# preshanth/rfi_toolbox

Measured on AMD Instinct MI355X. Metric: training patches/sec (128x128x3), higher is better.
Workload: dtype f32; 1 GPU; UNet(3,1,32) train step (fwd+BCE/dice+bwd+clip+Adam), batch 64/GPU x 128x128x3 NHWC, BASELINE configs[1] shape on the reference's U-Net (the '3-layer CNN' of configs[1] is not in the reference; its builder-defined form runs with --workload cnn3); global_batch=64, parallelism=dp1, params=7765985

## Files before the change

include/rfi_hip.h:

```cpp
#ifndef RFI_HIP_H
#define RFI_HIP_H

#include <stddef.h>
#include <stdint.h>

#ifdef __cplusplus
extern "C" {
#endif

#define RFI_HIP_ABI_VERSION 1

enum { RFI_HOST = 0, RFI_DEVICE = 1 };

typedef struct rfi_ctx rfi_ctx;
typedef struct rfi_model rfi_model;

int         rfi_abi_version(void);
const char* rfi_last_error(void);
int rfi_device_count(int* count);
int rfi_ctx_create(int device_id, rfi_ctx** out);
int rfi_ctx_destroy(rfi_ctx* ctx);
int rfi_ctx_set_overlap(rfi_ctx* ctx, int enabled);
int rfi_ctx_synchronize(rfi_ctx* ctx);
int rfi_ctx_stream(rfi_ctx* ctx, void** hip_stream);
// ... 147 lines not shown
                            const rfi_tiling* tiling, int batch, int combine, float threshold, uint8_t* flags,
                            int flags_mem, float* prob, int prob_mem);

typedef struct rfi_flag_stats {
    int64_t count;
    int64_t flagged;
    double mean, std, median, mad, max;
} rfi_flag_stats;
enum { RFI_FS_ALL = 1, RFI_FS_CLEAN = 2, RFI_FS_MEDIANS = 4 };
int rfi_flag_statistics(rfi_ctx* ctx, const void* data, int data_mem, int dtype, int64_t count,
                        const void* flags, int flags_mem, int flags_dtype, int want,
                        rfi_flag_stats* all_out, rfi_flag_stats* clean_out);

typedef struct rfi_sim_event {
    int32_t i0, i1, i2, i3;
    double s0, sdot, r0, phi0;
    double v0, v1;
} rfi_sim_event;
typedef struct rfi_sim_params {
    int32_t time_bins, freq_bins;
    int32_t n_power;
    int32_t gibbs_ringing;
    int32_t clean;
    int32_t fixed_baseline;
    double baseline_frac, detect_floor, drift_prob, max_time_fringes, max_freq_fringes;
    double gibbs_kernel[17];
} rfi_sim_params;
enum { RFI_SIM_C128 = 0, RFI_SIM_C64 = 1, RFI_SIM_NCHW = 2, RFI_SIM_NHWC = 3 };
#define RFI_SIM_SLOTS(T, F) (14 + (int)((double)(F) * 0.05) + (int)((double)(T) * 0.1))
int rfi_simulate_rfi(rfi_ctx* ctx, uint64_t seed, uint64_t first_sample, int n_samples, const rfi_sim_params* params,
                     const double* power_range_dev, int out_layout, void* out_dev, uint8_t* mask_dev,
                     rfi_sim_event* events_dev, double* baseline_frac_dev);

typedef struct rfi_norm_stats {
    int64_t count, nonfinite;
    double min, max, mean, var;
    double q[3][2];
} rfi_norm_stats;
enum { RFI_NORM_NCHW = 0, RFI_NORM_NHWC = 1 };
int rfi_norm_bracket(int64_t count, double q, int64_t* ranks, double* frac);
int rfi_norm_statistics(rfi_ctx* ctx, const void* const* chunks, const int64_t* counts, int n_chunks, int dtype,
                        int64_t segment, int quantiles, rfi_norm_stats* out, int n_out);
int rfi_norm_apply(rfi_ctx* ctx, const void* src_dev, int dtype, int src_layout, int n, int64_t pixels, double centre,
                   double scale, const double* params_dev, float* dst_dev, int dst_layout);

typedef struct rfi_augment_config {
    uint64_t seed;
    float p_hflip, p_vflip, p_rotate, rotate_limit_deg, p_ssr, shift_limit, scale_limit, ssr_rotate_limit_deg;
} rfi_augment_config;
int rfi_augment_params(const rfi_augment_config* cfg, uint64_t call, int n, int h, int w, int32_t* gates, double* inv);
int rfi_augment_batch(rfi_ctx* ctx, const float* x, int x_mem, const uint8_t* y, int y_mem, int n, int h, int w, int c,
                      const rfi_augment_config* cfg, uint64_t call, float* x_out, uint8_t* y_out);

int rfi_op_conv3x3(rfi_ctx* ctx, int impl, const float* x, int n, int h, int w, int cin,
                   const float* w_oihw, const float* bias, int cout,
                   const float* in_scale, const float* in_shift, int in_relu, float* y);
int rfi_op_conv1x1(rfi_ctx* ctx, int impl, const float* x, int n, int h, int w, int cin, const float* w_oihw, const float* bias,
                   int cout, const float* in_scale, const float* in_shift, int in_relu, float* y);
int rfi_op_conv3x3_dgrad(rfi_ctx* ctx, int impl, const float* dy, int n, int h, int w, int cout,
                         const float* w_oihw, int cin, float* dx);
int rfi_op_conv3x3_wgrad(rfi_ctx* ctx, int impl, const float* x, const float* dy, int n, int h,
                         int w, int cin, int cout, const float* in_scale, const float* in_shift,
                         int in_relu, float* dw_oihw);
int rfi_op_conv_s2(rfi_ctx* ctx, int impl, int ksize, const float* x, int n, int h, int w, int cin,
                   const float* w_oihw, int cout, float* y);
int rfi_op_conv_s2_dgrad(rfi_ctx* ctx, int impl, int ksize, const float* dy, int n, int h, int w, int cout,
                         const float* w_oihw, int cin, float* dx);
int rfi_op_conv_s2_wgrad(rfi_ctx* ctx, int impl, int ksize, const float* x, const float* dy, int n, int h, int w,
                         int cin, int cout, float* dw_oihw);
int rfi_op_convt2x2(rfi_ctx* ctx, int impl, const float* x, int n, int h, int w, int cin,
                    const float* w_iohw, const float* bias, int cout, float* y);
int rfi_op_convt2x2_dgrad(rfi_ctx* ctx, int impl, const float* dy, int n, int h, int w, int cout,
                          const float* w_iohw, int cin, float* dx);
int rfi_op_convt2x2_wgrad(rfi_ctx* ctx, int impl, const float* x, const float* dy, int n, int h,
                          int w, int cin, int cout, float* dw_iohw);
int rfi_op_roi_align(rfi_ctx* ctx, const float* x, int n, int h, int w, int c, const float* rois, int r,
                     float spatial_scale, int ph, int pw, int sampling_ratio, int aligned, float* out);
int rfi_op_roi_align_backward(rfi_ctx* ctx, const float* dout, int n, int h, int w, int c, const float* rois_sorted, int r,
                              float spatial_scale, int ph, int pw, int sampling_ratio, int aligned, float* dx);
int rfi_op_mask_targets(rfi_ctx* ctx, const uint8_t* masks, int g, int h, int w, const float* rois, int r, int ph, int pw,
                        int sampling_ratio, uint8_t* out);
int rfi_op_box_decode(rfi_ctx* ctx, const float* anchors, int64_t n_anchors, const float* deltas, int64_t n, float clip_h,
                      float clip_w, float* boxes);
int rfi_op_nms(rfi_ctx* ctx, const float* boxes_sorted, int n, float iou_threshold, int32_t* keep_host, int* n_keep);
int rfi_op_anchor_match_batched(rfi_ctx* ctx, const float* anchors, int64_t n, int64_t anchor_stride, const int32_t* anchor_count,
                                const float* gt_boxes, int images, int gt_max, const int32_t* gt_count, float fg_iou, float bg_iou,
                                int allow_low_quality, float* best_ws, int8_t* labels, int32_t* matched, float* targets);
int rfi_op_nms_batched(rfi_ctx* ctx, const float* boxes_sorted, const int32_t* count, int sets, int k, float iou_threshold, uint8_t* keep);
int rfi_op_rpn_loss(rfi_ctx* ctx, const float* head, int64_t pixels, int anchors_per_pixel, const int8_t* labels,
                    const float* targets, const int32_t* num_sampled_dev, float beta, float* dhead, void* workspace,
                    float* loss2_dev);
size_t rfi_op_rpn_loss_ws_bytes(void);
int rfi_op_segsort_u64(rfi_ctx* ctx, uint64_t* keys, int n_segs, int stride);
int rfi_op_sample_keys(rfi_ctx* ctx, const int8_t* labels, int images, int n, const int32_t* count, uint64_t seed, uint32_t step,
                       uint32_t stream0, uint64_t* keys, int stride);
int rfi_op_rpn_sample_apply(rfi_ctx* ctx, const uint64_t* keys_sorted, int images, int n, int stride, int batch, int max_pos,
                            const int8_t* labels, const float* targets, int levels, const int32_t* level_off_host,
                            int8_t* const* level_labels_host, float* const* level_targets_host, int32_t* n_sampled);
int rfi_op_topk_keys(rfi_ctx* ctx, const float* head, int images, int pixels, int anchors_per_pixel, uint64_t* keys, int stride);
int rfi_op_topk_decode(rfi_ctx* ctx, const uint64_t* keys_sorted, int images, int stride, int pixels, int anchors_per_pixel, int k,
                       const float* head, const float* anchors, float clip_h, float clip_w, float min_size, float* boxes, float* scores,
                       int32_t* counts, int levels, int level);
int rfi_op_proposals_select(rfi_ctx* ctx, const float* boxes, const float* scores, const uint8_t* keep, int images, int levels, int k,
                            int post_nms, const float* gt_boxes, int gt_max, const int32_t* gt_count, int pmax, float* props,
                            int32_t* pcount);
int rfi_op_roi_sample(rfi_ctx* ctx, const int8_t* labels, const int32_t* pcount, int images, int pmax, int batch, int max_pos,
                      uint64_t seed, uint32_t step, uint32_t stream0, int32_t* sel, int32_t* nsel, int32_t* npos);
int rfi_op_roi_compact(rfi_ctx* ctx, const int32_t* sel, const int32_t* nsel, const int32_t* npos, int images, int batch, int pmax,
                       const float* props, const int32_t* matched, const float* targets, const int32_t* gt_labels, int gt_max,
                       const int32_t* gt_base, float t1, float t2, float t3, float* rois, int32_t* cls, float* tgt, int32_t* gt,
                       int32_t* level, int32_t* img_start, float* rois_fg, float* rois_gt, int32_t* level_fg, int32_t* fg_start,
                       int32_t* counts);
int rfi_op_roi_align_ml(rfi_ctx* ctx, const float* const* maps_host, int n, int h0, int w0, int c, float scale0, const float* rois,
                        const int32_t* level, const int32_t* count_dev, int max_rois, int ph, int pw, int sampling_ratio, float* out);
int rfi_op_roi_align_ml_backward(rfi_ctx* ctx, float* const* dmaps_host, int n, int h0, int w0, int c, float scale0, const float* dout,
                                 const float* rois, const int32_t* level, const int32_t* img_start, int max_rois, int ph, int pw,
                                 int sampling_ratio);
int rfi_op_detect_candidates(rfi_ctx* ctx, const float* head, const float* props, const int32_t* pcount, int images, int pmax, int k1,
                             float clip_h, float clip_w, float score_thresh, float min_size, float* boxes, float* scores,
                             int32_t* counts);
int rfi_op_detect_select(rfi_ctx* ctx, const float* boxes, const float* scores, const uint8_t* keep, int images, int classes, int k,
                         int max_det, float t1, float t2, float t3, float* det_boxes, float* det_scores, int32_t* det_labels,
                         int32_t* det_count, float* rois, int32_t* level);
int rfi_op_rois_from_boxes(rfi_ctx* ctx, const float* props, const int32_t* pcount, int images, int pmax, float t1, float t2, float t3,
                           float* rois, int32_t* level);
int rfi_op_mask_paste(rfi_ctx* ctx, const float* logits, const float* det_boxes, const int32_t* det_count, int images, int max_det, int h,
                      int w, uint8_t* rfi_mask, uint8_t* masks);
int rfi_op_bn_add_relu16(rfi_ctx* ctx, const uint16_t* y, const float* scale, const float* shift, const uint16_t* s, const float* s_scale,
                         const float* s_shift, int64_t m, int c, uint16_t* out);
int rfi_op_relu_mask_sum16(rfi_ctx* ctx, const uint16_t* g0, const uint16_t* g1, const float* g2_f32, const uint16_t* g2_bf16,
                           int64_t g2_stride, const uint16_t* a, int64_t m, int c, uint16_t* dz);
int rfi_op_bn_backward16(rfi_ctx* ctx, const uint16_t* da, const uint16_t* y, int64_t m, int c, const float* gamma, const float* scale,
                         const float* shift, const float* mean, const float* invstd, float slope, uint16_t* dy, float* dgamma,
                         float* dbeta, float* dbias);
int rfi_readback_begin(rfi_ctx* ctx, const void* src_dev, size_t bytes);
int rfi_readback_end(rfi_ctx* ctx, void* dst_host, size_t bytes);
int rfi_op_fpn_merge(rfi_ctx* ctx, const float* lateral, const float* top, int n, int h, int w, int c, float* out);
int rfi_op_fpn_merge_backward(rfi_ctx* ctx, const float* dout, int n, int h, int w, int c, float* dtop);
int rfi_op_bn_stats(rfi_ctx* ctx, const float* y, int64_t m, int c, float* mean, float* var_biased);
int rfi_op_bn_relu_pool(rfi_ctx* ctx, const float* y, int n, int h, int w, int c, const float* scale,
                        const float* shift, float* skip, float* pooled);
int rfi_op_pool_bwd_merge(rfi_ctx* ctx, const float* y, int n, int h, int w, int c, const float* scale,
                          const float* shift, const float* dskip, const float* dpool, float* da);
int rfi_op_bn_relu_backward(rfi_ctx* ctx, const float* y, int64_t m, int c, const float* gamma,
                            const float* beta, float* da_inout, float* dgamma, float* dbeta, float* dbias);

#ifdef __cplusplus
}
#endif
#endif
```

rfi_toolbox_amd/_lib.py:

```python
from __future__ import annotations

import ctypes as C
import os

_HERE = os.path.dirname(os.path.abspath(__file__))
LIB_PATH = os.environ.get("RFI_HIP_LIB") or os.path.join(_HERE, "librfi_hip.so")

HOST, DEVICE = 0, 1
C128, C64, F64, F32 = 0, 1, 2, 3
U8, FLOAT32 = 0, 1
IMPL_AUTO, IMPL_DIRECT, IMPL_MFMA, IMPL_MFMA_BF16, IMPL_MFMA_BF16X3, IMPL_PLANES_X3, IMPL_PLANES_BF16, IMPL_WS_X3, IMPL_WS_BF16 = 0, 1, 2, 3, 4, 5, 6, 7, 8


FS_ALL, FS_CLEAN, FS_MEDIANS = 1, 2, 4


class FlagStats(C.Structure):
    _fields_ = [("count", C.c_int64), ("flagged", C.c_int64), ("mean", C.c_double), ("std", C.c_double),
                ("median", C.c_double), ("mad", C.c_double), ("max", C.c_double)]


SIM_C128, SIM_C64, SIM_NCHW, SIM_NHWC = 0, 1, 2, 3
NORM_NCHW, NORM_NHWC = 0, 1


class NormStats(C.Structure):
    _fields_ = [("count", C.c_int64), ("nonfinite", C.c_int64), ("min", C.c_double), ("max", C.c_double),
                ("mean", C.c_double), ("var", C.c_double), ("q", C.c_double * 2 * 3)]


class AugmentConfig(C.Structure):
    _fields_ = [("seed", C.c_uint64), ("p_hflip", C.c_float), ("p_vflip", C.c_float), ("p_rotate", C.c_float),
                ("rotate_limit_deg", C.c_float), ("p_ssr", C.c_float), ("shift_limit", C.c_float),
                ("scale_limit", C.c_float), ("ssr_rotate_limit_deg", C.c_float)]


class SimParams(C.Structure):
    _fields_ = [("time_bins", C.c_int32), ("freq_bins", C.c_int32), ("n_power", C.c_int32), ("gibbs_ringing", C.c_int32),
                ("clean", C.c_int32), ("fixed_baseline", C.c_int32), ("baseline_frac", C.c_double),
                ("detect_floor", C.c_double), ("drift_prob", C.c_double), ("max_time_fringes", C.c_double),
                ("max_freq_fringes", C.c_double), ("gibbs_kernel", C.c_double * 17)]


EDGE_PAD, EDGE_SHIFT = 0, 1
COMBINE_MEAN, COMBINE_MAX = 0, 1
VALUES_LOGITS, VALUES_PROBS = 0, 1


class Tiling(C.Structure):
    _fields_ = [("ps", C.c_int32), ("stride", C.c_int32), ("edge", C.c_int32), ("views", C.c_int32)]


class Hyper(C.Structure):
    _fields_ = [("lr", C.c_double), ("beta1", C.c_double), ("beta2", C.c_double), ("eps", C.c_double),
                ("weight_decay", C.c_double), ("max_grad_norm", C.c_double)]


def _load():
    if not os.path.exists(LIB_PATH):
        raise ImportError(
            f"{LIB_PATH} is missing: build it with `python -m rfi_toolbox_amd.build` "
            "(needs hipcc; gfx950 cross-compiles without a GPU). rfi_toolbox_amd has no CPU fallback.")
    return C.CDLL(LIB_PATH, mode=C.RTLD_GLOBAL)


lib = _load()

_vp, _i, _i64, _f, _sz = C.c_void_p, C.c_int, C.c_int64, C.c_float, C.c_size_t
_pi, _pi64, _pf, _pd = C.POINTER(C.c_int), C.POINTER(C.c_int64), C.POINTER(C.c_float), C.POINTER(C.c_double)
_pvp = C.POINTER(C.c_void_p)
_cp = C.c_char_p

_PROTOS = {
    "rfi_abi_version": (_i, []),
    "rfi_last_error": (_cp, []),
    "rfi_device_count": (_i, [_pi]),
    "rfi_ctx_create": (_i, [_i, _pvp]),
    "rfi_ctx_destroy": (_i, [_vp]),
    "rfi_ctx_synchronize": (_i, [_vp]),
    "rfi_ctx_set_overlap": (_i, [_vp, _i]),
    "rfi_ctx_stream": (_i, [_vp, _pvp]),
    "rfi_ctx_device_name": (_i, [_vp, _cp, _sz]),
    "rfi_ctx_allocations": (_i, [_vp, _pi64, C.POINTER(C.c_uint64)]),
    "rfi_malloc": (_i, [_vp, _sz, _pvp]),
    "rfi_free": (_i, [_vp, _vp]),
    "rfi_memcpy": (_i, [_vp, _vp, _i, _vp, _i, _sz]),
    "rfi_memset": (_i, [_vp, _vp, _i, _sz]),
    "rfi_timer_start": (_i, [_vp]),
    "rfi_timer_stop": (_i, [_vp, _pf]),
    "rfi_profile_enable": (_i, [_vp, _i]),
    "rfi_profile_reset": (_i, [_vp]),
    "rfi_profile_family_count": (_i, []),
    "rfi_profile_family_name": (_cp, [_i]),
    "rfi_profile_get": (_i, [_vp, _i, _pi64, _pd, _pd, _pd]),
    "rfi_profile_dump": (_i, [_vp, _cp]),
    "rfi_unet_create": (_i, [_vp, _i, _i, _i, _i, _pvp]),
    "rfi_cnn3_create": (_i, [_vp, _i, _i, _i, _pvp]),
    "rfi_unet_resnet_create": (_i, [_vp, _i, _i, _i, _pvp]),
    "rfi_mask_head_create": (_i, [_vp, _i, _i, _i, _pvp]),
    "rfi_model_input_grad": (_i, [_vp, _vp, _i]),
    "rfi_rpn_head_create": (_i, [_vp, _i, _i, _i, _pvp]),
    "rfi_box_head_create": (_i, [_vp, _i, _i, _i, _i, _pvp]),
    "rfi_op_add_inplace": (_i, [_vp, _vp, _vp, _i64]),
# ... 38 lines not shown
    "rfi_op_roi_align": (_i, [_vp, _vp, _i, _i, _i, _i, _vp, _i, _f, _i, _i, _i, _i, _vp]),
    "rfi_op_mask_targets": (_i, [_vp, _vp, _i, _i, _i, _vp, _i, _i, _i, _i, _vp]),
    "rfi_op_nms_batched": (_i, [_vp, _vp, _vp, _i, _i, _f, _vp]),
    "rfi_op_roi_align_backward": (_i, [_vp, _vp, _i, _i, _i, _i, _vp, _i, _f, _i, _i, _i, _i, _vp]),
    "rfi_op_fpn_merge": (_i, [_vp, _vp, _vp, _i, _i, _i, _i, _vp]),
    "rfi_op_box_decode": (_i, [_vp, _vp, _i64, _vp, _i64, _f, _f, _vp]),
    "rfi_op_nms": (_i, [_vp, _vp, _i, _f, _vp, _pi]),
    "rfi_op_rpn_loss_ws_bytes": (_sz, []),
    "rfi_op_rpn_loss": (_i, [_vp, _vp, _i64, _i, _vp, _vp, _vp, _f, _vp, _vp, _vp]),
    "rfi_op_fastrcnn_loss": (_i, [_vp, _vp, _i64, _i, _vp, _vp, _f, _vp, _vp, _vp]),
    "rfi_op_anchor_match_batched": (_i, [_vp, _vp, _i64, _i64, _vp, _vp, _i, _i, _vp, _f, _f, _i, _vp, _vp, _vp, _vp]),
    "rfi_op_segsort_u64": (_i, [_vp, _vp, _i, _i]),
    "rfi_op_sample_keys": (_i, [_vp, _vp, _i, _i, _vp, C.c_uint64, C.c_uint32, C.c_uint32, _vp, _i]),
    "rfi_op_rpn_sample_apply": (_i, [_vp, _vp, _i, _i, _i, _i, _i, _vp, _vp, _i, _vp, _vp, _vp, _vp]),
    "rfi_op_topk_keys": (_i, [_vp, _vp, _i, _i, _i, _vp, _i]),
    "rfi_op_topk_decode": (_i, [_vp, _vp, _i, _i, _i, _i, _i, _vp, _vp, _f, _f, _f, _vp, _vp, _vp, _i, _i]),
    "rfi_op_proposals_select": (_i, [_vp, _vp, _vp, _vp, _i, _i, _i, _i, _vp, _i, _vp, _i, _vp, _vp]),
    "rfi_op_roi_sample": (_i, [_vp, _vp, _vp, _i, _i, _i, _i, C.c_uint64, C.c_uint32, C.c_uint32, _vp, _vp, _vp]),
    "rfi_op_roi_compact": (_i, [_vp, _vp, _vp, _vp, _i, _i, _i, _vp, _vp, _vp, _vp, _i, _vp, _f, _f, _f, _vp, _vp, _vp, _vp, _vp, _vp,
                                _vp, _vp, _vp, _vp, _vp]),
    "rfi_op_roi_align_ml": (_i, [_vp, _vp, _i, _i, _i, _i, _f, _vp, _vp, _vp, _i, _i, _i, _i, _vp]),
    "rfi_op_roi_align_ml_backward": (_i, [_vp, _vp, _i, _i, _i, _i, _f, _vp, _vp, _vp, _vp, _i, _i, _i, _i]),
    "rfi_op_detect_candidates": (_i, [_vp, _vp, _vp, _vp, _i, _i, _i, _f, _f, _f, _f, _vp, _vp, _vp]),
    "rfi_op_detect_select": (_i, [_vp, _vp, _vp, _vp, _i, _i, _i, _i, _f, _f, _f, _vp, _vp, _vp, _vp, _vp, _vp]),
    "rfi_op_rois_from_boxes": (_i, [_vp, _vp, _vp, _i, _i, _f, _f, _f, _vp, _vp]),
    "rfi_op_mask_paste": (_i, [_vp, _vp, _vp, _vp, _i, _i, _i, _i, _vp, _vp]),
    "rfi_op_bn_add_relu16": (_i, [_vp, _vp, _vp, _vp, _vp, _vp, _vp, _i64, _i, _vp]),
    "rfi_op_relu_mask_sum16": (_i, [_vp, _vp, _vp, _vp, _vp, _i64, _vp, _i64, _i, _vp]),
    "rfi_op_bn_backward16": (_i, [_vp, _vp, _vp, _i64, _i, _vp, _vp, _vp, _vp, _vp, _f, _vp, _vp, _vp, _vp]),
    "rfi_readback_begin": (_i, [_vp, _vp, _sz]),
    "rfi_readback_end": (_i, [_vp, _vp, _sz]),
    "rfi_op_fpn_merge_backward": (_i, [_vp, _vp, _i, _i, _i, _i, _vp]),
    "rfi_comm_allreduce_sum_f32": (_i, [_vp, _vp, _i64]),
    "rfi_model_allreduce_grads": (_i, [_vp]),
    "rfi_preprocess_patches": (_i, [_vp, _vp, _i, _i, _i, _i, _i, _vp, _i]),
    "rfi_generate_waterfalls": (_i, [_vp, C.c_uint64, _i, _i, _i, _i, C.c_double, _i, _i, C.c_double, _vp, _vp, _i,
                                     _vp, _i, _vp, _i]),
    "rfi_preprocess_real": (_i, [_vp, _vp, _i, _i, _i, _i, _i, _i, _i, _i, C.c_double, _vp, _i, _vp, _i]),
    "rfi_mad_flags": (_i, [_vp, _vp, _i, _i, _i, _i, _i, C.c_double, _vp, _i]),
    "rfi_patch_any_flag": (_i, [_vp, _vp, _i, _i, _i, _i, _vp, _i, _i, _vp]),
    "rfi_preprocess_gather": (_i, [_vp, _vp, _i, _i, _i, _i, _i, _vp, _i, _vp, _i, _i, _vp, _i, _vp, _i]),
    "rfi_confusion_counts": (_i, [_vp, _vp, _i, _i, _vp, _i, _i, _i64, _pi64, _pi64, _pi64]),
    "rfi_threshold_logits": (_i, [_vp, _vp, _i64, _f, _vp]),
    "rfi_tiling_count": (_i, [_i, _i, C.POINTER(Tiling), _pi64]),
    "rfi_stitch_patches": (_i, [_vp, _vp, _i, _i, _i, _i, _i, C.POINTER(Tiling), _i, _f, _vp, _i, _vp, _i]),
    "rfi_model_predict_flags": (_i, [_vp, _vp, _i, _i, _i, _i, _i, C.POINTER(Tiling), _i, _i, _f, _vp, _i, _vp, _i]),
    "rfi_simulate_rfi": (_i, [_vp, C.c_uint64, C.c_uint64, _i, C.POINTER(SimParams), _vp, _i, _vp, _vp, _vp, _vp]),
    "rfi_flag_statistics": (_i, [_vp, _vp, _i, _i, _i64, _vp, _i, _i, _i, C.POINTER(FlagStats), C.POINTER(FlagStats)]),
    "rfi_norm_bracket": (_i, [_i64, C.c_double, _pi64, _pd]),
    "rfi_norm_statistics": (_i, [_vp, _pvp, _pi64, _i, _i, _i64, _i, C.POINTER(NormStats), _i]),
    "rfi_norm_apply": (_i, [_vp, _vp, _i, _i, _i, _i64, C.c_double, C.c_double, _vp, _vp, _i]),
    "rfi_augment_params": (_i, [C.POINTER(AugmentConfig), C.c_uint64, _i, _i, _i, C.POINTER(C.c_int32), _pd]),
    "rfi_augment_batch": (_i, [_vp, _vp, _i, _vp, _i, _i, _i, _i, _i, C.POINTER(AugmentConfig), C.c_uint64, _vp, _vp]),
    "rfi_op_conv3x3": (_i, [_vp, _i, _vp, _i, _i, _i, _i, _vp, _vp, _i, _vp, _vp, _i, _vp]),
    "rfi_op_conv1x1": (_i, [_vp, _i, _vp, _i, _i, _i, _i, _vp, _vp, _i, _vp, _vp, _i, _vp]),
    "rfi_op_conv_s2": (_i, [_vp, _i, _i, _vp, _i, _i, _i, _i, _vp, _i, _vp]),
    "rfi_op_conv_s2_dgrad": (_i, [_vp, _i, _i, _vp, _i, _i, _i, _i, _vp, _i, _vp]),
    "rfi_op_conv_s2_wgrad": (_i, [_vp, _i, _i, _vp, _vp, _i, _i, _i, _i, _i, _vp]),
    "rfi_op_conv3x3_dgrad": (_i, [_vp, _i, _vp, _i, _i, _i, _i, _vp, _i, _vp]),
    "rfi_op_conv3x3_wgrad": (_i, [_vp, _i, _vp, _vp, _i, _i, _i, _i, _i, _vp, _vp, _i, _vp]),
    "rfi_op_convt2x2": (_i, [_vp, _i, _vp, _i, _i, _i, _i, _vp, _vp, _i, _vp]),
    "rfi_op_convt2x2_dgrad": (_i, [_vp, _i, _vp, _i, _i, _i, _i, _vp, _i, _vp]),
    "rfi_op_convt2x2_wgrad": (_i, [_vp, _i, _vp, _vp, _i, _i, _i, _i, _i, _vp]),
    "rfi_op_bn_stats": (_i, [_vp, _vp, _i64, _i, _vp, _vp]),
    "rfi_op_bn_relu_pool": (_i, [_vp, _vp, _i, _i, _i, _i, _vp, _vp, _vp, _vp]),
    "rfi_op_pool_bwd_merge": (_i, [_vp, _vp, _i, _i, _i, _i, _vp, _vp, _vp, _vp, _vp]),
    "rfi_op_bn_relu_backward": (_i, [_vp, _vp, _i64, _i, _vp, _vp, _vp, _vp, _vp, _vp]),
}

for _name, (_res, _args) in _PROTOS.items():
    _fn = getattr(lib, _name)
    _fn.restype = _res
    _fn.argtypes = _args

EXPORTED = tuple(_PROTOS)


class RfiHipError(RuntimeError):
    pass


def check(rc):
    if rc != 0:
        raise RfiHipError(lib.rfi_last_error().decode("utf-8", "replace"))


def device_count() -> int:
    n = C.c_int(0)
    check(lib.rfi_device_count(C.byref(n)))
    return n.value
```

rfi_toolbox_amd/csrc/api_ops.cpp:

```cpp
#include <algorithm>

#include "model.hpp"

using namespace rfi;

namespace {
float* upload_lib_weight(rfi_ctx* ctx, CallScope& s, const float* dev_ref, size_t numel, bool convt,
                         int d0, int d1, int R) {
    std::vector<float> h(numel), lib;
    RFI_CHECK_HIP(hipMemcpyAsync(h.data(), dev_ref, numel * 4, hipMemcpyDeviceToHost, ctx->stream));
    RFI_CHECK_HIP(hipStreamSynchronize(ctx->stream));
    if (convt) to_lib_convt(h.data(), d0, d1, lib);
    else to_lib_conv(h.data(), d0, d1, R, lib);
    float* d = s.temp<float>(numel);
    RFI_CHECK_HIP(hipMemcpyAsync(d, lib.data(), numel * 4, hipMemcpyHostToDevice, ctx->stream));
    RFI_CHECK_HIP(hipStreamSynchronize(ctx->stream));
    return d;
}
void store_ref_wgrad(rfi_ctx* ctx, const float* lib_dev, size_t numel, bool convt, int d0, int d1, float* dst_ref) {
    std::vector<float> lib(numel), ref(numel);
    RFI_CHECK_HIP(hipMemcpyAsync(lib.data(), lib_dev, numel * 4, hipMemcpyDeviceToHost, ctx->stream));
    RFI_CHECK_HIP(hipStreamSynchronize(ctx->stream));
    if (convt) from_lib_convt(lib.data(), d0, d1, ref.data());
    else from_lib_conv(lib.data(), d0, d1, 3, ref.data());
    RFI_CHECK_HIP(hipMemcpyAsync(dst_ref, ref.data(), numel * 4, hipMemcpyHostToDevice, ctx->stream));
    RFI_CHECK_HIP(hipStreamSynchronize(ctx->stream));
}

struct PlaneTmp {
    bf16_t* p = nullptr;
    int64_t ps = 0;
    int nchunks = 0;
    PlaneSeg seg() const { return PlaneSeg{p, ps, nchunks}; }
};
PlaneTmp plane_tmp(rfi_ctx* ctx, CallScope& s, int64_t pixels, int C) {
    PlaneTmp t;
    t.nchunks = plane_chunks(C);
    t.ps = (int64_t)t.nchunks * 16;
    const size_t bytes = (size_t)pixels * t.ps * 2 + 64;
    t.p = reinterpret_cast<bf16_t*>(s.temp<float>((bytes + 3) / 4));
    RFI_CHECK_HIP(hipMemsetAsync(t.p, 0, bytes, ctx->stream));
    return t;
}
PlaneTmp planes_of(rfi_ctx* ctx, CallScope& s, const float* x, int64_t pixels, int C) {
    PlaneTmp t = plane_tmp(ctx, s, pixels, C);
    launch_act_split(ctx, View{x, C}, pixels, C, InXform{}, 1, t.p, t.ps);
    return t;
}
bf16_t* wb_of(rfi_ctx* ctx, CallScope& s, const float* src, int taps, int Cout, int Cin, int seg0, int seg1) {
    const size_t e = wb_elems(taps, Cout, seg0, seg1, 1);
    bf16_t* wb = reinterpret_cast<bf16_t*>(s.temp<float>((e * 2 + 64 + 3) / 4));
    RFI_CHECK_HIP(hipMemsetAsync(wb, 0, e * 2 + 64, ctx->stream));
    launch_weights_to_wb_one(ctx, WBDesc{src, wb, taps, Cout, Cin, {seg0, seg1}, 1});
    return wb;
}
}

extern "C" {

int rfi_op_conv3x3(rfi_ctx* ctx, int impl, const float* x, int n, int h, int w, int cin,
                   const float* w_oihw, const float* bias, int cout, const float* in_scale,
                   const float* in_shift, int in_relu, float* y) {
    return guarded([&] {
        ctx->activate();
        CallScope s(ctx);
        ConvArgs a;
        a.x = View{x, cin};
        a.N = n; a.H = h; a.W = w; a.Hin = h; a.Win = w; a.Cin = cin; a.Cout = cout;
        a.w = upload_lib_weight(ctx, s, w_oihw, (size_t)9 * cin * cout, false, cout, cin, 3);
        a.bias = bias;
        a.y = MutView{y, cout};
        a.Hout = h; a.Wout = w;
        a.xf = InXform{in_scale, in_shift, in_relu};
        launch_conv(ctx, a, impl);
    });
}
int rfi_op_conv1x1(rfi_ctx* ctx, int impl, const float* x, int n, int h, int w, int cin, const float* w_oihw, const float* bias,
                   int cout, const float* in_scale, const float* in_shift, int in_relu, float* y) {
    return guarded([&] {
        ctx->activate();
        CallScope s(ctx);
        ConvArgs a;
        a.x = View{x, cin};
        a.N = n; a.H = h; a.W = w; a.Hin = h; a.Win = w; a.Cin = cin; a.Cout = cout;
        a.w = upload_lib_weight(ctx, s, w_oihw, (size_t)cin * cout, false, cout, cin, 1);
        a.bias = bias;
        a.y = MutView{y, cout};
        a.Hout = h; a.Wout = w;
        a.R = 1; a.S = 1; a.pad = 0;
        a.xf = InXform{in_scale, in_shift, in_relu};
        launch_conv(ctx, a, impl);
    });
}
int rfi_op_conv3x3_dgrad(rfi_ctx* ctx, int impl, const float* dy, int n, int h, int w, int cout,
                         const float* w_oihw, int cin, float* dx) {
    return guarded([&] {
        ctx->activate();
        CallScope s(ctx);
        float* wf = upload_lib_weight(ctx, s, w_oihw, (size_t)9 * cin * cout, false, cout, cin, 3);
        float* wd = s.temp<float>((size_t)9 * cin * cout);
        launch_weight_to_dgrad(ctx, wf, 9, cout, cin, 1, wd);
        ConvArgs a;
        a.x = View{dy, cout};
        a.N = n; a.H = h; a.W = w; a.Hin = h; a.Win = w; a.Cin = cout; a.Cout = cin;
        a.w = wd;
        a.y = MutView{dx, cin};
        a.Hout = h; a.Wout = w;
        launch_conv(ctx, a, impl);
    });
}
int rfi_op_conv3x3_wgrad(rfi_ctx* ctx, int impl, const float* x, const float* dy, int n, int h, int w,
                         int cin, int cout, const float* in_scale, const float* in_shift, int in_relu,
                         float* dw_oihw) {
    return guarded([&] {
        ctx->activate();
        CallScope s(ctx);
        WgradArgs a;
        a.xop = View{x, cin};
        a.yop = View{dy, cout};
        a.xf_x = InXform{in_scale, in_shift, in_relu};
        a.N = n; a.H = h; a.W = w; a.Hx = h; a.Wx = w; a.Cx = cin; a.Cy = cout;
        a.tap_stride = (int64_t)cin * cout;
        a.sy = cin; a.sx = 1;
        const size_t numel = (size_t)9 * cin * cout;
        a.dw = s.temp<float>(numel);
        a.slab_floats = wgrad_slab_floats(a, impl);
        a.slab = s.temp<float>(a.slab_floats);
        launch_wgrad(ctx, a, impl);
        store_ref_wgrad(ctx, a.dw, numel, false, cout, cin, dw_oihw);
    });
}
int rfi_op_conv_s2(rfi_ctx* ctx, int impl, int ksize, const float* x, int n, int h, int w, int cin, const float* w_oihw,
                   int cout, float* y) {
    return guarded([&] {
        RFI_REQUIRE(ksize == 3 || ksize == 1, "conv_s2: kernel size 3 or 1");
        ctx->activate();
        CallScope s(ctx);
        if (impl == IMPL_PLANES_BF16) {
            RFI_REQUIRE(cout % 4 == 0, "conv_s2 on planes: cout % 4 == 0");
            const int64_t Mo = (int64_t)n * (h / 2) * (w / 2);
            const PlaneTmp xp = planes_of(ctx, s, x, (int64_t)n * h * w, cin);
            const float* wl = ksize == 3 ? upload_lib_weight(ctx, s, w_oihw, (size_t)9 * cin * cout, false, cout, cin, 3) : w_oihw;
            PlaneTmp yp = plane_tmp(ctx, s, Mo, cout);
            PConvArgs a;
            a.x[0] = xp.seg(); a.nseg = 1; a.P = 1;
            a.N = n; a.H = h / 2; a.W = w / 2; a.Hin = h; a.Win = w; a.Hout = h / 2; a.Wout = w / 2;
            a.R = ksize; a.S = 2; a.pad = ksize == 3 ? 1 : 0;
            a.Cout = cout;
            a.wB = wb_of(ctx, s, wl, ksize * ksize, cout, cin, cin, 0);
            a.y16 = yp.p; a.y_pstride = (int)yp.ps;
            launch_pconv(ctx, a);
            launch_planes_to_f32(ctx, yp.p, yp.ps, Mo, cout, 1, y, cout);
            return;
        }
        float* xs = s.temp<float>((size_t)n * h * w * cin);
        launch_s2d(ctx, x, n, h, w, cin, xs);
        ConvArgs a;
        a.N = n; a.H = h / 2; a.W = w / 2; a.Hin = h / 2; a.Win = w / 2; a.Cout = cout;
        a.x = View{xs, 4 * cin};
        a.y = MutView{y, cout};
        a.Hout = h / 2; a.Wout = w / 2;
        a.S = 1;
        if (ksize == 3) {
            float* w3 = upload_lib_weight(ctx, s, w_oihw, (size_t)9 * cin * cout, false, cout, cin, 3);
            float* w2 = s.temp<float>((size_t)16 * cin * cout);
            launch_w_s2d(ctx, w3, cout, cin, w2, true);
            a.w = w2; a.Cin = 4 * cin; a.R = 2; a.pad = 1;
        } else {
            a.w = w_oihw; a.Cin = cin; a.R = 1; a.pad = 0;
        }
        launch_conv(ctx, a, impl);
// ... 493 lines not shown
                      const rfi_augment_config* cfg, uint64_t call, float* x_out, uint8_t* y_out) {
    return guarded([&] {
        RFI_REQUIRE(ctx, "augment_batch: null context");
        check_augment_config(cfg, n, h, w);
        RFI_REQUIRE(c >= 1 && c <= 16, "augment_batch: 1 <= c <= 16");
        if (n == 0) return;
        const int64_t px = (int64_t)n * h * w;
        RFI_REQUIRE(cdiv((int64_t)h * w, 256) * n <= 0x7fffffff, "augment_batch: batch too large for one launch");
        RFI_REQUIRE(x && y && x_out && y_out, "augment_batch: null buffer");
        const char *xi = reinterpret_cast<const char*>(x), *xo = reinterpret_cast<const char*>(x_out);
        const char *yi = reinterpret_cast<const char*>(y), *yo = reinterpret_cast<const char*>(y_out);
        RFI_REQUIRE(x_mem == RFI_HOST || xi + px * c * 4 <= xo || xo + px * c * 4 <= xi, "augment_batch: x and x_out overlap");
        RFI_REQUIRE(y_mem == RFI_HOST || yi + px <= yo || yo + px <= yi, "augment_batch: y and y_out overlap");
        ctx->activate();
        CallScope sc(ctx);
        const float* dx = sc.in(x, x_mem, (size_t)px * c);
        const uint8_t* dy = sc.in(y, y_mem, (size_t)px);
        const uintptr_t al = c % 4 == 0 ? 16 : 4;
        RFI_REQUIRE(reinterpret_cast<uintptr_t>(dx) % al == 0 && reinterpret_cast<uintptr_t>(x_out) % al == 0,
                    "augment_batch: float buffers must be 4-byte aligned (16-byte when c % 4 == 0)");
        launch_augment(ctx, dx, dy, n, h, w, c, *cfg, call, x_out, y_out);
        sc.finish();
    });
}
int rfi_op_fpn_merge(rfi_ctx* ctx, const float* lateral, const float* top, int n, int h, int w, int c, float* out) {
    return guarded([&] {
        ctx->activate();
        launch_fpn_merge_fwd(ctx, lateral, top, n, h, w, c, out);
    });
}
int rfi_op_fpn_merge_backward(rfi_ctx* ctx, const float* dout, int n, int h, int w, int c, float* dtop) {
    return guarded([&] {
        ctx->activate();
        launch_fpn_merge_bwd_top(ctx, dout, n, h, w, c, dtop);
    });
}
int rfi_op_bn_stats(rfi_ctx* ctx, const float* y, int64_t m, int c, float* mean, float* var_biased) {
    return guarded([&] {
        ctx->activate();
        CallScope s(ctx);
        float* ws = s.temp<float>(bn_stats_ws_floats(c));
        float* tmp = s.temp<float>((size_t)6 * c);
        std::vector<float> ones((size_t)c, 1.0f), zeros((size_t)c, 0.0f);
        RFI_CHECK_HIP(hipMemcpyAsync(tmp, ones.data(), c * 4, hipMemcpyHostToDevice, ctx->stream));
        RFI_CHECK_HIP(hipMemcpyAsync(tmp + c, zeros.data(), c * 4, hipMemcpyHostToDevice, ctx->stream));
        RFI_CHECK_HIP(hipStreamSynchronize(ctx->stream));
        launch_bn_stats(ctx, y, m, c, ws);
        launch_bn_finalize(ctx, ws, m, c, tmp, tmp + c, nullptr, nullptr, 0, mean, tmp + 2 * c, tmp + 3 * c,
                           tmp + 4 * c, var_biased);
    });
}

int rfi_op_bn_relu_pool(rfi_ctx* ctx, const float* y, int n, int h, int w, int c, const float* scale,
                        const float* shift, float* skip, float* pooled) {
    return guarded([&] {
        ctx->activate();
        launch_bn_relu_pool(ctx, y, n, h, w, c, scale, shift, MutView{skip, c}, pooled);
    });
}
int rfi_op_pool_bwd_merge(rfi_ctx* ctx, const float* y, int n, int h, int w, int c, const float* scale,
                          const float* shift, const float* dskip, const float* dpool, float* da) {
    return guarded([&] {
        ctx->activate();
        launch_pool_bwd_merge(ctx, y, n, h, w, c, scale, shift, View{dskip, c}, dpool, da);
    });
}
int rfi_op_bn_relu_backward(rfi_ctx* ctx, const float* y, int64_t m, int c, const float* gamma,
                            const float* beta, float* da_inout, float* dgamma, float* dbeta, float* dbias) {
    return guarded([&] {
        ctx->activate();
        CallScope s(ctx);
        size_t wsf = bn_stats_ws_floats(c);
        if (bn_bwd_ws_floats(m, c) > wsf) wsf = bn_bwd_ws_floats(m, c);
        float* ws = s.temp<float>(wsf);
        float* t = s.temp<float>((size_t)6 * c);
        launch_bn_stats(ctx, y, m, c, ws);
        launch_bn_finalize(ctx, ws, m, c, gamma, beta, nullptr, nullptr, 0, t, t + c, t + 2 * c, t + 3 * c,
                           nullptr);
        launch_bn_bwd_reduce(ctx, da_inout, y, m, c, t + 2 * c, t + 3 * c, t, t + c, ws, t + 4 * c, t + 5 * c,
                             dgamma, dbeta);
        launch_bn_bwd_apply(ctx, da_inout, y, m, c, t + 2 * c, t + 3 * c, t, t + c, gamma, t + 4 * c, t + 5 * c,
                            ws, dbias);
    });
}

}
```

rfi_toolbox_amd/csrc/conv_mfma.hip:

```cpp
#include <algorithm>
#include <vector>

#include "planes.hpp"

namespace rfi {

void launch_conv_direct(rfi_ctx* ctx, const ConvArgs& a);

namespace {

typedef float f32x4 __attribute__((ext_vector_type(4)));
typedef float f32x16 __attribute__((ext_vector_type(16)));
typedef float f32x2 __attribute__((ext_vector_type(2)));
typedef __bf16 bf16x2 __attribute__((ext_vector_type(2)));
typedef short s16x4 __attribute__((ext_vector_type(4)));
typedef unsigned u32x2 __attribute__((ext_vector_type(2)));

__device__ __forceinline__ s16x4 pack_bf16(f32x4 x) {
    const f32x2 lo = {x.x, x.y}, hi = {x.z, x.w};
    u32x2 r;
    r.x = __builtin_bit_cast(unsigned, __builtin_convertvector(lo, bf16x2));
    r.y = __builtin_bit_cast(unsigned, __builtin_convertvector(hi, bf16x2));
    return __builtin_bit_cast(s16x4, r);
}
// ... 572 lines not shown
        *reinterpret_cast<u32x2*>(rec) = u32x2{h0, h1};
        *reinterpret_cast<u32x2*>(rec + 8) = u32x2{m0, m1};
        *reinterpret_cast<u32x2*>(rec + 16) = u32x2{l0, l1};
    }
}
__global__ void weights_to_x3_batched_kernel(const X3Desc* __restrict__ descs) {
    const X3Desc d = descs[blockIdx.y];
    const int64_t total = d.rows * d.nchunks * 4;
    for (int64_t i = (int64_t)blockIdx.x * blockDim.x + threadIdx.x; i < total; i += (int64_t)gridDim.x * blockDim.x) {
        const int q = (int)(i & 3);
        const int64_t rc = i >> 2;
        const int chunk = (int)(rc % d.nchunks);
        const int64_t row = rc / d.nchunks;
        const int c = chunk * KC + q * 4;
        f32x4 v = {0.f, 0.f, 0.f, 0.f};
        if (c < d.Cin) v = *reinterpret_cast<const f32x4*>(d.src + row * d.Cin + c);
        unsigned h0, m0, l0, h1, m1, l1;
        split_pair(v.x, v.y, h0, m0, l0);
        split_pair(v.z, v.w, h1, m1, l1);
        float* rec = d.dst + rc * WROW3 + q * 2;
        *reinterpret_cast<u32x2*>(rec) = u32x2{h0, h1};
        *reinterpret_cast<u32x2*>(rec + 8) = u32x2{m0, m1};
        *reinterpret_cast<u32x2*>(rec + 16) = u32x2{l0, l1};
    }
}
}
void launch_weights_to_x3_batched(rfi_ctx* ctx, const X3Desc* descs_dev, int n, double total_bytes) {
    ProfScope ps(ctx, FAM_ELEMWISE, 0, total_bytes);
    hipLaunchKernelGGL(weights_to_x3_batched_kernel, dim3(128, n), dim3(256), 0, ctx->stream, descs_dev);
    check_launch("weights_to_x3_batched");
}
void launch_weights_to_x3(rfi_ctx* ctx, const float* w, int taps, int Cout, int Cin, float* out) {
    const int nchunks = (Cin + KC - 1) / KC;
    const int64_t rows = (int64_t)taps * Cout, total = rows * nchunks * 4;
    ProfScope ps(ctx, FAM_ELEMWISE, 0, (double)rows * Cin * 4 + (double)rows * nchunks * 96);
    int64_t blocks = cdiv(total, 256);
    if (blocks > 4096) blocks = 4096;
    hipLaunchKernelGGL(weights_to_x3_kernel, dim3((unsigned)blocks), dim3(256), 0, ctx->stream, w, rows, Cin, nchunks, out);
    check_launch("weights_to_x3");
}

bool conv_mfma_eligible(const ConvArgs& a) {
    if (a.Cin % 4 != 0 || a.x.pstride % 4 != 0) return false;
    if ((reinterpret_cast<uintptr_t>(a.x.p) & 15) || (reinterpret_cast<uintptr_t>(a.w) & 15)) return false;
    if (a.xf.scale && ((reinterpret_cast<uintptr_t>(a.xf.scale) & 15) ||
                       (reinterpret_cast<uintptr_t>(a.xf.shift) & 15)))
        return false;
    const bool known = (a.R == 3 && a.S == 1 && a.pad == 1) || (a.R == 1 && a.S == 1 && a.pad == 0) ||
                       (a.R == 2 && a.S == 2 && a.pad == 0) || (a.R == 2 && a.S == 1 && (a.pad == 1 || a.pad == 0));
    return known;
}

void launch_conv(rfi_ctx* ctx, ConvArgs& a, int impl) {
    if (impl == IMPL_PLANES_X3 || impl == IMPL_PLANES_BF16) {
        RFI_REQUIRE(a.R == 3 && a.S == 1 && a.zgroups == 1, "conv: the plane kernels cover 3x3 stride-1 convolutions");
        a.planes = impl == IMPL_PLANES_X3 ? 3 : 1;
        impl = IMPL_MFMA;
    }
    if (impl == IMPL_MFMA_BF16) {
        a.bf16 = true;
        impl = IMPL_MFMA;
    }
    if (impl == IMPL_MFMA_BF16X3) {
        a.bf16x3 = true;
        a.wB3 = nullptr;
        impl = IMPL_MFMA;
    }
    if (impl == IMPL_WS_X3 && conv_stem_eligible(a)) {
        a.bf16x3 = true;
        launch_conv_stem(ctx, a);
        return;
    }
    if (impl == IMPL_WS_X3 || impl == IMPL_WS_BF16) {
        const int P = impl == IMPL_WS_X3 ? 3 : 1;
        const bool gw = !conv_ws_eligible(a) && gemm_ws_eligible(a);
        RFI_REQUIRE(gw || conv_ws_eligible(a), "conv: shape not eligible for the wave-specialised kernels");
        RFI_REQUIRE(!gw || P == 3, "conv: the wave-specialised GEMM kernel exists in the 3 x bf16 arithmetic only");
        a.bf16x3 = P == 3;
        a.bf16 = P == 1;
        const int taps = gw ? (a.R == 2 ? 4 : 1) : 9, cout = gw && a.zgroups == 4 ? 4 * a.Cout : a.Cout;
        CallScope sc(ctx);
        bf16_t* wb = sc.temp<bf16_t>(wb_elems(taps, cout, a.Cin, 0, P) + 32);
        launch_weights_to_wb_one(ctx, WBDesc{a.w, wb, taps, cout, a.Cin, {a.Cin, 0}, P});
        if (gw) launch_gemm_ws(ctx, a, wb);
        else launch_conv_ws(ctx, a, wb, P);
        return;
    }
    if (impl == IMPL_AUTO && a.bf16x3 && conv_stem_eligible(a)) {
        launch_conv_stem(ctx, a);
        return;
    }
    if (impl == IMPL_AUTO && a.bf16x3 && a.wB3 && conv_ws_eligible(a)) {
        launch_conv_ws(ctx, a, a.wB3, 3);
        return;
    }
    if (impl == IMPL_AUTO && a.bf16 && a.wB1 && conv_ws_eligible(a)) {
        launch_conv_ws(ctx, a, a.wB1, 1);
        return;
    }
    if (impl == IMPL_AUTO && a.bf16x3 && a.wB3 && gemm_ws_eligible(a)) {
        launch_gemm_ws(ctx, a, a.wB3);
        return;
    }
    RFI_REQUIRE(a.N > 0 && a.H > 0 && a.W > 0 && a.Cin > 0 && a.Cout > 0, "conv: empty shape");
    RFI_REQUIRE(a.x.pstride >= a.Cin && a.y.pstride >= a.Cout, "conv: pixel stride smaller than channels");
    RFI_REQUIRE(a.zgroups == 1 || (a.zgroups == 4 && a.R == 1), "conv: zgroups only for convT forward");
// ... 54 lines not shown
```

rfi_toolbox_amd/csrc/conv_ws.hip:

```cpp
#include <algorithm>
#include <type_traits>
#include <vector>

#include <hip/hip_ext.h>

#include "ws_common.hpp"

namespace rfi {
namespace {

using namespace ws;

struct WsDev {
    const float* x;
    int x_ps;
    unsigned x_bytes;
    const float* scale;
    const float* shift;
    float slope;
    int N, H, W, Cin, Cout;
    const bf16_t* wB;
    int nkc, ncb;
    const float* bias;
    float* y;
    int y_ps;
    double* stats;
    int wide_epi;
    unsigned long long* stamps;
};

template <int P> constexpr int ROWB = 32 * P + 16;

template <int TB, int TH, int TW, int NTL, bool ADB, int P>
struct WsCfg {
    static constexpr int HH = TH + 2, HW = TW + 2, HPI = HH * HW, HP = TB * HPI;
    static constexpr int A_BYTES = (HP * ROWB<P> + 1023) & ~1023;
    static constexpr int NPIECE = 9 * NTL * P;
    static constexpr int B_BYTES = NPIECE * 1024;
    static constexpr int B_ITEMS = (NPIECE + 3) / 4;
    static constexpr int HALO_ITEMS = (HP * 4 + 255) / 256;
    static constexpr int B_OFF = (ADB ? 2 : 1) * A_BYTES;
    static constexpr int STAT_OFF = B_OFF + 2 * B_BYTES;
    static constexpr int STAT_BYTES = 4 * NTL * 64 * 2 * 8;
    static constexpr int EPI_WAVE_BYTES = 16 * 36 * 4;
    static constexpr bool WIDE_OK = STAT_OFF + 4 * EPI_WAVE_BYTES <= 160 * 1024;
    static constexpr int LDS_BYTES = STAT_OFF + ((STAT_BYTES > 4 * EPI_WAVE_BYTES || !WIDE_OK) ? STAT_BYTES : 4 * EPI_WAVE_BYTES);
    static_assert(TB * TH * TW == 256, "a tile is 256 output pixels");
    static_assert(32 % TW == 0 || TW % 32 == 0, "a 32-pixel block covers whole rows or a part of one");
    static_assert(LDS_BYTES <= 160 * 1024, "LDS budget");
};


template <int TB, int TH, int TW, int NTL, int XF, bool ADB, int P>
__global__ __launch_bounds__(512) void conv_ws_kernel(WsDev d) {
    using C = WsCfg<TB, TH, TW, NTL, ADB, P>;
    constexpr int RB = ROWB<P>;
    extern __shared__ __attribute__((aligned(16))) unsigned char smem[];
#ifdef RFI_DIAG_STAMPS
    unsigned long long st_[4] = {0, 0, 0, 0};
#endif
    const int tid = threadIdx.x;
    const int lane = tid & 63, wave = __builtin_amdgcn_readfirstlane(tid >> 6);

    const int tiles_x = (d.W + TW - 1) / TW, tiles_y = (d.H + TH - 1) / TH, tiles_b = (d.N + TB - 1) / TB;
    const int ntiles = tiles_b * tiles_y * tiles_x;
    const int GX = gridDim.x;
    int t_begin, t_count, j, gx;
    if (GX >= 8 && (GX & 7) == 0) {
        const int xcd = blockIdx.x & 7, q8 = ntiles >> 3, r8 = ntiles & 7;
        j = blockIdx.x >> 3;
        gx = GX >> 3;
        t_begin = xcd < r8 ? xcd * (q8 + 1) : r8 * (q8 + 1) + (xcd - r8) * q8;
        t_count = q8 + (xcd < r8 ? 1 : 0);
    } else {
        j = blockIdx.x; gx = GX; t_begin = 0; t_count = ntiles;
    }
    const int my_tiles = (j < t_count) ? (t_count - j + gx - 1) / gx : 0;
    const int cb0 = blockIdx.y * NTL, n0 = cb0 * 32;
    double* const st_out = d.stats ? d.stats + ((size_t)blockIdx.x * d.Cout + n0) * 2 : nullptr;
    if (my_tiles == 0) {
        if (st_out && tid < 32 * NTL && n0 + tid < d.Cout) st_out[tid * 2] = st_out[tid * 2 + 1] = 0.0;
        return;
    }
    struct Tile { int n, oy0, ox0; };
    auto tile_of = [&](int k) {
        const int t = t_begin + j + k * gx;
        Tile r;
        r.ox0 = (t % tiles_x) * TW;
        r.oy0 = ((t / tiles_x) % tiles_y) * TH;
        r.n = (t / (tiles_x * tiles_y)) * TB;
        return r;
    };
    const int nkc = d.nkc;
    const int nitems = my_tiles * nkc;
    double* const s_stat = reinterpret_cast<double*>(smem + C::STAT_OFF);

    if (wave >= 4) {
        const int ptid = tid - 256, pw = wave - 4;
        const unsigned q4b = (unsigned)(ptid & 3) * 16u;
        const __amdgpu_buffer_rsrc_t xrs = __builtin_amdgcn_make_buffer_rsrc(const_cast<float*>(d.x), 0, (int)d.x_bytes, 0x00020000);
        unsigned h_rc[C::HALO_ITEMS];
#pragma unroll
        for (int it = 0; it < C::HALO_ITEMS; ++it) {
            const int idx = ptid + it * 256, pix = idx >> 2;
            const int b = pix / C::HPI, rem = pix % C::HPI;
            h_rc[it] = idx < C::HP * 4 ? ((unsigned)b << 24) | ((unsigned)(rem / C::HW) << 12) | (unsigned)(rem % C::HW) : (0xfffu << 12);
        }
        unsigned voff[C::HALO_ITEMS];
        unsigned vmsk[C::HALO_ITEMS];
        auto setup_halo = [&](const Tile& t) {
#pragma unroll
            for (int it = 0; it < C::HALO_ITEMS; ++it) {
                const int n = t.n + (int)(h_rc[it] >> 24);
                const int iy = t.oy0 - 1 + (int)((h_rc[it] >> 12) & 0xfff), ix = t.ox0 - 1 + (int)(h_rc[it] & 0xfff);
                const bool ok = n < d.N && (unsigned)iy < (unsigned)d.H && (unsigned)ix < (unsigned)d.W;
                voff[it] = ok ? (unsigned)(((n * d.H + iy) * d.W + ix) * d.x_ps) * 4u + q4b : 0x80000000u;
                vmsk[it] = ok ? 0xffffffffu : 0u;
            }
        };
        u32x4 raw[C::HALO_ITEMS];
        f32x4 screg = {1.f, 1.f, 1.f, 1.f}, shreg = {0.f, 0.f, 0.f, 0.f};
        unsigned pl[C::HALO_ITEMS][2 * P];
        auto issue_loads = [&](int c0) {
            if constexpr (XF != 0) {
                screg = *reinterpret_cast<const f32x4*>(d.scale + c0 + (ptid & 3) * 4);
                shreg = *reinterpret_cast<const f32x4*>(d.shift + c0 + (ptid & 3) * 4);
            }
            __builtin_amdgcn_sched_barrier(0);
#pragma unroll
            for (int it = 0; it < C::HALO_ITEMS; ++it) raw[it] = __builtin_amdgcn_raw_buffer_load_b128(xrs, voff[it], c0 * 4, 0);
        };
        auto split_all = [&]() {
#pragma unroll
            for (int it = 0; it < C::HALO_ITEMS; ++it) {
                f32x4 v = __builtin_bit_cast(f32x4, raw[it]);
                if constexpr (XF != 0) {
#pragma unroll
                    for (int e = 0; e < 4; ++e) {
                        float t = v[e] * screg[e] + shreg[e];
                        if constexpr (XF == 1) asm("v_max_f32 %0, 0, %1" : "=v"(t) : "v"(t));
                        else t = __builtin_fmaxf(t, t * d.slope);
                        v[e] = __builtin_bit_cast(float, __builtin_bit_cast(unsigned, t) & vmsk[it]);
                    }
                }
                if constexpr (P == 3) {
                    split_pair(v.x, v.y, pl[it][0], pl[it][2], pl[it][4]);
                    split_pair(v.z, v.w, pl[it][1], pl[it][3], pl[it][5]);
                } else {
                    pl[it][0] = cvt_pair(v.x, v.y);
                    pl[it][1] = cvt_pair(v.z, v.w);
                }
            }
        };
        auto write_all = [&](int buf) {
            unsigned char* const sA = smem + buf * C::A_BYTES + (ptid >> 2) * RB + (ptid & 3) * 8;
#pragma unroll
            for (int it = 0; it < C::HALO_ITEMS; ++it) {
                if (ptid + it * 256 < C::HP * 4) {
                    unsigned char* row = sA + it * 64 * RB;
#pragma unroll
                    for (int p = 0; p < P; ++p) *reinterpret_cast<u32x2*>(row + 32 * p) = u32x2{pl[it][2 * p], pl[it][2 * p + 1]};
                }
            }
        };
        const unsigned char* const wb = reinterpret_cast<const unsigned char*>(d.wB);
        auto issue_B = [&](int kc, int buf) {
            unsigned char* const sB = smem + C::B_OFF + buf * C::B_BYTES;
#pragma unroll
            for (int i = 0; i < C::B_ITEMS; ++i) {
                const int p = pw + 4 * i;
                if (p < C::NPIECE) {
                    const int tap = p / (P * NTL), r = p - tap * (P * NTL), nt = r / P, plane = r - nt * P;
                    const int cb = cb0 + nt < d.ncb ? cb0 + nt : d.ncb - 1;
                    const unsigned off = (unsigned)((((tap * nkc + kc) * d.ncb + cb) * P + plane) * 1024 + lane * 16);
                    __builtin_amdgcn_global_load_lds((gbl_void*)(wb + off), (lds_void*)(sB + p * 1024), 16, 0, 0);
                }
            }
        };
        int lk = 0, lch = 0;
        Tile lt = tile_of(0);
        setup_halo(lt);
        issue_loads(0);
        for (int q = -1; q < nitems; ++q) {
            WS_T(t0);
            const bool more = q + 1 < nitems;
            if (more) {
                split_all();
                WS_T(t1);
                WS_ACC(2, t0, t1);
                if constexpr (ADB) write_all((q + 1) & 1);
                __builtin_amdgcn_sched_barrier(0);
                issue_B(lch, (q + 1) & 1);
                __builtin_amdgcn_sched_barrier(0);
                if (q + 2 < nitems) {
                    if (++lch == nkc) {
                        lch = 0;
                        ++lk;
                        lt = tile_of(lk);
                        setup_halo(lt);
                    }
                }
                issue_loads(lch * 16);
                __builtin_amdgcn_sched_barrier(0);
                WS_T(t2);
                wait_vmcnt<C::HALO_ITEMS>();
                if constexpr (ADB) asm volatile("s_waitcnt lgkmcnt(0)" ::: "memory");
                WS_T(t3);
                WS_ACC(3, t2, t3);
            }
            WS_T(t4);
            wg_barrier();
            if constexpr (!ADB) {
                if (more) write_all(0);
                asm volatile("s_waitcnt lgkmcnt(0)" ::: "memory");
                wg_barrier();
            }
            WS_T(t5);
            WS_ACC(0, t0, t4);
            WS_ACC(1, t4, t5);
        }
    } else {
        const int cw = wave, li = lane & 31, lh = lane >> 5;
        int a_base[2];
#pragma unroll
        for (int mt = 0; mt < 2; ++mt) {
            const int p = cw * 64 + mt * 32 + li;
            const int b = p / (TH * TW), r = p % (TH * TW);
            a_base[mt] = ((b * C::HH + r / TW) * C::HW + r % TW) * RB + lh * 16;
        }
        const int b_base = lane * 16;
        float bias[NTL];
        unsigned lane_off[NTL];
#pragma unroll
        for (int nt = 0; nt < NTL; ++nt) {
            const int co = n0 + nt * 32 + li;
            bias[nt] = (d.bias && co < d.Cout) ? d.bias[co] : 0.0f;
            asm volatile("" : "+v"(bias[nt]));
            lane_off[nt] = (unsigned)(4 * lh * d.y_ps + co);
        }
        constexpr bool DEFER = NTL == 1;
        f32x16 acc[2][NTL], outr[2][NTL];
#pragma unroll
        for (int mt = 0; mt < 2; ++mt)
#pragma unroll
            for (int nt = 0; nt < NTL; ++nt)
#pragma unroll
                for (int r = 0; r < 16; ++r) acc[mt][nt][r] = 0.0f;
        double d1[NTL], d2[NTL];
        float s1[NTL], s2[NTL];
#pragma unroll
        for (int nt = 0; nt < NTL; ++nt) { d1[nt] = d2[nt] = 0.0; s1[nt] = s2[nt] = 0.0f; }
        constexpr int E = 32 * NTL;
        auto epi_elem = [&](const f32x16 (&src)[2][NTL], int e, unsigned tile_off) {
            const int nt = e / 32, mt = (e >> 4) & 1, r = e & 15;
            const int p = cw * 64 + mt * 32 + (r & 3) + 8 * (r >> 2);
// ... 198 lines not shown
                    }
                    epi_finish();
                }
                cch = 0;
                ++ck;
                if (ck < my_tiles) ct = tile_of(ck);
            }
            WS_T(t4);
            wg_barrier();
            WS_T(t5);
            WS_ACC(0, t0, t1);
            WS_ACC(2, t1, t4);
            WS_ACC(1, t4, t5);
        }
        if constexpr (DEFER) {
            if (pend) {
                epi_generic(outr, pt);
                epi_finish();
            }
        }
        if (st_out) {
#pragma unroll
            for (int nt = 0; nt < NTL; ++nt) {
                s_stat[((cw * NTL + nt) * 64 + lane) * 2] = d1[nt];
                s_stat[((cw * NTL + nt) * 64 + lane) * 2 + 1] = d2[nt];
            }
        }
    }
#ifdef RFI_DIAG_STAMPS
    if (d.stamps && lane == 0) {
        unsigned long long* o = d.stamps + ((size_t)(blockIdx.y * gridDim.x + blockIdx.x) * 8 + wave) * 8;
        for (int i = 0; i < 4; ++i) o[i] = st_[i];
        o[4] = (unsigned long long)nitems;
    }
#endif
    if (st_out) {
        __syncthreads();
        if (tid < 32 * NTL && n0 + tid < d.Cout) {
            const int nt = tid >> 5, cl = tid & 31;
            double t1 = 0.0, t2 = 0.0;
#pragma unroll
            for (int w = 0; w < 4; ++w)
#pragma unroll
                for (int h = 0; h < 2; ++h) {
                    t1 += s_stat[((w * NTL + nt) * 64 + h * 32 + cl) * 2];
                    t2 += s_stat[((w * NTL + nt) * 64 + h * 32 + cl) * 2 + 1];
                }
            st_out[tid * 2] = t1;
            st_out[tid * 2 + 1] = t2;
        }
    }
}

template <int TB, int TH, int TW, int NTL, int XF, int P>
void launch_ws(rfi_ctx* ctx, ConvArgs& a, WsDev& d) {
    constexpr bool ADB = NTL == 1 || P == 1;
    using C = WsCfg<TB, TH, TW, NTL, ADB, P>;
    const int ntiles = (int)(cdiv(a.N, TB) * cdiv(a.H, TH) * cdiv(a.W, TW));
    const int ycols = (int)cdiv(d.ncb, NTL);
    const int gmax = std::max(8, 256 / ycols);
    const int tx = (int)cdiv(ntiles, 8);
    const int per = (int)cdiv(tx, std::max(1, gmax / 8));
    int GX = 8 * (int)cdiv(tx, per);
    if (ntiles < 8) GX = ntiles;
    if (a.stats && GX <= a.stats_max_records) a.stats_records = GX;
    else { a.stats = nullptr; a.stats_records = 0; }
    d.stats = a.stats;
    static PerDeviceOnce attr_once;
    attr_once.run(ctx->device, [&] {
        RFI_CHECK_HIP(hipFuncSetAttribute(reinterpret_cast<const void*>(&conv_ws_kernel<TB, TH, TW, NTL, XF, ADB, P>),
                                          hipFuncAttributeMaxDynamicSharedMemorySize, (int)C::LDS_BYTES));
    });
#ifdef RFI_DIAG_STAMPS
    {
        const size_t nw = (size_t)GX * ycols * 8;
        RFI_CHECK_HIP(hipMalloc(reinterpret_cast<void**>(&d.stamps), nw * 64));
        RFI_CHECK_HIP(hipMemsetAsync(d.stamps, 0, nw * 64, ctx->stream));
        hipLaunchKernelGGL((conv_ws_kernel<TB, TH, TW, NTL, XF, ADB, P>), dim3(GX, ycols), dim3(512), C::LDS_BYTES, ctx->stream, d);
        std::vector<unsigned long long> hs(nw * 8);
        RFI_CHECK_HIP(hipMemcpyAsync(hs.data(), d.stamps, nw * 64, hipMemcpyDeviceToHost, ctx->stream));
        RFI_CHECK_HIP(hipStreamSynchronize(ctx->stream));
        double c[5] = {0, 0, 0, 0, 0}, p[5] = {0, 0, 0, 0, 0};
        for (size_t w = 0; w < nw; ++w)
            for (int i = 0; i < 5; ++i) ((w & 7) < 4 ? c : p)[i] += (double)hs[w * 8 + i];
        std::fprintf(stderr, "[stamps] conv_ws<%d,%d,%d,%d,%d> N%d %dx%d %d->%d grid %dx%d items/wg %.1f | cycles per item: consumer mfma %.0f "
                     "epilogue %.0f barriers %.0f (+ in front of tap 8: %.0f) | producer work %.0f (split %.0f, dma wait %.0f) barriers+write %.0f\n", TB, TH, TW, NTL, XF,
                     a.N, a.H, a.W, a.Cin, a.Cout, GX, ycols, c[4] / (nw / 2), c[0] / c[4], c[2] / c[4], c[1] / c[4], c[3] / c[4], p[0] / p[4],
                     p[2] / p[4], p[3] / p[4], p[1] / p[4]);
        RFI_CHECK_HIP(hipFree(d.stamps));
        d.stamps = nullptr;
        return;
    }
#endif
    if (a.done) {
        hipExtLaunchKernelGGL((conv_ws_kernel<TB, TH, TW, NTL, XF, ADB, P>), dim3(GX, ycols), dim3(512), C::LDS_BYTES, ctx->stream, nullptr,
                              a.done, 0, d);
        a.done_used = true;
    } else {
        hipLaunchKernelGGL((conv_ws_kernel<TB, TH, TW, NTL, XF, ADB, P>), dim3(GX, ycols), dim3(512), C::LDS_BYTES, ctx->stream, d);
    }
    check_launch("conv_ws");
}

template <int NTL, int XF, int P>
void dispatch_ws(rfi_ctx* ctx, ConvArgs& a, WsDev& d) {
    if (a.W >= 32) launch_ws<1, 8, 32, NTL, XF, P>(ctx, a, d);
    else if (a.W >= 16) launch_ws<1, 16, 16, NTL, XF, P>(ctx, a, d);
    else launch_ws<4, 8, 8, NTL, XF, P>(ctx, a, d);
}
template <int NTL, int P>
void dispatch_xf(rfi_ctx* ctx, ConvArgs& a, WsDev& d, int xf) {
    if (xf == 0) dispatch_ws<NTL, 0, P>(ctx, a, d);
    else if (xf == 1) dispatch_ws<NTL, 1, P>(ctx, a, d);
    else dispatch_ws<NTL, 2, P>(ctx, a, d);
}

}

bool conv_ws_eligible(const ConvArgs& a) {
    if (!(a.R == 3 && a.S == 1 && a.pad == 1 && a.zgroups == 1 && a.fold == 0)) return false;
    if (a.Hin != a.H || a.Win != a.W || a.Hout != a.H || a.Wout != a.W) return false;
    if (a.osy != 1 || a.osx != 1 || a.ooy != 0 || a.oox != 0) return false;
    if (a.y16 || a.W < 8 || a.H < 8) return false;
    if (a.Cin % 16 != 0 || a.x.pstride % 4 != 0 || (reinterpret_cast<uintptr_t>(a.x.p) & 15)) return false;
    if (a.xf.scale && ((reinterpret_cast<uintptr_t>(a.xf.scale) & 15) || (reinterpret_cast<uintptr_t>(a.xf.shift) & 15))) return false;
    if ((int64_t)a.N * a.H * a.W * a.x.pstride * 4 >= (int64_t)1 << 31 || (int64_t)a.N * a.H * a.W * a.y.pstride >= (int64_t)1 << 31) return false;
    return true;
}

void launch_conv_ws(rfi_ctx* ctx, ConvArgs& a, const bf16_t* wB, int P) {
    RFI_REQUIRE(conv_ws_eligible(a), "conv_ws: shape not eligible");
    RFI_REQUIRE(P == 1 || P == 3, "conv_ws: planes must be 1 or 3");
    WsDev d;
    d.x = a.x.p; d.x_ps = a.x.pstride;
    d.x_bytes = (unsigned)((int64_t)a.N * a.H * a.W * a.x.pstride * 4);
    d.scale = a.xf.scale; d.shift = a.xf.shift;
    d.slope = a.xf.relu == 0 ? 1.0f : a.xf.slope;
    d.N = a.N; d.H = a.H; d.W = a.W; d.Cin = a.Cin; d.Cout = a.Cout;
    d.wB = wB;
    d.nkc = plane_chunks(a.Cin); d.ncb = (a.Cout + 31) / 32;
    RFI_REQUIRE((int64_t)wb_elems(9, a.Cout, a.Cin, 0, P) * 2 < ((int64_t)1 << 32), "conv_ws: filter tensor too large");
    d.bias = a.bias;
    d.y = a.y.p; d.y_ps = a.y.pstride;
    d.stats = nullptr;
    d.stamps = nullptr;
    d.wide_epi = a.y.pstride % 4 == 0 && (reinterpret_cast<uintptr_t>(a.y.p) & 15) == 0;
    const int64_t tiles = (a.W >= 16 ? (int64_t)a.N : cdiv(a.N, 4)) * cdiv(a.H, a.W >= 32 ? 8 : a.W >= 16 ? 16 : 8) * cdiv(a.W, a.W >= 32 ? 32 : a.W >= 16 ? 16 : 8);
    int ntl = 1;
    if (a.Cout > 32 && tiles * cdiv(d.ncb, 2) >= 224) ntl = 2;
    if (P == 1 && a.Cout > 64 && tiles * cdiv(d.ncb, 4) >= 224) ntl = 4;
    const double flops = a.algo_flops >= 0 ? a.algo_flops : 2.0 * a.N * a.H * a.W * (double)a.Cout * 9 * a.Cin;
    std::string label;
    if (ctx->profiling)
        label = "conv_ws N" + std::to_string(a.N) + " " + std::to_string(a.H) + "x" + std::to_string(a.W) + " " +
                std::to_string(a.Cin) + "->" + std::to_string(a.Cout) + (a.xf.scale ? " xf" : "") + (P == 3 ? " 3xbf16" : " bf16") +
                (a.W >= 32 ? " t8x32" : a.W >= 16 ? " t16x16" : " t4x8x8") + " ntl" + std::to_string(ntl);
    const double bytes = 4.0 * ((double)a.N * a.H * a.W * a.Cin + 9.0 * a.Cin * a.Cout) + 4.0 * a.N * a.H * a.W * a.Cout;
    ProfScope ps(ctx, FAM_CONV_MFMA, flops, bytes, label);
    const int xf = !a.xf.scale ? 0 : (a.xf.relu == 1 || (a.xf.relu == 2 && a.xf.slope == 0.0f)) ? 1 : 2;
    if (P == 3) {
        if (ntl == 2) dispatch_xf<2, 3>(ctx, a, d, xf);
        else dispatch_xf<1, 3>(ctx, a, d, xf);
    } else {
        if (ntl == 4) dispatch_xf<4, 1>(ctx, a, d, xf);
        else if (ntl == 2) dispatch_xf<2, 1>(ctx, a, d, xf);
        else dispatch_xf<1, 1>(ctx, a, d, xf);
    }
}

}
```

rfi_toolbox_amd/csrc/elem_kernels.hip:

```cpp
#include <hip/hip_ext.h>

#include "kernels.hpp"

namespace rfi {

namespace {

constexpr int kBlock = 256;
constexpr int kFinCh = 2;
constexpr int kFinLanes = kBlock / kFinCh;

__device__ __forceinline__ double wave_sum(double v) {
#pragma unroll
    for (int o = 32; o > 0; o >>= 1) v += __shfl_down(v, o, 64);
    return v;
}

__device__ __forceinline__ double finish_sum(double v, double* red) {
#pragma unroll
    for (int o = 32; o >= kFinCh; o >>= 1) v += __shfl_xor(v, o, 64);
    const int wave = threadIdx.x >> 6, lane = threadIdx.x & 63;
    __syncthreads();
    if (lane < kFinCh) red[wave * kFinCh + lane] = v;
    __syncthreads();
// ... 1442 lines not shown
    }
    if (dbias && finish_dbias) launch_bn_bwd_apply_finish(ctx, partial_ws, M, C, dbias);
}
void launch_bn_bwd_apply_finish(rfi_ctx* ctx, const float* partial_ws, int64_t M, int C, float* dbias) {
    ChanGeom g = geom_rows(M, C);
    ProfScope ps(ctx, FAM_BN);
    hipLaunchKernelGGL(finish_channel_sum_kernel, dim3((int)cdiv(C, kFinCh)), dim3(kBlock), 0,
                       ctx->stream, reinterpret_cast<const double*>(partial_ws), g.rblocks, (int64_t)C, C, dbias);
    check_launch("finish_channel_sum");
}

int bn_bwd_apply_records(int64_t M, int C) { return geom_rows(M, C).rblocks; }
void launch_finish_channel_sums_batched(rfi_ctx* ctx, const FinishSumDesc* descs_dev, int n, int max_count) {
    if (n <= 0) return;
    ProfScope ps(ctx, FAM_BN);
    hipLaunchKernelGGL(finish_channel_sum_batched_kernel, dim3((int)cdiv(max_count, kFinCh), n), dim3(kBlock), 0, ctx->stream, descs_dev);
    check_launch("finish_channel_sum_batched");
}

size_t channel_sum_ws_floats(int64_t M, int C) {
    (void)M;
    return (size_t)kMaxRowBlocks * C * 2;
}
void launch_channel_sum(rfi_ctx* ctx, YRef v, int64_t M, int C, float* partial_ws, float* out, bool finish) {
    ChanGeom g = geom_rows(M, C);
    const int pstride = (int)v.stride(C);
    const bool vec = g.V == 4 && pstride % 4 == 0 && (reinterpret_cast<uintptr_t>(v.p) & (v.bf16 ? 7 : 15)) == 0;
    RFI_REQUIRE(finish || vec, "channel_sum: deferred finishing needs the vector path (C % 4 == 0, an aligned view)");
    RFI_REQUIRE(vec || !v.bf16, "channel_sum: a bfloat16 view needs C % 4 == 0 and 8-byte aligned rows");
    if (!vec && g.V == 4) g = geom_rows(M, C, false);
    {
        ProfScope ps(ctx, FAM_REDUCE, 0, (double)M * C * (v.bf16 ? 2 : 4));
        if (g.V == 4)
            hipLaunchKernelGGL(channel_sum_kernel<4>, dim3(g.rblocks, g.cblocks), dim3(kBlock), 0, ctx->stream,
                               v.p, v.bf16, pstride, M, C, g.CL, g.rows_per_block,
                               reinterpret_cast<double*>(partial_ws));
        else
            hipLaunchKernelGGL(channel_sum_kernel<1>, dim3(g.rblocks, g.cblocks), dim3(kBlock), 0, ctx->stream,
                           v.p, v.bf16, pstride, M, C, g.CL, g.rows_per_block,
                           reinterpret_cast<double*>(partial_ws));
        check_launch("channel_sum");
    }
    if (finish) {
        ProfScope ps(ctx, FAM_REDUCE);
        hipLaunchKernelGGL(finish_channel_sum_kernel, dim3((int)cdiv(C, kFinCh)), dim3(kBlock), 0,
                           ctx->stream, reinterpret_cast<const double*>(partial_ws), g.rblocks, (int64_t)C, C, out);
        check_launch("finish_channel_sum");
    }
}
void launch_channel_sum(rfi_ctx* ctx, View v, int64_t M, int C, float* partial_ws, float* out, bool finish) {
    launch_channel_sum(ctx, YRef(v.p, (int64_t)v.pstride), M, C, partial_ws, out, finish);
}

void launch_bn_relu_pool(rfi_ctx* ctx, const float* y, int N, int H, int W, int C,
                         const float* scale, const float* shift, MutView skip, float* pooled, float slope) {
    const int64_t total = (int64_t)N * (H / 2) * (W / 2) * C;
    RFI_REQUIRE(skip.p || pooled, "bn_relu_pool: nothing to write");
    {
        ProfScope ps(ctx, FAM_ELEMWISE, 0, (double)N * H * W * C * (skip.p ? 8 : 4) + (pooled ? (double)total * 4 : 0.0));
        if (skip.p && pooled)
            hipLaunchKernelGGL((bn_relu_pool_kernel<true, true>), dim3(grid_for(total)), dim3(kBlock), 0, ctx->stream, y,
                               N, H, W, C, scale, shift, skip.p, skip.pstride, pooled, slope);
        else if (pooled)
            hipLaunchKernelGGL((bn_relu_pool_kernel<false, true>), dim3(grid_for(total)), dim3(kBlock), 0, ctx->stream, y,
                               N, H, W, C, scale, shift, nullptr, 0, pooled, slope);
        else
            hipLaunchKernelGGL((bn_relu_pool_kernel<true, false>), dim3(grid_for(total)), dim3(kBlock), 0, ctx->stream, y,
                               N, H, W, C, scale, shift, skip.p, skip.pstride, nullptr, slope);
        check_launch("bn_relu_pool");
    }
    if (skip.p && ((H & 1) || (W & 1))) {
        ProfScope ps(ctx, FAM_ELEMWISE);
        hipLaunchKernelGGL(bn_relu_edge_kernel, dim3(grid_for((int64_t)N * H * W * C)), dim3(kBlock), 0,
                           ctx->stream, y, N, H, W, C, scale, shift, skip.p, skip.pstride, slope);
        check_launch("bn_relu_edge");
    }
}

static bool pool_vec_ok(YRef y, int C, const float* scale, const float* shift, YRef dskip, YRef dpool_, const float* da) {
    const void* dpool = dpool_.p;
    return C % 4 == 0 && dskip.stride(C) % 4 == 0 && y.stride(C) % 4 == 0 &&
           !((reinterpret_cast<uintptr_t>(y.p) | reinterpret_cast<uintptr_t>(scale) | reinterpret_cast<uintptr_t>(shift) |
              reinterpret_cast<uintptr_t>(dskip.p) | reinterpret_cast<uintptr_t>(dpool) | reinterpret_cast<uintptr_t>(da)) & 15);
}
int launch_pool_bwd_merge_sums(rfi_ctx* ctx, YRef y, int N, int H, int W, int C, const float* scale,
                               const float* shift, const float* mean, const float* invstd, YRef dskip, YRef dpool,
                               float* da, float slope, float* partial_ws, unsigned short* da16) {
    if (!pool_vec_ok(y, C, scale, shift, dskip, dpool, da16 ? reinterpret_cast<const float*>(da16) : da) || dpool.stride(C) != C ||
        (reinterpret_cast<uintptr_t>(da16) & 7) ||
        ((reinterpret_cast<uintptr_t>(mean) | reinterpret_cast<uintptr_t>(invstd)) & 15))
        return 0;
    const int C4 = C / 4;
    const int64_t total = (int64_t)N * (H / 2) * (W / 2) * C4;
    const bool small = C4 <= kBlock && kBlock % C4 == 0, wide = C4 > kBlock && C4 % kBlock == 0;
    if ((H & 1) || (W & 1) || !(small || wide) || total < (int64_t)kBlock * 16) return 0;
    int grid = grid_for(total, kMaxRowBlocks);
    int records = grid;
    if (wide) {
        const int per = C4 / kBlock;
        grid = std::max(per, grid / per * per);
        records = grid / per;
    }
    if ((int64_t)grid * kBlock > total) return 0;
    ProfScope ps(ctx, FAM_ELEMWISE, 0, (double)N * H * W * C * (y.bf16 ? 10 : 12) + (double)total * (dpool.bf16 ? 8 : 16));
    hipLaunchKernelGGL(pool_bwd_merge_vec_kernel<true>, dim3(grid), dim3(kBlock), 0, ctx->stream, y.p, y.bf16, y.stride(C), N, H, W,
                       C, scale, shift, mean, invstd, dskip.p, dskip.bf16, (int)dskip.stride(C), dpool.p, dpool.bf16, da, slope, reinterpret_cast<double*>(partial_ws), da16);
// ... 287 lines not shown
```

rfi_toolbox_amd/csrc/kernels.hpp:

```cpp
#pragma once
#include "common.hpp"

namespace rfi {

struct InXform {
    const float* scale = nullptr;
    const float* shift = nullptr;
    int relu = 0;
    float slope = 0.0f;
};
static inline InXform act_xform(const float* scale, const float* shift, float slope) {
    return InXform{scale, shift, slope != 0.0f ? 2 : 1, slope};
}

struct View {
    const float* p = nullptr;
    int pstride = 0;
};
struct MutView {
    float* p = nullptr;
    int pstride = 0;
};

struct ConvArgs {
    View x;
    int N = 0, H = 0, W = 0;
    int Hin = 0, Win = 0;
    int Cin = 0, Cout = 0;
    const float* w = nullptr;
    const float* w3 = nullptr;
    const unsigned short* wB3 = nullptr;
    const unsigned short* wB1 = nullptr;
    const float* bias = nullptr;
    MutView y;
    int Hout = 0, Wout = 0;
    int osy = 1, osx = 1;
    int ooy = 0, oox = 0;
    int R = 3, S = 1, pad = 1;
    int zgroups = 1;
    unsigned short* y16 = nullptr;
    int fold = 0;
    InXform xf;
    double algo_flops = -1;
    bool bf16 = false;
    bool bf16x3 = false;
    int planes = 0;
    double* stats = nullptr;
    int stats_max_records = 0;
    int stats_records = 0;
    hipEvent_t done = nullptr;
    bool done_used = false;
#ifdef RFI_DIAG_STAMPS
    unsigned long long* stamps = nullptr;
#endif
};

enum ConvImpl { IMPL_AUTO = 0, IMPL_DIRECT = 1, IMPL_MFMA = 2, IMPL_MFMA_BF16 = 3, IMPL_MFMA_BF16X3 = 4,
                IMPL_PLANES_X3 = 5, IMPL_PLANES_BF16 = 6, IMPL_WS_X3 = 7, IMPL_WS_BF16 = 8 };
bool conv_ws_eligible(const ConvArgs& a);
void launch_conv_ws(rfi_ctx* ctx, ConvArgs& a, const unsigned short* wB, int P);
bool gemm_ws_eligible(const ConvArgs& a);
void launch_gemm_ws(rfi_ctx* ctx, ConvArgs& a, const unsigned short* wB3);

bool conv_mfma_eligible(const ConvArgs& a);
size_t weights_x3_floats(int taps, int Cout, int Cin);
void launch_weights_to_x3(rfi_ctx* ctx, const float* w, int taps, int Cout, int Cin, float* out);
struct X3Desc { const float* src; float* dst; int64_t rows; int Cin; int nchunks; };
void launch_weights_to_x3_batched(rfi_ctx* ctx, const X3Desc* descs_dev, int n, double total_bytes);
bool conv_stem_eligible(const ConvArgs& a);
void launch_conv_stem(rfi_ctx* ctx, ConvArgs& a);
void launch_conv(rfi_ctx* ctx, ConvArgs& a, int impl = IMPL_AUTO);

struct WgradArgs {
    View xop, yop;
    InXform xf_x, xf_y;
    int N = 0, H = 0, W = 0;
    int Hx = 0, Wx = 0;
    int Cx = 0, Cy = 0;
    int R = 3, S = 1, pad = 1;
    float* dw = nullptr;
    int64_t tap_stride = 0;
    int sy = 0, sx = 0;
    float* slab = nullptr;
    size_t slab_floats = 0;
    double algo_flops = -1;
    bool bf16 = false;
    bool bf16x3 = false;
    int planes = 0;
};
size_t wgrad_slab_floats(const WgradArgs& a, int impl);
bool wgrad_ws_eligible(const WgradArgs& a);
void launch_wgrad_ws(rfi_ctx* ctx, const WgradArgs& a);
size_t wgrad_ws_slab_floats(const WgradArgs& a);
bool wgrad_stem_eligible(const WgradArgs& a);
void launch_wgrad_stem(rfi_ctx* ctx, const WgradArgs& a);
void launch_wgrad(rfi_ctx* ctx, const WgradArgs& a, int impl = IMPL_AUTO);

struct YRef {
    const void* p = nullptr;
    int bf16 = 0;
    int64_t ps = 0;
    YRef(const float* f) : p(f) {}
    YRef(float* f) : p(f) {}
    YRef(const float* f, int64_t pstride) : p(f), ps(pstride) {}
    YRef(const unsigned short* h, int64_t pstride) : p(h), bf16(1), ps(pstride) {}
    YRef(View v) : p(v.p), ps(v.pstride) {}
    int64_t stride(int C) const { return ps ? ps : C; }
};

size_t bn_stats_ws_floats(int C);
void launch_bn_stats(rfi_ctx* ctx, const float* y, int64_t M, int C, float* partial_ws);
void launch_bn_finalize(rfi_ctx* ctx, const float* partial_ws, int64_t M, int C, const float* gamma,
                        const float* beta, float* running_mean, float* running_var,
                        int ema_repeats, float* mean, float* invstd, float* scale, float* shift,
                        float* var_out, int records = 0,
                        hipEvent_t done = nullptr);
void launch_bn_eval_coeffs(rfi_ctx* ctx, int C, const float* gamma, const float* beta,
                           const float* running_mean, const float* running_var, float* scale,
                           float* shift);
void launch_bn_bwd_reduce(rfi_ctx* ctx, YRef da, YRef y, int64_t M, int C,
                          const float* scale, const float* shift, const float* mean,
                          const float* invstd, float* partial_ws, float* c1, float* c2,
                          float* dgamma, float* dbeta, float slope = 0.0f);
size_t bn_bwd_ws_floats(int64_t M, int C);
void launch_bn_bwd_finalize_records(rfi_ctx* ctx, const float* partial_ws, int records, int64_t M, int C, float* c1,
                                    float* c2, float* dgamma, float* dbeta);
void launch_bn_bwd_apply(rfi_ctx* ctx, YRef da_inout, YRef y, int64_t M, int C,
                         const float* scale, const float* shift, const float* mean,
                         const float* invstd, const float* gamma, const float* c1, const float* c2,
                         float* partial_ws, float* dbias, float slope = 0.0f,
                         unsigned short* planes_out = nullptr, int64_t planes_pstride = 0, int planes_P = 0,
                         hipEvent_t done = nullptr, bool finish_dbias = true, const float* head_dl = nullptr,
                         const float* head_w = nullptr);
void launch_bn_bwd_apply_finish(rfi_ctx* ctx, const float* partial_ws, int64_t M, int C, float* dbias);
struct FinishSumDesc { const double* partial; int records; int64_t stride; int count; float* out; };
int bn_bwd_apply_records(int64_t M, int C);
void launch_finish_channel_sums_batched(rfi_ctx* ctx, const FinishSumDesc* descs_dev, int n, int max_count);

void launch_bn_relu_pool(rfi_ctx* ctx, const float* y, int N, int H, int W, int C,
                         const float* scale, const float* shift, MutView skip, float* pooled, float slope = 0.0f);
void launch_pool_bwd_merge(rfi_ctx* ctx, YRef y, int N, int H, int W, int C,
                           const float* scale, const float* shift, YRef dskip, YRef dpool,
                           float* da, float slope = 0.0f, unsigned short* da16 = nullptr);
int launch_pool_bwd_merge_sums(rfi_ctx* ctx, YRef y, int N, int H, int W, int C, const float* scale,
                               const float* shift, const float* mean, const float* invstd, YRef dskip, YRef dpool,
                               float* da, float slope, float* partial_ws, unsigned short* da16 = nullptr);
void launch_head_fwd(rfi_ctx* ctx, YRef y, int64_t M, int C, const float* scale,
                     const float* shift, const float* w, const float* b, int Cout, float* logits,
                     float slope = 0.0f);
void launch_sigmoid_fwd(rfi_ctx* ctx, const float* z, int64_t n, float* x);
void launch_sigmoid_bwd(rfi_ctx* ctx, const float* x, int64_t n, float* d_inout);
void launch_loss_reduce(rfi_ctx* ctx, const float* logits, const uint8_t* labels, int64_t count,
                        double* partial_ws, double* sums4, float* loss_out);
size_t loss_ws_doubles(int64_t count);
void launch_loss_bwd(rfi_ctx* ctx, const float* logits, const uint8_t* labels, int64_t count,
                     const double* sums4, float* dlogits);
void launch_focal_reduce(rfi_ctx* ctx, const float* logits, const uint8_t* labels, int64_t count, float alpha,
                         float gamma, double* partial_ws, float* loss_out);
void launch_focal_bwd(rfi_ctx* ctx, const float* logits, const uint8_t* labels, int64_t count, float alpha,
                      float gamma, float* dlogits);
int launch_head_bwd(rfi_ctx* ctx, YRef y, int64_t M, int C, const float* scale,
                    const float* shift, const float* w, int Cout, const float* dlogits, float* da,
                    float* partial_ws, float* dw, float* db, float slope = 0.0f, const float* bn_mean = nullptr,
                    const float* bn_invstd = nullptr, float* bn_records_ws = nullptr, unsigned short* da16 = nullptr,
                    bool* skip_da = nullptr, bool finish = true);
size_t head_bwd_ws_floats(int64_t M, int C, int Cout);
void launch_channel_sum(rfi_ctx* ctx, View v, int64_t M, int C, float* partial_ws, float* out, bool finish = true);
void launch_channel_sum(rfi_ctx* ctx, YRef v, int64_t M, int C, float* partial_ws, float* out, bool finish = true);
size_t channel_sum_ws_floats(int64_t M, int C);

void launch_nchw_to_nhwc(rfi_ctx* ctx, const float* src, int N, int C, int H, int W, float* dst);
void launch_nhwc_to_nchw(rfi_ctx* ctx, const float* src, int N, int C, int H, int W, float* dst);
void launch_weight_to_dgrad(rfi_ctx* ctx, const float* wf, int taps, int Cout, int Cin, int flip,
                            float* wd);
struct RelayoutDesc {
    int64_t src_off, dst_off;
    int taps, cout, cin, flip;
    int64_t tile0 = 0;
};
int64_t relayout_assign_tiles(RelayoutDesc* descs, int n);
void launch_weight_to_dgrad_batched(rfi_ctx* ctx, const RelayoutDesc* descs_dev, int n, const float* src,
                                    float* dst, double total_bytes, int64_t total_tiles);
void launch_u8_to_f32(rfi_ctx* ctx, const uint8_t* src, int64_t n, float* dst);
void launch_relu_bwd(rfi_ctx* ctx, float* dA, const float* Y, int64_t n);
void launch_pad_channels(rfi_ctx* ctx, const float* src, int64_t M, int c, int cp, float* dst);

void launch_sumsq(rfi_ctx* ctx, const float* g, int64_t n, double* partial_ws, double* sumsq);
size_t sumsq_ws_doubles(int64_t n);
struct AdamArgs {
    float* p; float* g; float* m; float* v; int64_t n;
    float beta2, eps, wd, max_norm, grad_scale;
    float one_minus_beta1, one_minus_beta2;
    float neg_step, bc2_sqrt;
// ... 127 lines not shown
```

rfi_toolbox_amd/csrc/model.cpp:

```cpp
#include "model.hpp"

#include <cmath>
#include <cstdlib>
#include <random>

using namespace rfi;

namespace rfi {

void DevBuf::ensure(rfi_ctx* c, size_t floats) {
    if (floats <= n && p) return;
    if (p) c->release(p);
    ctx = c;
    p = static_cast<float*>(c->alloc(floats * sizeof(float)));
    n = floats;
}
void DevBuf::free() {
    if (p && ctx) ctx->release(p);
    p = nullptr;
    n = 0;
}

}

// ... 70 lines not shown
    if (wb_pool) { ctx->release(wb_pool); wb_pool = nullptr; }
    if (wb_descs) { ctx->release(wb_descs); wb_descs = nullptr; }
    planesP = P;
    wd_dirty = true;
    pN = 0;
}

void rfi_model::prepare(int n, int h, int w) {
    RFI_REQUIRE(n > 0 && h > 0 && w > 0, "forward: empty batch or image");
    join_pending_side();
    if (ctx->stream != ctx->main_stream) {
        ctx->stream = ctx->main_stream;
        RFI_CHECK_HIP(hipStreamSynchronize(ctx->side_stream));
        side_seq = 0;
    }
    if (side_seq != 0 || ctx->fork_ring_used != 0 || ctx->bucket_ev_used != 0 || pend_hi > pend_lo) {
        RFI_CHECK_HIP(hipStreamSynchronize(ctx->main_stream));
        RFI_CHECK_HIP(hipStreamSynchronize(ctx->side_stream));
        if (ctx->comm_stream) RFI_CHECK_HIP(hipStreamSynchronize(ctx->comm_stream));
        side_seq = 0;
        ctx->fork_ring_used = 0;
        ctx->bucket_ev_used = 0;
        pend_lo = pend_hi = 0;
    }
    prepare_shape(n, h, w);
}

void UNetModel::prepare_shape(int n, int h, int w) {
    const int div = 1 << depth;
    RFI_REQUIRE(h % div == 0 && w % div == 0,
                "forward: H and W must be multiples of 2^depth (" + std::to_string(div) +
                    "), as the reference's pool/up-conv/cat chain requires; got " +
                    std::to_string(h) + "x" + std::to_string(w));
    if (n == pN && h == pH && w == pW && !bufs.empty()) return;
    ctx->activate();
    const int D = depth;
    if (bufs.empty()) {
        auto mk = [&](std::vector<int>& v) { v.assign(D + 1, -1); for (int l = 1; l <= D; ++l) v[l] = new_buf(); };
        mk(encY1); mk(encY2); mk(concat); mk(pool); mk(decY1); mk(decY2);
        mk(gA); mk(gB); mk(dconcat); mk(dpool); mk(gAe); mk(gBe);
        bottY1 = new_buf(); bottY2 = new_buf(); gBottA = new_buf(); gBottB = new_buf();
        logits = new_buf(); dlogits = new_buf(); probs = new_buf();
        x_stage = new_buf(); x_stage2 = new_buf(); x_pad = new_buf(); out_stage = new_buf();
        ws_red = new_buf(); ws_slab = new_buf(); lab_stage = new_buf();
    }
    size_t slab_need = 0, red_need = 0;
    auto upd_red = [&](size_t f) { if (f > red_need) red_need = f; };
    for (int l = 1; l <= D; ++l) {
        const size_t M = (size_t)n * (h >> (l - 1)) * (w >> (l - 1));
        const size_t C = (size_t)feat << (l - 1);
        for (int i : {decY1[l], decY2[l], gA[l], gB[l]}) bufs[i].ensure(ctx, M * C);
        if (!planesP && !resnet_encoder) for (int i : {gAe[l], gBe[l]}) bufs[i].ensure(ctx, M * C);
        if (!resnet_encoder) for (int i : {encY1[l], encY2[l]}) bufs[i].ensure(ctx, M * C);
        bufs[concat[l]].ensure(ctx, M * 2 * C);
        bufs[dconcat[l]].ensure(ctx, M * 2 * C);
        if (!resnet_encoder || l == D) {
            bufs[pool[l]].ensure(ctx, M / 4 * C);
            bufs[dpool[l]].ensure(ctx, M / 4 * C);
        }
    }
    {
        const size_t M = (size_t)n * (h >> D) * (w >> D);
        const size_t C = (size_t)feat << D;
        for (int i : {bottY1, bottY2, gBottA, gBottB}) bufs[i].ensure(ctx, M * C);
    }
    const size_t M1 = (size_t)n * h * w;
    bufs[logits].ensure(ctx, M1 * out_ch);
    bufs[dlogits].ensure(ctx, M1 * out_ch);
    bufs[probs].ensure(ctx, M1 * out_ch);
    bufs[x_stage].ensure(ctx, M1 * in_ch);
    bufs[x_stage2].ensure(ctx, M1 * in_ch);
    bufs[x_pad].ensure(ctx, M1 * convs[0].cin_p);
    bufs[out_stage].ensure(ctx, M1 * out_ch);
    bufs[lab_stage].ensure(ctx, (M1 + 3) / 4 + 4);
    size_t cmax = (size_t)feat << depth;
    upd_red(bn_stats_ws_floats((int)cmax));
    upd_red(bn_bwd_ws_floats(M1, (int)cmax));
    upd_red(head_bwd_ws_floats(M1, feat, out_ch) + bn_bwd_ws_floats(M1, feat));
    upd_red(channel_sum_ws_floats(M1, (int)cmax));
    upd_red(loss_ws_doubles(M1) * 2);
    upd_red(sumsq_ws_doubles(n_flat) * 2);
    bufs[ws_red].ensure(ctx, red_need + 16);
    auto conv_geom = [&](int ci, int& H, int& W) {
        H = h >> (convs[ci].level - 1);
        W = w >> (convs[ci].level - 1);
    };
    for (size_t ci = 0; ci < convs.size(); ++ci) {
        int H, W;
        conv_geom((int)ci, H, W);
        WgradArgs a;
        a.N = n; a.H = H; a.W = W; a.Hx = H; a.Wx = W;
        a.Cx = convs[ci].cin_p; a.Cy = convs[ci].cout;
        a.R = 3; a.S = 1; a.pad = 1;
        if (convs[ci].stride == 2) { a.Cx *= 4; a.R = 2; }
        if (convs[ci].R == 1) { a.R = 1; a.pad = 0; }
        a.xop.pstride = a.Cx; a.yop.pstride = a.Cy;
        a.tap_stride = (int64_t)a.Cx * a.Cy;
        a.bf16x3 = true;
        slab_need = std::max(slab_need, wgrad_slab_floats(a, IMPL_AUTO));
    }
    for (int k = 0; k < D; ++k) {
        const int l = D - k;
        WgradArgs a;
        a.N = n; a.H = h >> l; a.W = w >> l; a.Hx = a.H * 2; a.Wx = a.W * 2;
        a.Cx = ups[k].cout; a.Cy = ups[k].cin;
        a.xop.pstride = 2 * ups[k].cout; a.yop.pstride = a.Cy;
        a.R = 2; a.S = 2; a.pad = 0;
// ... 229 lines not shown
            hd.push_back(WBDesc{params + u.w_off, ws_pool + o, 1, 4 * u.cout, u.cin, {u.cin, 0}, P});
            ws_by_w[params + u.w_off] = ws_pool + o;
            o += ef + 32;
            hdg.push_back(WBDesc{u.wd, ws_pool + o, 4, u.cin, u.cout, {u.cout, 0}, P});
            ws_by_w[u.wd] = ws_pool + o;
            o += ed + 32;
            ws_bytes_fwd += 2.0 * ef + 4.0 * 4 * u.cin * u.cout;
            ws_bytes += 2.0 * ed + 4.0 * 4 * u.cin * u.cout;
        }
        ws_n_fwd = (int)hd.size();
        ws_bytes += ws_bytes_fwd;
        hd.insert(hd.end(), hdg.begin(), hdg.end());
        ws_n = (int)hd.size();
        ws_descs = ctx->upload_table(hd.data(), hd.size() * sizeof(WBDesc));
    }
    const WBDesc* descs = static_cast<const WBDesc*>(ws_descs);
    if (which == 0 && ws_n) launch_weights_to_wb(ctx, descs, ws_n, ws_bytes);
    if (which == 1 && ws_n_fwd) launch_weights_to_wb(ctx, descs, ws_n_fwd, ws_bytes_fwd);
    if (which == 2 && ws_n > ws_n_fwd) launch_weights_to_wb(ctx, descs + ws_n_fwd, ws_n - ws_n_fwd, ws_bytes - ws_bytes_fwd);
}

ConvArgs rfi_model::conv_same(View x, InXform xf, Shape s, int R, int pad, int cin, int cout, const float* w, const float* w3,
                              const float* bias, float* y) const {
    ConvArgs a;
    a.x = x;
    a.N = s.N; a.H = s.H; a.W = s.W; a.Hin = s.H; a.Win = s.W;
    a.Cin = cin; a.Cout = cout;
    set_filters(a, w, w3);
    a.bias = bias;
    a.y = MutView{y, cout};
    a.Hout = s.H; a.Wout = s.W;
    a.R = R; a.S = 1; a.pad = pad;
    a.xf = xf;
    return a;
}

WgradArgs rfi_model::wgrad_same(View x, InXform xf_x, const float* dy, Shape s, int R, int pad, int cin, int cout,
                                float* dw) const {
    WgradArgs wa;
    wa.xop = x;
    wa.yop = View{dy, cout};
    wa.xf_x = xf_x;
    wa.N = s.N; wa.H = s.H; wa.W = s.W; wa.Hx = s.H; wa.Wx = s.W;
    wa.Cx = cin; wa.Cy = cout;
    wa.R = R; wa.S = 1; wa.pad = pad;
    wa.dw = dw;
    wa.tap_stride = (int64_t)cin * cout;
    wa.sy = cin; wa.sx = 1;
    set_wgrad(wa);
    return wa;
}

void rfi_model::conv_bn(ConvBN& c, View in, InXform xf, Shape s, const float* w, const float* w3, int R, int pad, int cin,
                        float* Y, bool train, double flops) {
    ConvArgs a = conv_same(in, xf, s, R, pad, cin, c.cout, w, w3, c.has_bias ? params + c.b_off : nullptr, Y);
    a.algo_flops = flops;
    float* ws = buf(ws_red);
    if (train) {
        a.stats = reinterpret_cast<double*>(ws);
        a.stats_max_records = (int)(bn_stats_ws_floats(c.cout) / ((size_t)c.cout * 4));
    }
    launch_conv(ctx, a);
    const int64_t M = (int64_t)s.N * s.H * s.W;
    if (train) {
        if (a.stats_records == 0) launch_bn_stats(ctx, Y, M, c.cout, ws);
        launch_bn_finalize(ctx, ws, M, c.cout, params + c.g_off, params + c.be_off, c.running_mean(), c.running_var(),
                           c.ema_repeats, c.mean(), c.invstd(), c.scale(), c.shift(), nullptr, a.stats_records);
        c.nbt += c.ema_repeats;
    } else {
        launch_bn_eval_coeffs(ctx, c.cout, params + c.g_off, params + c.be_off, c.running_mean(), c.running_var(),
                              c.scale(), c.shift());
    }
}

ConvArgs rfi_model::convt_args(const UpConv& u, View x, InXform xf, Shape s) const {
    ConvArgs a;
    a.x = x;
    a.N = s.N; a.H = s.H; a.W = s.W; a.Hin = s.H; a.Win = s.W;
    a.Cin = u.cin; a.Cout = u.cout;
    set_filters(a, params + u.w_off, u.w3);
    a.bias = params + u.b_off;
    a.Hout = 2 * s.H; a.Wout = 2 * s.W;
    a.osy = 2; a.osx = 2;
    a.R = 1; a.S = 1; a.pad = 0;
    a.zgroups = 4;
    a.xf = xf;
    return a;
}

void rfi_model::convt_backward(const UpConv& u, View dup, View x, InXform xf, Shape s, float* dx) {
    WgradArgs wa;
    wa.xop = dup;
    wa.yop = x;
    wa.xf_y = xf;
    wa.N = s.N; wa.H = s.H; wa.W = s.W; wa.Hx = 2 * s.H; wa.Wx = 2 * s.W;
    wa.Cx = u.cout; wa.Cy = u.cin;
    wa.R = 2; wa.S = 2; wa.pad = 0;
    wa.dw = grads + u.w_off;
    wa.tap_stride = (int64_t)u.cin * u.cout;
    wa.sy = 1; wa.sx = u.cin;
    set_wgrad(wa);
    wgrad_on_side(wa, nullptr);
    ConvArgs a;
    a.x = dup;
    a.N = s.N; a.H = s.H; a.W = s.W; a.Hin = 2 * s.H; a.Win = 2 * s.W;
    a.Cin = u.cout; a.Cout = u.cin;
    set_filters(a, u.wd, u.wd3);
    a.y = MutView{dx, u.cin};
    a.Hout = s.H; a.Wout = s.W;
    a.R = 2; a.S = 2; a.pad = 0;
    launch_conv(ctx, a);
}


rfi::View rfi_model::network_input(const float* x_dev, int n, int h, int w) {
    const int cp = convs[0].cin_p;
    if (cp == in_ch) return View{x_dev, in_ch};
    launch_pad_channels(ctx, x_dev, (int64_t)n * h * w, in_ch, cp, buf(x_pad));
    return View{buf(x_pad), cp};
}

void rfi_model::forward(const float* x_dev, int n, int h, int w, bool train_mode) {
    prepare(n, h, w);
    refresh_dgrad_weights();
    forward_pass(x_dev, n, h, w, train_mode);
}

void UNetModel::forward_pass(const float* x_dev, int n, int h, int w, bool train_mode) {
    if (planesP) return forward_planes(x_dev, n, h, w, train_mode);
    const int D = depth, IB = i_bott;
    auto run_conv_bn = [&](ConvBN& c, View in, InXform xf, Shape s, float* Y) {
        conv_bn(c, in, xf, s, params + c.w_off, c.w3, 3, 1, c.cin_p, Y, train_mode, 2.0 * s.N * s.H * s.W * 9.0 * c.cin * c.cout);
    };
    View cur = network_input(x_dev, n, h, w);
    if (resnet_encoder) cur = forward_resnet_encoder(cur, n, h, w, train_mode);
    else for (int l = 1; l <= D; ++l) {
        Shape s{n, h >> (l - 1), w >> (l - 1)};
        ConvBN& c1 = convs[2 * (l - 1)];
        ConvBN& c2 = convs[2 * (l - 1) + 1];
        run_conv_bn(c1, cur, InXform{}, s, buf(encY1[l]));
        if (l == 1) side_rebuild_wd();
        run_conv_bn(c2, View{buf(encY1[l]), c1.cout}, bn_xf(c1), s, buf(encY2[l]));
        launch_bn_relu_pool(ctx, buf(encY2[l]), s.N, s.H, s.W, c2.cout, c2.scale(), c2.shift(),
                            MutView{buf(concat[l]) + c2.cout, 2 * c2.cout}, buf(pool[l]), act_slope);
        cur = View{buf(pool[l]), c2.cout};
    }
    {
        Shape s{n, h >> D, w >> D};
        ConvBN& c1 = convs[IB];
        ConvBN& c2 = convs[IB + 1];
        run_conv_bn(c1, cur, InXform{}, s, buf(bottY1));
        run_conv_bn(c2, View{buf(bottY1), c1.cout}, bn_xf(c1), s, buf(bottY2));
    }
    const float* prevY = buf(bottY2);
    ConvBN* prevBN = &convs[IB + 1];
    for (int l = D; l >= 1; --l) {
        const int k = D - l;
        UpConv& u = ups[k];
        Shape sin{n, h >> l, w >> l};
        Shape s{n, h >> (l - 1), w >> (l - 1)};
        ConvArgs a = convt_args(u, View{prevY, u.cin}, bn_xf(*prevBN), sin);
        a.y = MutView{buf(concat[l]), 2 * u.cout};
        launch_conv(ctx, a);
        ConvBN& c1 = convs[IB + 2 + 2 * k];
        ConvBN& c2 = convs[IB + 2 + 2 * k + 1];
        run_conv_bn(c1, View{buf(concat[l]), 2 * u.cout}, InXform{}, s, buf(decY1[l]));
        run_conv_bn(c2, View{buf(decY1[l]), c1.cout}, bn_xf(c1), s, buf(decY2[l]));
        prevY = buf(decY2[l]);
        prevBN = &c2;
    }
    const int64_t M1 = (int64_t)n * h * w;
    launch_head_fwd(ctx, prevY, M1, feat, prevBN->scale(), prevBN->shift(), params + head_w_off,
                    params + head_b_off, out_ch, buf(logits), act_slope);
    if (head_sigmoid) launch_sigmoid_fwd(ctx, buf(logits), M1 * out_ch, buf(probs));
}

void rfi_model::loss_forward(const uint8_t* labels_dev, int n, int h, int w) {
    RFI_REQUIRE(out_ch == 1, "loss: the reference's BCE+dice step is defined for out_channels == 1");
    const int64_t cnt = (int64_t)n * h * w * out_scale * out_scale;
    if (loss_kind == 1) {
        launch_focal_reduce(ctx, buf(head_sigmoid ? probs : logits), labels_dev, cnt, focal_alpha, focal_gamma,
                            reinterpret_cast<double*>(buf(ws_red)), d_scalars);
        return;
    }
    launch_loss_reduce(ctx, buf(head_sigmoid ? probs : logits), labels_dev, cnt,
                       reinterpret_cast<double*>(buf(ws_red)), d_sums, d_scalars);
}

void rfi_model::side_begin() {
    if (!ctx->overlap) return;
    RFI_CHECK_HIP(hipEventRecord(ctx->fork_ev, ctx->main_stream));
    RFI_CHECK_HIP(hipStreamWaitEvent(ctx->side_stream, ctx->fork_ev, 0));
    ctx->stream = ctx->side_stream;
}
hipEvent_t rfi_model::next_fork_event() {
    static const bool off = getenv("RFI_NO_STOP_EVENTS") != nullptr;
    if (!ctx->overlap || off) return nullptr;
    if (ctx->fork_ring_used == ctx->fork_ring.size()) {
        hipEvent_t e;
        RFI_CHECK_HIP(hipEventCreateWithFlags(&e, hipEventDisableTiming));
        ctx->fork_ring.push_back(e);
    }
    return ctx->fork_ring[ctx->fork_ring_used++];
}
void rfi_model::side_begin_after(hipEvent_t producer_done) {
    if (!producer_done) return side_begin();
    if (!ctx->overlap) return;
    RFI_CHECK_HIP(hipStreamWaitEvent(ctx->side_stream, producer_done, 0));
    ctx->stream = ctx->side_stream;
}
void rfi_model::side_end() {
    if (!ctx->overlap) return;
    const int ring = (int)ctx->side_done.size();
    RFI_CHECK_HIP(hipEventRecord(ctx->side_done[side_seq % ring], ctx->side_stream));
    ctx->stream = ctx->main_stream;
    if (side_bound > 0 && side_seq >= side_bound)
        RFI_CHECK_HIP(hipStreamWaitEvent(ctx->main_stream, ctx->side_done[(side_seq - side_bound) % ring], 0));
    ++side_seq;
}
// ... 22 lines not shown

static hipEvent_t bucket_event(rfi_ctx* ctx) {
    if (ctx->bucket_ev_used == ctx->bucket_ev.size()) {
        hipEvent_t e;
        RFI_CHECK_HIP(hipEventCreateWithFlags(&e, hipEventDisableTiming));
        ctx->bucket_ev.push_back(e);
    }
    return ctx->bucket_ev[ctx->bucket_ev_used++];
}
void rfi_model::bucket_ready(size_t lo, size_t hi) {
    if (!exchange_in_backward || !ctx->exchange_active() || hi <= lo) return;
    static const bool no_buckets = getenv("RFI_NO_BUCKETS") != nullptr;
    const char* mf = getenv("RFI_BUCKET_MIN_FLOATS");
    const size_t min_floats = mf ? (size_t)atoll(mf) : (size_t)1 << 20;
    if (pend_hi > pend_lo) {
        RFI_REQUIRE(hi == pend_lo || lo == pend_hi, "bucket_ready: buckets must be adjacent");
        pend_lo = std::min(pend_lo, lo);
        pend_hi = std::max(pend_hi, hi);
    } else {
        pend_lo = lo;
        pend_hi = hi;
    }
    if (no_buckets) return;
    if (pend_hi - pend_lo < min_floats && pend_lo != 0) return;
    flush_bucket();
}
void rfi_model::flush_bucket() {
    if (pend_hi <= pend_lo) return;
    const size_t lo = pend_lo, hi = pend_hi;
    pend_lo = pend_hi = 0;
    hipEvent_t em = bucket_event(ctx);
    RFI_CHECK_HIP(hipEventRecord(em, ctx->main_stream));
    RFI_CHECK_HIP(hipStreamWaitEvent(ctx->comm_stream, em, 0));
    if (ctx->overlap) {
        hipEvent_t es = bucket_event(ctx);
        RFI_CHECK_HIP(hipEventRecord(es, ctx->side_stream));
        RFI_CHECK_HIP(hipStreamWaitEvent(ctx->comm_stream, es, 0));
    }
    comm_bucket_allreduce(ctx, grads + lo, (int64_t)(hi - lo));
}
void rfi_model::exchange_join() {
    if (!ctx->exchange_active()) return;
    flush_bucket();
    hipEvent_t e = bucket_event(ctx);
    RFI_CHECK_HIP(hipEventRecord(e, ctx->comm_stream));
    RFI_CHECK_HIP(hipStreamWaitEvent(ctx->main_stream, e, 0));
    ctx->bucket_ev_used = 0;
}

namespace {

void backward_conv_bn(UNetModel* m, ConvBN& c, float* dA, const float* Y, View in, InXform in_xf,
                      Shape s, float* dx, int have_records,
                      const float* head_dl = nullptr, const float* head_w = nullptr) {
    rfi_ctx* ctx = m->ctx;
    const int64_t M = (int64_t)s.N * s.H * s.W;
    float* ws = m->buf(m->ws_red);
    if (have_records > 0)
        launch_bn_bwd_finalize_records(ctx, ws, have_records, M, c.cout, c.c1(), c.c2(), m->grads + c.g_off,
                                       m->grads + c.be_off);
    else
        launch_bn_bwd_reduce(ctx, dA, Y, M, c.cout, c.scale(), c.shift(), c.mean(), c.invstd(), ws, c.c1(),
                             c.c2(), m->grads + c.g_off, m->grads + c.be_off, m->act_slope);
    const hipEvent_t dy_done = dx ? nullptr : m->next_fork_event();
    launch_bn_bwd_apply(ctx, dA, Y, M, c.cout, c.scale(), c.shift(), c.mean(), c.invstd(),
                        m->params + c.g_off, c.c1(), c.c2(), m->dbias_deferred ? m->dbias_pool + c.dbias_rec_off : ws,
                        m->grads + c.b_off, m->act_slope, nullptr, 0, 0, dy_done, !m->dbias_deferred, head_dl, head_w);
    WgradArgs wa = m->wgrad_same(in, in_xf, dA, s, 3, 1, c.cin_p, c.cout, m->grads + c.w_off);
    wa.algo_flops = 2.0 * s.N * s.H * s.W * 9.0 * c.cin * c.cout;
    if (!dx) {
        m->wgrad_on_side(wa, dy_done);
        return;
    }
    ConvArgs a = m->conv_same(View{dA, c.cout}, InXform{}, s, 3, 1, c.cout, c.cin, c.wd, c.wd3, nullptr, dx);
    a.done = m->next_fork_event();
    launch_conv(ctx, a);
    m->wgrad_on_side(wa, a.done_used ? a.done : nullptr, !a.done_used);
}

}

void rfi_model::wgrad_on_side(const rfi::WgradArgs& wa, hipEvent_t after, bool after_everything) {
    SideScope side(this, after_everything ? nullptr : after);
    launch_wgrad(ctx, wa);
    side.end();
}

void rfi_model::backward(const float* x_dev, const uint8_t* labels_dev, int n, int h, int w) {
    join_pending_side();
    backward_pass(x_dev, labels_dev, n, h, w);
}

void UNetModel::backward_pass(const float* x_dev, const uint8_t* labels_dev, int n, int h, int w) {
    const int D = depth, IB = i_bott;
    const int64_t M1 = (int64_t)n * h * w;
    refresh_dgrad_weights();
    wait_wd();
    if (planesP) return backward_planes(x_dev, labels_dev, n, h, w);
    side_bound = resnet_encoder ? 2 : 0;
    dbias_deferred = !resnet_encoder && dbias_pool && !ctx->exchange_active();
    if (loss_kind == 1)
        launch_focal_bwd(ctx, buf(head_sigmoid ? probs : logits), labels_dev, M1, focal_alpha, focal_gamma, buf(dlogits));
    else
        launch_loss_bwd(ctx, buf(head_sigmoid ? probs : logits), labels_dev, M1, d_sums, buf(dlogits));
    if (head_sigmoid) launch_sigmoid_bwd(ctx, buf(probs), M1 * out_ch, buf(dlogits));
    int head_records = 0;
    bool head_skip = out_ch == 1;
    {
        ConvBN& last = convs[IB + 2 + 2 * (D - 1) + 1];
        const bool hdefer = dbias_deferred && head_fin_deferred;
        head_records = launch_head_bwd(ctx, buf(decY2[1]), M1, feat, last.scale(), last.shift(), params + head_w_off,
                                       out_ch, buf(dlogits), buf(gA[1]),
                                       hdefer ? dbias_pool + head_rec_off : buf(ws_red) + bn_bwd_ws_floats(M1, feat),
                                       grads + head_w_off, grads + head_b_off, act_slope, last.mean(), last.invstd(),
                                       buf(ws_red), nullptr, &head_skip, !hdefer);
    }
    for (int l = 1; l <= D; ++l) {
        const int k = D - l;
        Shape s{n, h >> (l - 1), w >> (l - 1)};
        Shape sin{n, h >> l, w >> l};
        ConvBN& c1 = convs[IB + 2 + 2 * k];
        ConvBN& c2 = convs[IB + 2 + 2 * k + 1];
        UpConv& u = ups[k];
        const bool from_head = l == 1 && head_skip;
        backward_conv_bn(this, c2, buf(gA[l]), buf(decY2[l]), View{buf(decY1[l]), c1.cout}, bn_xf(c1), s,
                         buf(gB[l]), l == 1 ? head_records : 0, from_head ? buf(dlogits) : nullptr,
                         from_head ? params + head_w_off : nullptr);
        backward_conv_bn(this, c1, buf(gB[l]), buf(decY1[l]), View{buf(concat[l]), 2 * u.cout}, InXform{}, s,
                         buf(dconcat[l]), 0);
        const float* prevY = (l == D) ? buf(bottY2) : buf(decY2[l + 1]);
        ConvBN& prevBN = (l == D) ? convs[IB + 1] : convs[IB + 2 + 2 * (k - 1) + 1];
        View dUp{buf(dconcat[l]), 2 * u.cout};
        {
            const bool defer = dbias_deferred && u.cout % 4 == 0;
            launch_channel_sum(ctx, dUp, (int64_t)s.N * s.H * s.W, u.cout, defer ? dbias_pool + u.dbias_rec_off : buf(ws_red),
                               grads + u.b_off, !defer);
        }
        convt_backward(u, dUp, View{prevY, u.cin}, bn_xf(prevBN), sin, (l == D) ? buf(gBottA) : buf(gA[l + 1]));
        bucket_ready(u.w_off, l == 1 ? n_flat : ups[k + 1].w_off);
    }
    {
        Shape s{n, h >> D, w >> D};
        ConvBN& c1 = convs[IB];
        ConvBN& c2 = convs[IB + 1];
        backward_conv_bn(this, c2, buf(gBottA), buf(bottY2), View{buf(bottY1), c1.cout}, bn_xf(c1), s, buf(gBottB), 0);
        backward_conv_bn(this, c1, buf(gBottB), buf(bottY1), View{buf(pool[D]), c1.cin}, InXform{}, s, buf(dpool[D]), 0);
        bucket_ready(c1.w_off, ups[0].w_off);
    }
    if (resnet_encoder) {
        backward_resnet_encoder(x_dev, n, h, w);
        side_join();
        return;
    }
    for (int l = D; l >= 1; --l) {
        Shape s{n, h >> (l - 1), w >> (l - 1)};
        ConvBN& c1 = convs[2 * (l - 1)];
        ConvBN& c2 = convs[2 * (l - 1) + 1];
        const std::vector<int>& gA = this->gAe;
        const std::vector<int>& gB = this->gBe;
        int have = launch_pool_bwd_merge_sums(ctx, buf(encY2[l]), s.N, s.H, s.W, c2.cout, c2.scale(), c2.shift(), c2.mean(),
                                              c2.invstd(), View{buf(dconcat[l]) + c2.cout, 2 * c2.cout}, buf(dpool[l]),
                                              buf(gA[l]), act_slope, buf(ws_red));
        if (!have)
            launch_pool_bwd_merge(ctx, buf(encY2[l]), s.N, s.H, s.W, c2.cout, c2.scale(), c2.shift(),
                                  View{buf(dconcat[l]) + c2.cout, 2 * c2.cout}, buf(dpool[l]), buf(gA[l]), act_slope);
        backward_conv_bn(this, c2, buf(gA[l]), buf(encY2[l]), View{buf(encY1[l]), c1.cout}, bn_xf(c1), s, buf(gB[l]), have);
        View in = (l == 1) ? (c1.cin_p == in_ch ? View{x_dev, in_ch} : View{buf(x_pad), c1.cin_p})
                           : View{buf(pool[l - 1]), c1.cin};
        backward_conv_bn(this, c1, buf(gB[l]), buf(encY1[l]), in, InXform{}, s,
                         (l == 1) ? nullptr : buf(dpool[l - 1]), 0);
        bucket_ready(c1.w_off, convs[l == D ? IB : 2 * l].w_off);
    }
    if (dbias_deferred) launch_finish_channel_sums_batched(ctx, static_cast<const FinishSumDesc*>(dbias_descs), dbias_n, dbias_max_c);
    side_join();
    side_bound = 2;
}

void rfi_model::apply(const rfi_hyper& hp, float grad_scale) {
    join_pending_side();
    double* ws = reinterpret_cast<double*>(buf(ws_red));
    launch_sumsq(ctx, grads, (int64_t)n_flat, ws, d_sums + 4);
    adam_step += 1;
    AdamArgs a;
    a.p = params; a.g = grads; a.m = adam_m; a.v = adam_v; a.n = (int64_t)n_flat;
    a.beta2 = (float)hp.beta2; a.eps = (float)hp.eps; a.wd = (float)hp.weight_decay;
    a.max_norm = (float)hp.max_grad_norm; a.grad_scale = grad_scale;
    a.one_minus_beta1 = (float)(1.0 - hp.beta1);
    a.one_minus_beta2 = (float)(1.0 - hp.beta2);
    a.neg_step = (float)(-(hp.lr / (1.0 - std::pow(hp.beta1, (double)adam_step))));
    a.bc2_sqrt = (float)std::sqrt(1.0 - std::pow(hp.beta2, (double)adam_step));
    a.sumsq = d_sums + 4;
    a.norm_out = d_scalars + 1;
    launch_adam(ctx, a);
    wd_dirty = true;
    x3_fresh = false;
}

void rfi_model::set_compute_dtype(int dtype) {
    arith = dtype == 1 || dtype == 4 ? Arith::BF16 : dtype == 2 || dtype == 3 ? Arith::X3 : Arith::F32;
}
void UNetModel::set_compute_dtype(int dtype) {
    rfi_model::set_compute_dtype(dtype);
    if (resnet_encoder) set_planes(dtype == 1 && feat % 16 == 0 ? 1 : 0);
    else set_planes(dtype == 1 ? 1 : (dtype == 3 ? 3 : 0));
}

void rfi_model::debug_tensor(const std::string&, const std::string&, int, bool, const float*&, size_t&) {
    throw Error("debug_tensor: this model exposes only logits / dlogits / chan (and the decoder tensors of the ResNet-encoder U-Net)");
}
void UNetModel::debug_tensor(const std::string& name, const std::string& base, int idx, bool to_host, const float*& src, size_t& n) {
    if (resnet_encoder && (base == "encY1" || base == "encY2" || base == "pool" || base == "dpool"))
        return rfi_model::debug_tensor(name, base, idx, to_host, src, n);
    RFI_REQUIRE(!(y16_flow && planesP == 1 && (base == "encY1" || base == "encY2" || base == "decY1" || base == "bottY1" ||
                                               (base == "decY2" && idx == 1))),
                "debug_tensor: this conv output is stored as bfloat16 in the bfloat16 compute mode");
    RFI_REQUIRE(!(g16_flow && planesP == 1 && (base == "gB" || base == "dpool" || base == "gBottB" || base == "gA")),
                "debug_tensor: this gradient tensor is stored as bfloat16 in the bfloat16 compute mode");
    RFI_REQUIRE(!(convt_planes && planesP == 1 && (base == "decY2" || base == "bottY2" || base == "gBottA")),
                "debug_tensor: with the transposed convs on the plane kernels this tensor is stored as bfloat16");
    const int D = depth;
    auto level = [&](const std::vector<int>& v, size_t chmul) {
        RFI_REQUIRE(idx >= 1 && idx <= D, "debug_tensor: level out of range");
        const size_t M = (size_t)pN * (pH >> (idx - 1)) * (pW >> (idx - 1));
        src = buf(v[idx]);
        n = M * ((size_t)feat << (idx - 1)) * chmul;
    };
    const size_t Mb = (size_t)pN * (pH >> D) * (pW >> D), Cb = (size_t)feat << D;
    if (base == "encY1") level(encY1, 1);
    else if (base == "encY2") level(encY2, 1);
    else if (base == "decY1") level(decY1, 1);
    else if (base == "decY2") level(decY2, 1);
    else if (base == "gA") level(!planesP && !resnet_encoder ? gAe : gA, 1);
    else if (base == "gB") level(!planesP && !resnet_encoder ? gBe : gB, 1);
    else if (base == "concat") level(concat, 2);
    else if (base == "dconcat") {
        level(dconcat, 2);
        if (convt_planes && planesP == 1 && to_host) {
            const PlaneBuf& g = pl[g16cat[idx]];
            launch_planes_to_f32(ctx, g.p, g.pstride, (int64_t)(n / ((size_t)2 * (feat << (idx - 1)))), 2 * (feat << (idx - 1)), 1,
                                 buf(dconcat[idx]), 2 * (feat << (idx - 1)));
        }
    }
    else if (base == "pool") { level(pool, 1); n /= 4; }
    else if (base == "dpool") { level(dpool, 1); n /= 4; }
    else if (base == "bottY1") { src = buf(bottY1); n = Mb * Cb; }
    else if (base == "bottY2") { src = buf(bottY2); n = Mb * Cb; }
    else if (base == "gBottA") { src = buf(gBottA); n = Mb * Cb; }
    else if (base == "gBottB") { src = buf(gBottB); n = Mb * Cb; }
    else throw Error("debug_tensor: unknown tensor " + name);
}

void UNetModel::algorithmic_flops(int n, int h, int w, double& fwd, double& step) const {
    double f = 0, stem = 0;
    for (size_t ci = 0; ci < convs.size(); ++ci) {
        const int lvl = convs[ci].level, R = convs[ci].R;
        const double M = (double)n * (h >> (lvl - 1)) * (w >> (lvl - 1));
        const double fl = 2.0 * M * R * R * convs[ci].cin * convs[ci].cout;
        f += fl;
        if (ci == 0) stem = fl;
    }
    for (int k = 0; k < depth; ++k) {
        const int l = depth - k;
        const double M = (double)n * (h >> l) * (w >> l);
        f += 2.0 * M * 4.0 * ups[k].cin * ups[k].cout;
    }
    f += 2.0 * n * h * w * (double)feat * out_ch;
    fwd = f;
    step = 3.0 * f - stem;
}
```

rfi_toolbox_amd/csrc/model.hpp:

```cpp
#pragma once
#include "planes.hpp"

namespace rfi {

struct DevBuf {
    rfi_ctx* ctx = nullptr;
    float* p = nullptr;
    size_t n = 0;
    void ensure(rfi_ctx* c, size_t floats);
    void free();
};

struct PlaneBuf {
    rfi_ctx* ctx = nullptr;
    bf16_t* p = nullptr;
    size_t elems = 0;
    int64_t pstride = 0;
    int nchunks = 0;
    void ensure(rfi_ctx* c, int64_t pixels, int C, int P);
    void free();
};

struct ConvBN {
    std::string conv_name, bn_name;
// ... 160 lines not shown
    int relayout_n = 0;
    int64_t relayout_tiles = 0;
    double relayout_bytes = 0;

    int pN = 0, pH = 0, pW = 0;
    std::vector<rfi::DevBuf> bufs;
    int logits = -1, dlogits = -1;
    int x_stage = -1, x_stage2 = -1, x_pad = -1, out_stage = -1, ws_red = -1, ws_slab = -1, lab_stage = -1;
    int gx = -1;
    bool ext_dlogits = false;
    double* d_sums = nullptr;
    float* d_scalars = nullptr;
    float last_loss = 0, last_norm = 0;

    rfi_model(int in, int out, int f, int d) : in_ch(in), out_ch(out), feat(f), depth(d) {}
    virtual ~rfi_model();
    virtual void build() = 0;
    void prepare(int n, int h, int w);
    virtual void prepare_shape(int n, int h, int w) = 0;
    void forward(const float* x_dev, int n, int h, int w, bool train_mode);
    virtual void forward_pass(const float* x_dev, int n, int h, int w, bool train_mode) = 0;
    void loss_forward(const uint8_t* labels_dev, int n, int h, int w);
    void backward(const float* x_dev, const uint8_t* labels_dev, int n, int h, int w);
    virtual void backward_pass(const float* x_dev, const uint8_t* labels_dev, int n, int h, int w) = 0;
    void apply(const rfi_hyper& hp, float grad_scale);
    virtual void algorithmic_flops(int n, int h, int w, double& fwd, double& step) const = 0;
    virtual void set_compute_dtype(int dtype);
    virtual void debug_tensor(const std::string& name, const std::string& base, int idx, bool to_host, const float*& src, size_t& n);

    size_t chan_floats = 0, wd_floats = 0;
    int add_conv(rfi::ConvBN c);
    void add_up(const std::string& name, int cin, int cout);
    void add_head(const std::string& name, int cin);
    void alloc_state();
    void reset_channel_state();
    const rfi::Entry& entry(const char* name) const;
    void init_params(uint64_t seed);
    void load_entry(const rfi::Entry& e, const void* host, size_t bytes);
    void store_entry(const rfi::Entry& e, void* host, size_t bytes);
    void store_flat(const float* flat, const rfi::Entry& e, void* host, size_t bytes);
    void load_adam(const rfi::Entry& e, const void* host_m, const void* host_v, size_t bytes);
    float* buf(int i) { return bufs[i].p; }
    int new_buf() { bufs.emplace_back(); return (int)bufs.size() - 1; }
    rfi::View network_input(const float* x_dev, int n, int h, int w);
    void refresh_dgrad_weights();
    virtual bool wd_split_ok() const { return false; }
    virtual void refresh_model_weights(int which) {}

    rfi::ConvArgs conv_same(rfi::View x, rfi::InXform xf, rfi::Shape s, int R, int pad, int cin, int cout, const float* w,
                            const float* w3, const float* bias, float* y) const;
    rfi::WgradArgs wgrad_same(rfi::View x, rfi::InXform xf_x, const float* dy, rfi::Shape s, int R, int pad, int cin, int cout,
                              float* dw) const;
    void conv_bn(rfi::ConvBN& c, rfi::View in, rfi::InXform xf, rfi::Shape s, const float* w, const float* w3, int R, int pad,
                 int cin, float* Y, bool train, double flops);
    rfi::ConvArgs convt_args(const rfi::UpConv& u, rfi::View x, rfi::InXform xf, rfi::Shape s) const;
    void convt_backward(const rfi::UpConv& u, rfi::View dup, rfi::View x, rfi::InXform xf, rfi::Shape s, float* dx);

    int side_seq = 0;
    int side_bound = 2;
    void side_begin();
    hipEvent_t next_fork_event();
    void side_begin_after(hipEvent_t producer_done);
    void side_end();
    void side_join();
    hipEvent_t lazy_ev = nullptr;
    bool lazy_pending = false;
    void side_join_lazy();
    void join_pending_side();
    void wgrad_on_side(const rfi::WgradArgs& wa, hipEvent_t after, bool after_everything = false);
    bool exchange_in_backward = false;
    void bucket_ready(size_t lo, size_t hi);
    size_t pend_lo = 0, pend_hi = 0;
    void flush_bucket();
    void exchange_join();
};

namespace rfi {
struct SideScope {
    rfi_model* m;
    bool ended = false;
    explicit SideScope(rfi_model* model, hipEvent_t after = nullptr) : m(model) { m->side_begin_after(after); }
    void end() { m->side_end(); ended = true; }
    ~SideScope() { if (!ended) m->ctx->stream = m->ctx->main_stream; }
};
}

struct UNetModel : rfi_model {
    const bool resnet_encoder;
    UNetModel(int in, int out, int f, int d, bool resnet) : rfi_model(in, out, f, d), resnet_encoder(resnet) {
        x3_skips_ws_layers = !resnet;
    }
    ~UNetModel() override;
    void build() override;
    void prepare_shape(int n, int h, int w) override;
    void forward_pass(const float* x_dev, int n, int h, int w, bool train_mode) override;
    void backward_pass(const float* x_dev, const uint8_t* labels_dev, int n, int h, int w) override;
    void algorithmic_flops(int n, int h, int w, double& fwd, double& step) const override;
    void set_compute_dtype(int dtype) override;
    void debug_tensor(const std::string& name, const std::string& base, int idx, bool to_host, const float*& src, size_t& n) override;
    bool wd_split_ok() const override;
    void refresh_model_weights(int which) override;

    int i_bott = 0;
    float act_slope = 0.0f;
    rfi::InXform bn_xf(const rfi::ConvBN& c) const { return rfi::act_of(c, act_slope); }
    std::vector<int> encY1, encY2, concat, pool, decY1, decY2, gA, gB, dconcat, dpool;
    std::vector<int> gAe, gBe;
    int bottY1 = -1, bottY2 = -1, gBottA = -1, gBottB = -1;
    float* dbias_pool = nullptr;
    void* dbias_descs = nullptr;
    int dbias_n = 0, dbias_max_c = 0;
    bool dbias_deferred = false;
    size_t head_rec_off = 0;
    bool head_fin_deferred = false;

    struct ResBlock {
        int c1 = -1, c2 = -1, cd = -1;
        int stride = 1, cin = 0, cout = 0, level = 1;
        int Y1 = -1, Y2 = -1, Yd = -1, xs = -1, A = -1;
    };
    std::vector<ResBlock> blocks;
    int rs_stemY = -1, rs_a0 = -1, rs_g0 = -1, rs_g1 = -1, rs_dX = -1, rs_dS = -1, rs_dW = -1, rs_dzd = -1;
    int rs_dz[2] = {-1, -1}, rs_dA1[2] = {-1, -1};
    float* rs_ones = nullptr;
    float* rs_zeros = nullptr;
    float* rs_wpool = nullptr;
    void build_resnet();
    void prepare_resnet(int n, int h, int w);
    void refresh_resnet_weights();
    rfi::View forward_resnet_encoder(rfi::View x, int n, int h, int w, bool train_mode);
    void backward_resnet_encoder(const float* x_dev, int n, int h, int w);

    std::vector<rfi::PlaneBuf> pl;
    std::vector<int> pA1e, pSkip, pPool, pUp, pA1d, pdYa, pdYb, pdYaE, pdYbE, upf;
    int pXin = -1, pA1b = -1, pdYbottA = -1, pdYbottB = -1;
    bool y16_flow = false;
    std::vector<int> yE1, yE2, yD1;
    int yB1 = -1, yD2top = -1;
    bool g16_flow = false;
    std::vector<int> g16A, g16B, g16pool;
    int g16BottB = -1;
    struct ResPlanes {
        int Y1 = -1, Y2 = -1, Yd = -1, A1 = -1, A = -1, dY1 = -1, dY2 = -1, dYd = -1;
        rfi::bf16_t* wBcls[4] = {nullptr, nullptr, nullptr, nullptr};
        float* cls = nullptr;
    };
    std::vector<ResPlanes> rpb;
    int rpStemY = -1, rpA0 = -1, rpdY0 = -1, rp_dA1 = -1, rp_dX = -1;
    int rp_dz[2] = {-1, -1};
    float* rs_cls_pool = nullptr;
    bool resnet_planes() const { return resnet_encoder && planesP == 1; }
    void forward_resnet_planes(rfi::PlaneSeg& cur, int n, int h, int w, bool train_mode);
    void backward_resnet_planes(int n, int h, int w);
    bool convt_planes = false;
    rfi::YRef skip_grad(int l, int C) {
        if (convt_planes) return rfi::YRef(pl[g16cat[l]].p + C, pl[g16cat[l]].pstride);
        return rfi::YRef(buf(dconcat[l]) + C, (int64_t)2 * C);
    }
    std::vector<int> yD2, pUpIn, g16cat;
    int yB2 = -1, g16BottA = -1;
// ... 77 lines not shown
```

rfi_toolbox_amd/csrc/wgrad_mfma.hip:

```cpp
#include <algorithm>

#include "planes.hpp"

namespace rfi {

void launch_wgrad_direct(rfi_ctx* ctx, const WgradArgs& a);
size_t wgrad_direct_slab_floats(const WgradArgs& a);
bool wgrad_split_eligible(const WgradArgs& a);
size_t wgrad_split_slab_floats(const WgradArgs& a);
void launch_wgrad_split(rfi_ctx* ctx, const WgradArgs& a);

namespace {

typedef float f32x4 __attribute__((ext_vector_type(4)));
typedef float f32x16 __attribute__((ext_vector_type(16)));
typedef float f32x2 __attribute__((ext_vector_type(2)));
typedef __bf16 bf16x2 __attribute__((ext_vector_type(2)));
typedef short s16x4 __attribute__((ext_vector_type(4)));
typedef unsigned u32x2 __attribute__((ext_vector_type(2)));

typedef __bf16 bf16x8 __attribute__((ext_vector_type(8)));
typedef unsigned u32x4 __attribute__((ext_vector_type(4)));
struct Split3 { bf16x8 h, m, l; };
__device__ __forceinline__ unsigned cvt_pair(float a, float b) {
// ... 335 lines not shown
}

enum { SEL_PLAN = 0, SEL_LAUNCH = 1 };

template <int R, int S, int TH, int TW>
Plan select(rfi_ctx* ctx, const WgradArgs& a, int what, int cus) {
    const bool y64 = a.Cy > 32, x64 = a.Cx > 32;
#define RFI_WG(BY_, BX_)                                                        \
    do {                                                                        \
        if (what == SEL_LAUNCH) launch_cfg<R, S, BY_, BX_, TH, TW>(ctx, a);     \
        return plan_cfg<R, S, BY_, BX_, TH, TW>(a, cus);                        \
    } while (0)
    if (y64 && x64) RFI_WG(64, 64);
    if (y64) RFI_WG(64, 32);
    if (x64) RFI_WG(32, 64);
    RFI_WG(32, 32);
#undef RFI_WG
}

bool wgrad_mfma_eligible(const WgradArgs& a) {
    if (a.Cx % 4 || a.Cy % 4 || a.xop.pstride % 4 || a.yop.pstride % 4) return false;
    if ((reinterpret_cast<uintptr_t>(a.xop.p) & 15) || (reinterpret_cast<uintptr_t>(a.yop.p) & 15)) return false;
    return (a.R == 3 && a.S == 1 && a.pad == 1) || (a.R == 2 && a.S == 2 && a.pad == 0);
}

Plan dispatch(rfi_ctx* ctx, const WgradArgs& a, int what, int cus) {
    if (a.R == 3) {
        const bool splits_pixels = !(a.Cy > 32 && a.Cx > 32);
        if (splits_pixels && a.H >= 16) return select<3, 1, 16, 8>(ctx, a, what, cus);
        return select<3, 1, 8, 8>(ctx, a, what, cus);
    }
    return select<2, 2, 4, 8>(ctx, a, what, cus);
}

}

size_t wgrad_slab_floats(const WgradArgs& a, int impl) {
    size_t need = wgrad_direct_slab_floats(a);
    if ((impl == IMPL_PLANES_X3 || impl == IMPL_PLANES_BF16) && a.R == 3 && a.S == 1)
        return std::max(need, pwgrad_slab_floats_f32(a));
    if (impl == IMPL_MFMA_BF16 || impl == IMPL_MFMA_BF16X3) impl = IMPL_MFMA;
    if (impl != IMPL_DIRECT && wgrad_split_eligible(a)) need = std::max(need, wgrad_split_slab_floats(a));
    if (impl != IMPL_DIRECT) need = std::max(need, wgrad_ws_slab_floats(a));
    if (impl != IMPL_DIRECT && wgrad_mfma_eligible(a)) {
        const Plan p = dispatch(nullptr, a, SEL_PLAN, 256);
        const size_t m = (size_t)p.nsplit * p.wp * p.slab_stride;
        if (m > need) need = m;
    }
    return need;
}

void launch_wgrad(rfi_ctx* ctx, const WgradArgs& a_in, int impl) {
    WgradArgs a = a_in;
    if (impl == IMPL_PLANES_X3 || impl == IMPL_PLANES_BF16) {
        RFI_REQUIRE(a.R == 3 && a.S == 1, "wgrad: the plane kernel covers 3x3 stride-1 convolutions");
        launch_pwgrad_from_f32(ctx, a, impl == IMPL_PLANES_X3 ? 3 : 1);
        return;
    }
    if (impl == IMPL_MFMA_BF16) {
        a.bf16 = true;
        impl = IMPL_MFMA;
    }
    if (impl == IMPL_MFMA_BF16X3) {
        a.bf16x3 = true;
        impl = IMPL_MFMA;
    }
    RFI_REQUIRE(a.N > 0 && a.H > 0 && a.W > 0 && a.Cx > 0 && a.Cy > 0, "wgrad: empty shape");
    RFI_REQUIRE((int64_t)a.N * a.Hx * a.Wx * a.xop.pstride < (int64_t)1 << 31 &&
                    (int64_t)a.N * a.H * a.W * a.yop.pstride < (int64_t)1 << 31,
                "wgrad: tensor too large for 32-bit element offsets");
    const bool ok = wgrad_mfma_eligible(a) || ((a.bf16 || a.bf16x3) && wgrad_split_eligible(a));
    if (impl == IMPL_MFMA) RFI_REQUIRE(ok, "wgrad: shape/alignment not eligible for the MFMA kernel");
    if (impl == IMPL_DIRECT || !ok) {
        launch_wgrad_direct(ctx, a);
        return;
    }
    if (a.bf16x3 && wgrad_stem_eligible(a)) {
        launch_wgrad_stem(ctx, a);
        return;
    }
    if ((a.bf16x3 || a.bf16) && wgrad_ws_eligible(a) && (wgrad_split_eligible(a) || (a.R == 2 && a.S == 2))) {
        launch_wgrad_ws(ctx, a);
        return;
    }
    const bool only_split = (a.R == 2 && a.S == 1) || a.R == 1;
    if (only_split) RFI_REQUIRE((a.bf16 || a.bf16x3) && wgrad_split_eligible(a),
                                "wgrad: 2x2 stride-1 and 1x1 weight gradients need the bf16 or 3 x bf16 arithmetic and 4-channel alignment");
    if ((a.bf16x3 || only_split) && wgrad_split_eligible(a)) {
        launch_wgrad_split(ctx, a);
        return;
    }
    dispatch(ctx, a, SEL_LAUNCH, 256);
}

}
```

rfi_toolbox_amd/csrc/wgrad_ws.hip:

```cpp
#include <algorithm>
#include <cstdio>
#include <vector>

#include "ws_common.hpp"

namespace rfi {
namespace {

using namespace ws;
typedef short s16x4 __attribute__((ext_vector_type(4)));
typedef __attribute__((address_space(3))) s16x4 lds_s16x4;

struct WWsDev {
    WgradArgs a;
    int nsplit;
    int64_t slab_stride;
    unsigned x_bytes, y_bytes;
    unsigned long long* stamps;
};

template <int R, int BYB, int BXB, int TH, int TW, int P, int ST = 1, int PWV = 4>
struct WWCfg {
    static constexpr int NTAP = R * R;
    static constexpr int BM = TH * TW;
// ... 11 lines not shown
    static constexpr int RED_BYTES = (WP > 1) ? BLOCKS * TC * 4096 : 0;
    static constexpr int TR_FLOATS = 32 * 33;
    static constexpr int EPI_BYTES = RED_BYTES + 4 * TR_FLOATS * 4;
    static constexpr int LDS_BYTES = 2 * STAGE > EPI_BYTES ? 2 * STAGE : EPI_BYTES;
    static_assert(BLOCKS == 1 || BLOCKS == 2 || BLOCKS == 4, "1, 2 or 4 channel blocks");
    static_assert(BM % 16 == 0 && KS % WP == 0 && TW % 4 == 0, "tile must split into k-steps of 16 pixels");
    static_assert(NPT % YQ == 0 && NPT % XQ == 0, "a producer thread keeps one channel group for all its items");
    static_assert(PWV == 4 || PWV == 8, "4 consumer waves + 4 or 8 producer waves");
    static_assert(ST == 1 || (ST == 2 && R == 2), "stride 2: the transposed conv's 2x2 taps");
    static_assert(LDS_BYTES <= 160 * 1024, "LDS budget");
};

template <int P>
__device__ __forceinline__ f32x16 mma(const bf16x8 (&a)[P], const bf16x8 (&b)[P], f32x16 acc) {
    if constexpr (P == 3) return mma3(a, b, acc);
    else return __builtin_amdgcn_mfma_f32_32x32x16_bf16(a[0], b[0], acc, 0, 0, 0);
}
__device__ __forceinline__ bf16x8 tr_frag(const unsigned char* p0, const unsigned char* p1) {
    const s16x4 lo = __builtin_amdgcn_ds_read_tr16_b64_v4i16((lds_s16x4*)p0);
    const s16x4 hi = __builtin_amdgcn_ds_read_tr16_b64_v4i16((lds_s16x4*)p1);
    return __builtin_bit_cast(bf16x8, __builtin_shufflevector(lo, hi, 0, 1, 2, 3, 4, 5, 6, 7));
}

__device__ __forceinline__ void lds_barrier() { asm volatile("s_waitcnt lgkmcnt(0)\n\ts_barrier" ::: "memory"); }

template <int R, int BYB, int BXB, int TH, int TW, int P, int XM, int ST = 1, int PWV = 4>
__global__ __launch_bounds__(256 + 64 * PWV) void wgrad_ws_kernel(WWsDev d) {
    using C = WWCfg<R, BYB, BXB, TH, TW, P, ST, PWV>;
    const WgradArgs& a = d.a;
    extern __shared__ __attribute__((aligned(16))) unsigned char smem[];
#ifdef RFI_DIAG_STAMPS
    unsigned long long st_[4] = {0, 0, 0, 0};
#endif
    const int tid = threadIdx.x;
    const int lane = tid & 63, wave = __builtin_amdgcn_readfirstlane(tid >> 6);
    const int cy0 = blockIdx.y * BYB * 32, cx0 = blockIdx.z * BXB * 32;
    const int split = blockIdx.x;
    const int tiles_x = (a.W + TW - 1) / TW, tiles_y = (a.H + TH - 1) / TH;
    const int ntiles = a.N * tiles_y * tiles_x;
    const int my_tiles = split < ntiles ? (ntiles - split + d.nsplit - 1) / d.nsplit : 0;

    if (wave >= 4) {
        const int ptid = tid - 256;
        constexpr int YSTEP = C::NPT / C::YQ, XSTEP = C::NPT / C::XQ;
        const int yq = ptid % C::YQ, xq = ptid % C::XQ;
        const int ypix0 = ptid / C::YQ, xpix0 = ptid / C::XQ;
        const int cyq = cy0 + yq * 4, cxq = cx0 + xq * 4;
        const bool y_cok = cyq < a.Cy, x_cok = cxq < a.Cx;
        f32x4 ysc = {1.f, 1.f, 1.f, 1.f}, ysh = {0.f, 0.f, 0.f, 0.f}, xsc = ysc, xsh = ysh;
        if (a.xf_y.scale && y_cok) {
            ysc = *reinterpret_cast<const f32x4*>(a.xf_y.scale + cyq);
            ysh = *reinterpret_cast<const f32x4*>(a.xf_y.shift + cyq);
        }
        if (a.xf_x.scale && x_cok) {
            xsc = *reinterpret_cast<const f32x4*>(a.xf_x.scale + cxq);
            xsh = *reinterpret_cast<const f32x4*>(a.xf_x.shift + cxq);
        }
        const __amdgpu_buffer_rsrc_t yrs = __builtin_amdgcn_make_buffer_rsrc(const_cast<float*>(a.yop.p), 0, (int)d.y_bytes, 0x00020000);
        const __amdgpu_buffer_rsrc_t xrs = __builtin_amdgcn_make_buffer_rsrc(const_cast<float*>(a.xop.p), 0, (int)d.x_bytes, 0x00020000);
        constexpr unsigned NOWHERE = 0x81000000u, OUTSIDE = 0x80000000u;
        unsigned y_rel[C::Y_ITEMS], x_rel[C::X_ITEMS];
        int y_dyx[C::Y_ITEMS], x_dyx[C::X_ITEMS];
#pragma unroll
        for (int it = 0; it < C::Y_ITEMS; ++it) {
            const int pix = ypix0 + it * YSTEP, dy = pix / TW, dx = pix % TW;
            y_rel[it] = (pix < C::BM && y_cok) ? (unsigned)((dy * a.W + dx) * a.yop.pstride + cyq) * 4u : NOWHERE;
            y_dyx[it] = pix < C::BM ? (dy << 16) | dx : 0x7fff7fff;
        }
#pragma unroll
        for (int it = 0; it < C::X_ITEMS; ++it) {
            const int pix = xpix0 + it * XSTEP, dy = pix / C::HW, dx = pix % C::HW;
            x_rel[it] = (pix < C::HP && x_cok) ? (unsigned)((dy * a.Wx + dx) * a.xop.pstride + cxq) * 4u : NOWHERE;
            x_dyx[it] = pix < C::HP ? (dy << 16) | dx : 0x7fff7fff;
        }
        const int y_lds = (yq >> 3) * (C::BM * C::ROW) + (yq & 7) * 8 + ypix0 * C::ROW;
        const int x_lds = (xq >> 3) * (C::HP * C::ROW) + (xq & 7) * 8 + xpix0 * C::ROW;
        struct TileRegs {
            u32x4 yreg[C::Y_ITEMS], xreg[C::X_ITEMS];
            unsigned yvalid = ~0u, xvalid = ~0u;
            bool yfull = true, xin = true;
        };
        TileRegs tr0;
        auto load_tile = [&](int tile, TileRegs& tr) {
            u32x4 (&yreg)[C::Y_ITEMS] = tr.yreg;
            u32x4 (&xreg)[C::X_ITEMS] = tr.xreg;
            unsigned &yvalid = tr.yvalid, &xvalid = tr.xvalid;
            bool &yfull = tr.yfull, &xin = tr.xin;
            const int tx_i = tile % tiles_x, ty_i = (tile / tiles_x) % tiles_y, n = tile / (tiles_x * tiles_y);
            const int oy0 = ty_i * TH, ox0 = tx_i * TW;
            const int iy0 = oy0 * ST - a.pad, ix0 = ox0 * ST - a.pad;
            const unsigned ybase = (unsigned)(((n * a.H + oy0) * a.W + ox0) * a.yop.pstride) * 4u;
            const unsigned xbase = (unsigned)(((n * a.Hx + iy0) * a.Wx + ix0) * a.xop.pstride) * 4u;
            yfull = oy0 + TH <= a.H && ox0 + TW <= a.W;
            xin = iy0 >= 0 && ix0 >= 0 && iy0 + C::HH <= a.Hx && ix0 + C::HW <= a.Wx;
            if (yfull) {
                yvalid = ~0u;
#pragma unroll
                for (int it = 0; it < C::Y_ITEMS; ++it) yreg[it] = __builtin_amdgcn_raw_buffer_load_b128(yrs, ybase + y_rel[it], 0, 0);
            } else {
                yvalid = 0;
#pragma unroll
                for (int it = 0; it < C::Y_ITEMS; ++it) {
                    const bool ok = oy0 + (y_dyx[it] >> 16) < a.H && ox0 + (y_dyx[it] & 0xffff) < a.W;
                    yreg[it] = __builtin_amdgcn_raw_buffer_load_b128(yrs, ok ? ybase + y_rel[it] : OUTSIDE, 0, 0);
                    yvalid |= (ok ? 1u : 0u) << it;
                }
            }
            if (xin) {
                xvalid = ~0u;
#pragma unroll
                for (int it = 0; it < C::X_ITEMS; ++it) xreg[it] = __builtin_amdgcn_raw_buffer_load_b128(xrs, xbase + x_rel[it], 0, 0);
            } else {
                xvalid = 0;
#pragma unroll
                for (int it = 0; it < C::X_ITEMS; ++it) {
                    const bool ok = (unsigned)(iy0 + (x_dyx[it] >> 16)) < (unsigned)a.Hx && (unsigned)(ix0 + (x_dyx[it] & 0xffff)) < (unsigned)a.Wx;
                    xreg[it] = __builtin_amdgcn_raw_buffer_load_b128(xrs, ok ? xbase + x_rel[it] : OUTSIDE, 0, 0);
                    xvalid |= (ok ? 1u : 0u) << it;
                }
            }
        };
        auto put = [&](f32x4 v, unsigned char* dst) {
            if constexpr (P == 3) {
                unsigned h0, m0, l0, h1, m1, l1;
                split_pair(v.x, v.y, h0, m0, l0);
                split_pair(v.z, v.w, h1, m1, l1);
                *reinterpret_cast<u32x2*>(dst) = u32x2{h0, h1};
                *reinterpret_cast<u32x2*>(dst + 64) = u32x2{m0, m1};
                *reinterpret_cast<u32x2*>(dst + 128) = u32x2{l0, l1};
            } else {
                *reinterpret_cast<u32x2*>(dst) = u32x2{cvt_pair(v.x, v.y), cvt_pair(v.z, v.w)};
            }
        };
        auto xform = [&](f32x4 v, const f32x4& sc, const f32x4& sh, const InXform& xf, auto mask_c, unsigned valid) {
            const unsigned m = (unsigned)__builtin_amdgcn_sbfe((int)valid, 0, 1);
#pragma unroll
            for (int e = 0; e < 4; ++e) {
                float t = v[e] * sc[e] + sh[e];
                if constexpr (XM == 1) {
                    asm("v_max_f32 %0, 0, %1" : "=v"(t) : "v"(t));
                } else {
                    if (xf.relu) {
                        const float u = t * xf.slope;
                        asm("v_max_f32 %0, %1, %2" : "=v"(t) : "v"(t), "v"(u));
                    }
                }
                if constexpr (decltype(mask_c)::value) t = __builtin_bit_cast(float, __builtin_bit_cast(unsigned, t) & m);
                v[e] = t;
            }
            return v;
        };
        auto store_tile = [&](int buf, const TileRegs& tr) {
            const u32x4 (&yreg)[C::Y_ITEMS] = tr.yreg;
            const u32x4 (&xreg)[C::X_ITEMS] = tr.xreg;
            const unsigned yvalid = tr.yvalid, xvalid = tr.xvalid;
            const bool xin = tr.xin;
            unsigned char* const sY = smem + buf * C::STAGE + y_lds;
            unsigned char* const sX = smem + buf * C::STAGE + C::Y_BYTES + x_lds;
            const bool do_y = XM == 2 && a.xf_y.scale != nullptr, do_x = XM == 1 || (XM == 2 && a.xf_x.scale != nullptr);
#pragma unroll
            for (int it = 0; it < C::Y_ITEMS; ++it) {
                f32x4 v = __builtin_bit_cast(f32x4, yreg[it]);
                if (do_y) v = xform(v, ysc, ysh, a.xf_y, std::true_type{}, yvalid >> it);
                if (it * YSTEP + YSTEP <= C::BM || ypix0 + it * YSTEP < C::BM) put(v, sY + it * YSTEP * C::ROW);
            }
            if (do_x && !xin) {
#pragma unroll
                for (int it = 0; it < C::X_ITEMS; ++it) {
                    const f32x4 v = xform(__builtin_bit_cast(f32x4, xreg[it]), xsc, xsh, a.xf_x, std::true_type{}, xvalid >> it);
                    if (it * XSTEP + XSTEP <= C::HP || xpix0 + it * XSTEP < C::HP) put(v, sX + it * XSTEP * C::ROW);
                }
            } else {
#pragma unroll
                for (int it = 0; it < C::X_ITEMS; ++it) {
                    f32x4 v = __builtin_bit_cast(f32x4, xreg[it]);
                    if (do_x) v = xform(v, xsc, xsh, a.xf_x, std::false_type{}, 0u);
                    if (it * XSTEP + XSTEP <= C::HP || xpix0 + it * XSTEP < C::HP) put(v, sX + it * XSTEP * C::ROW);
                }
            }
        };
        auto phase = [&](int k, TileRegs& tr) {
            WS_T(t0);
            if (k + 1 < my_tiles) {
                store_tile((k + 1) & 1, tr);
                if (k + 2 < my_tiles) load_tile(split + (k + 2) * d.nsplit, tr);
                asm volatile("s_waitcnt lgkmcnt(0)" ::: "memory");
            }
            WS_T(t1);
            wg_barrier();
            WS_T(t2);
            WS_ACC(0, t0, t1);
            WS_ACC(1, t1, t2);
        };
        load_tile(split, tr0);
        for (int k = -1; k < my_tiles; ++k) phase(k, tr0);
#ifdef RFI_DIAG_STAMPS
        if (d.stamps && lane == 0 && (PWV == 4 || (wave >= 8 && wave < 12))) {
            unsigned long long* o = d.stamps + ((size_t)((blockIdx.z * gridDim.y + blockIdx.y) * gridDim.x + blockIdx.x) * 8 + (PWV == 4 ? wave : wave - 4)) * 8;
            o[0] = st_[0]; o[1] = st_[1]; o[2] = (unsigned long long)my_tiles;
        }
#endif
    } else {
        const int blk = wave % C::BLOCKS, ps = wave / C::BLOCKS;
        const int by = blk / BXB, bx = blk % BXB;
        const int ll = lane & 15, q = ll >> 2, pc = ll & 3, gq = lane >> 4;
        const int lane_off = (gq & 1) * 32 + pc * 8;
        const int kh = gq >> 1;
        auto xpix = [&](int t) { return ST * ((t / TW) * C::HW + (t % TW)); };
        f32x16 acc[C::NTAP];
#pragma unroll
        for (int t = 0; t < C::NTAP; ++t)
#pragma unroll
            for (int r = 0; r < 16; ++r) acc[t][r] = 0.0f;
        WS_T(tp0);
        wg_barrier();
        WS_T(tp1);
        for (int k = 0; k < my_tiles; ++k) {
            WS_T(t0);
            const unsigned char* const sY = smem + (k & 1) * C::STAGE;
// ... 98 lines not shown
#pragma unroll
                for (int r = 0; r < 16; ++r) {
                    const int cy = cy0 + by * 32 + (r & 3) + 8 * (r >> 2) + 4 * lh;
                    if (cy < a.Cy && cx < a.Cx)
                        slab[(int64_t)tap * a.tap_stride + (int64_t)cy * a.sy + (int64_t)cx * a.sx] = acc[tap][r];
                }
            }
        }
#ifdef RFI_DIAG_STAMPS
        asm volatile("s_waitcnt vmcnt(0)" ::: "memory");
        WS_T(tp4);
        if (d.stamps && lane == 0) {
            unsigned long long* o = d.stamps + ((size_t)((blockIdx.z * gridDim.y + blockIdx.y) * gridDim.x + blockIdx.x) * 8 + wave) * 8;
            o[0] = st_[0]; o[1] = st_[1]; o[2] = (unsigned long long)my_tiles;
            o[3] = tp1 - tp0; o[4] = tp2 - tp1; o[5] = tp3 - tp2; o[6] = tp4 - tp3;
        }
#endif
    }
}

struct Plan { int nsplit; int64_t slab_stride; };

template <int R, int BYB, int BXB, int TH, int TW>
Plan plan_cfg(const WgradArgs& a) {
    const int ntiles = a.N * (int)cdiv(a.H, TH) * (int)cdiv(a.W, TW);
    const int chunks = (int)cdiv(a.Cy, 32 * BYB) * (int)cdiv(a.Cx, 32 * BXB);
    int nsplit = (int)cdiv(256, chunks);
    if (nsplit > ntiles) nsplit = ntiles;
    if (nsplit < 1) nsplit = 1;
    return Plan{nsplit, (int64_t)R * R * a.tap_stride};
}

template <int R, int BYB, int BXB, int TH, int TW, int P, int XM, int ST = 1, int PWV = 4>
void launch_cfg(rfi_ctx* ctx, const WgradArgs& a) {
    using C = WWCfg<R, BYB, BXB, TH, TW, P, ST, PWV>;
    const Plan p = plan_cfg<R, BYB, BXB, TH, TW>(a);
    RFI_REQUIRE(a.slab && a.slab_floats >= (size_t)p.nsplit * p.slab_stride, "wgrad_ws: slab workspace too small");
    WWsDev d{a, p.nsplit, p.slab_stride, (unsigned)((int64_t)a.N * a.Hx * a.Wx * a.xop.pstride * 4),
             (unsigned)((int64_t)a.N * a.H * a.W * a.yop.pstride * 4), nullptr};
    dim3 grid(p.nsplit, (unsigned)cdiv(a.Cy, 32 * BYB), (unsigned)cdiv(a.Cx, 32 * BXB));
    const size_t lds = C::LDS_BYTES;
    static PerDeviceOnce attr_once;
    attr_once.run(ctx->device, [&] {
        RFI_CHECK_HIP(hipFuncSetAttribute(reinterpret_cast<const void*>(&wgrad_ws_kernel<R, BYB, BXB, TH, TW, P, XM, ST, PWV>),
                                          hipFuncAttributeMaxDynamicSharedMemorySize, (int)lds));
    });
    {
        const double flops = a.algo_flops >= 0 ? a.algo_flops : 2.0 * a.N * a.H * a.W * (double)a.Cy * a.Cx * R * R;
        std::string label;
        if (ctx->profiling)
            label = "wgrad_ws R" + std::to_string(R) + (ST == 2 ? "s2" : "") + " N" + std::to_string(a.N) + " " + std::to_string(a.H) + "x" +
                    std::to_string(a.W) + " cx" + std::to_string(a.Cx) + " cy" + std::to_string(a.Cy) + " split" +
                    std::to_string(p.nsplit) + (P == 3 ? " 3xbf16" : " bf16") + " b" + std::to_string(BYB) + "x" + std::to_string(BXB) +
                    " t" + std::to_string(TH) + "x" + std::to_string(TW) + " xm" + std::to_string(XM) + (PWV == 8 ? " pw8" : "");
        const double bytes = 4.0 * ((double)a.N * a.Hx * a.Wx * a.Cx + (double)a.N * a.H * a.W * a.Cy + (double)R * R * a.Cx * a.Cy);
        ProfScope ps(ctx, FAM_WGRAD_MFMA, flops, bytes, label);
#ifdef RFI_DIAG_STAMPS
        const size_t nw = (size_t)grid.x * grid.y * grid.z * 8;
        RFI_CHECK_HIP(hipMalloc(reinterpret_cast<void**>(&d.stamps), nw * 64));
        RFI_CHECK_HIP(hipMemsetAsync(d.stamps, 0, nw * 64, ctx->stream));
#endif
        hipLaunchKernelGGL((wgrad_ws_kernel<R, BYB, BXB, TH, TW, P, XM, ST, PWV>), grid, dim3(256 + C::NPT), lds, ctx->stream, d);
        check_launch("wgrad_ws");
#ifdef RFI_DIAG_STAMPS
        std::vector<unsigned long long> hs(nw * 8);
        RFI_CHECK_HIP(hipMemcpyAsync(hs.data(), d.stamps, nw * 64, hipMemcpyDeviceToHost, ctx->stream));
        RFI_CHECK_HIP(hipStreamSynchronize(ctx->stream));
        double c[7] = {0, 0, 0, 0, 0, 0, 0}, pr[7] = {0, 0, 0, 0, 0, 0, 0};
        for (size_t w = 0; w < nw; ++w)
            for (int i = 0; i < 7; ++i) ((w & 7) < 4 ? c : pr)[i] += (double)hs[w * 8 + i];
        std::fprintf(stderr, "[stamps] wgrad_ws<%d,%d,%d,%d,%d> N%d %dx%d cx%d cy%d grid %ux%ux%u tiles/wg %.1f | cycles per tile: consumer mfma %.0f "
                     "barrier %.0f | producer work %.0f barrier %.0f | per consumer wave: prologue %.0f loop %.0f reduce %.0f slab store %.0f\n", R, BYB, BXB, TH, TW, a.N, a.H, a.W, a.Cx, a.Cy, grid.x, grid.y, grid.z,
                     c[2] / (nw / 2), c[0] / c[2], c[1] / c[2], pr[0] / pr[2], pr[1] / pr[2], c[3] / (nw / 2), c[4] / (nw / 2), c[5] / (nw / 2), c[6] / (nw / 2));
        RFI_CHECK_HIP(hipFree(d.stamps));
#endif
    }
    launch_reduce_slabs(ctx, a.slab, p.nsplit, p.slab_stride, a.dw);
}

template <int R>
void select(rfi_ctx* ctx, const WgradArgs& a) {
    const bool y2 = a.Cy > 32, x2 = a.Cx > 32;
    const bool p1 = a.bf16 && !a.bf16x3;
    const bool xm1 = R == 3 && a.xf_x.scale && a.xf_x.relu == 1 && a.xf_x.slope == 0.0f && !a.xf_y.scale;
#define RFI_WW(BYB_, BXB_, TH_, TW_)                                                \
    do {                                                                            \
        if constexpr (R == 3) {                                                     \
            if (xm1) {                                                              \
                if (p1) launch_cfg<R, BYB_, BXB_, TH_, TW_, 1, 1>(ctx, a);          \
                else launch_cfg<R, BYB_, BXB_, TH_, TW_, 3, 1>(ctx, a);             \
                return;                                                             \
            }                                                                       \
        }                                                                           \
        if (p1) launch_cfg<R, BYB_, BXB_, TH_, TW_, 1, 2>(ctx, a);                  \
        else launch_cfg<R, BYB_, BXB_, TH_, TW_, 3, 2>(ctx, a);                     \
        return;                                                                     \
    } while (0)
    if constexpr (R == 1) {
        if (y2 && x2) {
            if (p1) launch_cfg<1, 2, 2, 8, 8, 1, 2, 1, 8>(ctx, a);
            else launch_cfg<1, 2, 2, 8, 8, 3, 2, 1, 8>(ctx, a);
            return;
        }
    } else {
        if (y2 && x2) RFI_WW(2, 2, 8, 8);
    }
    if (y2) RFI_WW(2, 1, 8, 8);
    if (x2) RFI_WW(1, 2, 8, 8);
    if (a.W >= 16) RFI_WW(1, 1, 8, 16);
    RFI_WW(1, 1, 16, 8);
#undef RFI_WW
}

void select_t2(rfi_ctx* ctx, const WgradArgs& a, Plan* plan_only) {
    const bool p1 = a.bf16 && !a.bf16x3;
    const bool y2 = a.Cy > 32, x2 = a.Cx > 32;
#define RFI_WT(BYB_, BXB_, TH_, TW_)                                                       \
    do {                                                                                   \
        if (plan_only) { *plan_only = plan_cfg<2, BYB_, BXB_, TH_, TW_>(a); return; }      \
        if (p1) launch_cfg<2, BYB_, BXB_, TH_, TW_, 1, 2, 2, 8>(ctx, a);                   \
        else launch_cfg<2, BYB_, BXB_, TH_, TW_, 3, 2, 2, 8>(ctx, a);                      \
        return;                                                                            \
    } while (0)
    if (y2 && x2) RFI_WT(2, 2, 4, 8);
    if (y2) RFI_WT(2, 1, 8, 8);
    if (x2) RFI_WT(1, 2, 4, 8);
    RFI_WT(1, 1, 8, 8);
#undef RFI_WT
}

}

bool wgrad_ws_eligible(const WgradArgs& a) {
    if (a.Cx % 4 || a.Cy % 4 || a.xop.pstride % 4 || a.yop.pstride % 4) return false;
    if ((reinterpret_cast<uintptr_t>(a.xop.p) & 15) || (reinterpret_cast<uintptr_t>(a.yop.p) & 15)) return false;
    if ((int64_t)a.N * a.Hx * a.Wx * a.xop.pstride * 4 >= 0x7f000000ll || (int64_t)a.N * a.H * a.W * a.yop.pstride * 4 >= 0x7f000000ll) return false;
    if (((int64_t)a.Wx + 1) * a.xop.pstride * 4 >= (1 << 24)) return false;
    if (a.R == 2 && a.S == 2 && a.pad == 0) {
        return a.Hx == 2 * a.H && a.Wx == 2 * a.W;
    }
    if (a.S != 1) return false;
    return (a.R == 3 && a.pad == 1) || (a.R == 2 && a.pad == 1) || (a.R == 1 && a.pad == 0);
}
size_t wgrad_ws_slab_floats(const WgradArgs& a) {
    if (!(a.R == 2 && a.S == 2) || !wgrad_ws_eligible(a)) return 0;
    Plan p{0, 0};
    select_t2(nullptr, a, &p);
    return (size_t)p.nsplit * p.slab_stride;
}
void launch_wgrad_ws(rfi_ctx* ctx, const WgradArgs& a) {
    RFI_REQUIRE(wgrad_ws_eligible(a) && (a.bf16 || a.bf16x3), "wgrad_ws: shape or arithmetic not eligible");
    if (a.R == 3) select<3>(ctx, a);
    else if (a.R == 2 && a.S == 2) select_t2(ctx, a, nullptr);
    else if (a.R == 2) select<2>(ctx, a);
    else select<1>(ctx, a);
}

}
```

Measured before the change: 9149 patches/s.

## Let conv3x3 forward and wgrad read a concatenated input from two sources

Adds a second-source descriptor so 3x3 convolutions and their weight gradients can read the U-Net decoder's skip and upsampled tensors directly, each with its own BN/ReLU transform, instead of needing a materialised concatenation. The WS forward and wgrad kernels gain a two-source path that switches buffer resource and transform per channel chunk. Ineligible cases fall back to a concat kernel into a temporary buffer. This is meant to remove the concat copy's memory traffic, at the cost of extra per-chunk branching and register use in the kernels.

```diff
diff --git a/include/rfi_hip.h b/include/rfi_hip.h
--- a/include/rfi_hip.h
+++ b/include/rfi_hip.h
@@ -223,16 +223,24 @@
 int rfi_augment_batch(rfi_ctx* ctx, const float* x, int x_mem, const uint8_t* y, int y_mem, int n, int h, int w, int c,
                       const rfi_augment_config* cfg, uint64_t call, float* x_out, uint8_t* y_out);
 
+typedef struct rfi_conv_source2 {
+    const float* x;
+    int c;
+    const float* scale;
+    const float* shift;
+    int relu;
+    float slope;
+} rfi_conv_source2;
 int rfi_op_conv3x3(rfi_ctx* ctx, int impl, const float* x, int n, int h, int w, int cin,
                    const float* w_oihw, const float* bias, int cout,
-                   const float* in_scale, const float* in_shift, int in_relu, float* y);
+                   const float* in_scale, const float* in_shift, int in_relu, float* y, const rfi_conv_source2* second);
 int rfi_op_conv1x1(rfi_ctx* ctx, int impl, const float* x, int n, int h, int w, int cin, const float* w_oihw, const float* bias,
                    int cout, const float* in_scale, const float* in_shift, int in_relu, float* y);
 int rfi_op_conv3x3_dgrad(rfi_ctx* ctx, int impl, const float* dy, int n, int h, int w, int cout,
                          const float* w_oihw, int cin, float* dx);
 int rfi_op_conv3x3_wgrad(rfi_ctx* ctx, int impl, const float* x, const float* dy, int n, int h,
                          int w, int cin, int cout, const float* in_scale, const float* in_shift,
-                         int in_relu, float* dw_oihw);
+                         int in_relu, float* dw_oihw, const rfi_conv_source2* second);
 int rfi_op_conv_s2(rfi_ctx* ctx, int impl, int ksize, const float* x, int n, int h, int w, int cin,
                    const float* w_oihw, int cout, float* y);
 int rfi_op_conv_s2_dgrad(rfi_ctx* ctx, int impl, int ksize, const float* dy, int n, int h, int w, int cout,
@@ -310,7 +318,7 @@
 int rfi_op_fpn_merge_backward(rfi_ctx* ctx, const float* dout, int n, int h, int w, int c, float* dtop);
 int rfi_op_bn_stats(rfi_ctx* ctx, const float* y, int64_t m, int c, float* mean, float* var_biased);
 int rfi_op_bn_relu_pool(rfi_ctx* ctx, const float* y, int n, int h, int w, int c, const float* scale,
-                        const float* shift, float* skip, float* pooled);
+                        const float* shift, float* skip, float* pooled, float slope);
 int rfi_op_pool_bwd_merge(rfi_ctx* ctx, const float* y, int n, int h, int w, int c, const float* scale,
                           const float* shift, const float* dskip, const float* dpool, float* da);
 int rfi_op_bn_relu_backward(rfi_ctx* ctx, const float* y, int64_t m, int c, const float* gamma,
diff --git a/rfi_toolbox_amd/_lib.py b/rfi_toolbox_amd/_lib.py
--- a/rfi_toolbox_amd/_lib.py
+++ b/rfi_toolbox_amd/_lib.py
@@ -49,6 +49,11 @@
 
 class Tiling(C.Structure):
     _fields_ = [("ps", C.c_int32), ("stride", C.c_int32), ("edge", C.c_int32), ("views", C.c_int32)]
+
+
+class ConvSource2(C.Structure):
+    _fields_ = [("x", C.c_void_p), ("c", C.c_int), ("scale", C.c_void_p), ("shift", C.c_void_p), ("relu", C.c_int),
+                ("slope", C.c_float)]
 
 
 class Hyper(C.Structure):
@@ -193,18 +198,18 @@
     "rfi_norm_apply": (_i, [_vp, _vp, _i, _i, _i, _i64, C.c_double, C.c_double, _vp, _vp, _i]),
     "rfi_augment_params": (_i, [C.POINTER(AugmentConfig), C.c_uint64, _i, _i, _i, C.POINTER(C.c_int32), _pd]),
     "rfi_augment_batch": (_i, [_vp, _vp, _i, _vp, _i, _i, _i, _i, _i, C.POINTER(AugmentConfig), C.c_uint64, _vp, _vp]),
-    "rfi_op_conv3x3": (_i, [_vp, _i, _vp, _i, _i, _i, _i, _vp, _vp, _i, _vp, _vp, _i, _vp]),
+    "rfi_op_conv3x3": (_i, [_vp, _i, _vp, _i, _i, _i, _i, _vp, _vp, _i, _vp, _vp, _i, _vp, C.POINTER(ConvSource2)]),
     "rfi_op_conv1x1": (_i, [_vp, _i, _vp, _i, _i, _i, _i, _vp, _vp, _i, _vp, _vp, _i, _vp]),
     "rfi_op_conv_s2": (_i, [_vp, _i, _i, _vp, _i, _i, _i, _i, _vp, _i, _vp]),
     "rfi_op_conv_s2_dgrad": (_i, [_vp, _i, _i, _vp, _i, _i, _i, _i, _vp, _i, _vp]),
     "rfi_op_conv_s2_wgrad": (_i, [_vp, _i, _i, _vp, _vp, _i, _i, _i, _i, _i, _vp]),
     "rfi_op_conv3x3_dgrad": (_i, [_vp, _i, _vp, _i, _i, _i, _i, _vp, _i, _vp]),
-    "rfi_op_conv3x3_wgrad": (_i, [_vp, _i, _vp, _vp, _i, _i, _i, _i, _i, _vp, _vp, _i, _vp]),
+    "rfi_op_conv3x3_wgrad": (_i, [_vp, _i, _vp, _vp, _i, _i, _i, _i, _i, _vp, _vp, _i, _vp, C.POINTER(ConvSource2)]),
     "rfi_op_convt2x2": (_i, [_vp, _i, _vp, _i, _i, _i, _i, _vp, _vp, _i, _vp]),
     "rfi_op_convt2x2_dgrad": (_i, [_vp, _i, _vp, _i, _i, _i, _i, _vp, _i, _vp]),
     "rfi_op_convt2x2_wgrad": (_i, [_vp, _i, _vp, _vp, _i, _i, _i, _i, _i, _vp]),
     "rfi_op_bn_stats": (_i, [_vp, _vp, _i64, _i, _vp, _vp]),
-    "rfi_op_bn_relu_pool": (_i, [_vp, _vp, _i, _i, _i, _i, _vp, _vp, _vp, _vp]),
+    "rfi_op_bn_relu_pool": (_i, [_vp, _vp, _i, _i, _i, _i, _vp, _vp, _vp, _vp, _f]),
     "rfi_op_pool_bwd_merge": (_i, [_vp, _vp, _i, _i, _i, _i, _vp, _vp, _vp, _vp, _vp]),
     "rfi_op_bn_relu_backward": (_i, [_vp, _vp, _i64, _i, _vp, _vp, _vp, _vp, _vp, _vp]),
 }
@@ -217,6 +222,24 @@
 EXPORTED = tuple(_PROTOS)
 
 
+def _optional_tail(name, defaults):
+    fn = getattr(lib, name)
+    need = len(fn.argtypes) - len(defaults)
+
+    def call(*args):
+        if not need <= len(args) <= need + len(defaults):
+            raise TypeError(f"{name} takes {need} to {need + len(defaults)} arguments ({len(args)} given)")
+        return fn(*args, *defaults[len(args) - need:])
+
+    call.argtypes, call.restype, call.__name__ = fn.argtypes, fn.restype, name
+    setattr(lib, name, call)
+
+
+_optional_tail("rfi_op_conv3x3", (None,))
+_optional_tail("rfi_op_conv3x3_wgrad", (None,))
+_optional_tail("rfi_op_bn_relu_pool", (0.0,))
+
+
 class RfiHipError(RuntimeError):
     pass
 
diff --git a/rfi_toolbox_amd/csrc/api_ops.cpp b/rfi_toolbox_amd/csrc/api_ops.cpp
--- a/rfi_toolbox_amd/csrc/api_ops.cpp
+++ b/rfi_toolbox_amd/csrc/api_ops.cpp
@@ -60,12 +60,19 @@
 
 int rfi_op_conv3x3(rfi_ctx* ctx, int impl, const float* x, int n, int h, int w, int cin,
                    const float* w_oihw, const float* bias, int cout, const float* in_scale,
-                   const float* in_shift, int in_relu, float* y) {
+                   const float* in_shift, int in_relu, float* y, const rfi_conv_source2* second) {
     return guarded([&] {
         ctx->activate();
         CallScope s(ctx);
         ConvArgs a;
         a.x = View{x, cin};
+        if (second && second->x) {
+            RFI_REQUIRE(second->c > 0 && second->c < cin, "conv3x3: the second source holds some, not all, of the cin channels");
+            a.x = View{x, cin - second->c};
+            a.x2 = View{second->x, second->c};
+            a.Cin2 = second->c;
+            a.xf2 = InXform{second->scale, second->shift, second->relu, second->slope};
+        }
         a.N = n; a.H = h; a.W = w; a.Hin = h; a.Win = w; a.Cin = cin; a.Cout = cout;
         a.w = upload_lib_weight(ctx, s, w_oihw, (size_t)9 * cin * cout, false, cout, cin, 3);
         a.bias = bias;
@@ -111,12 +118,19 @@
 }
 int rfi_op_conv3x3_wgrad(rfi_ctx* ctx, int impl, const float* x, const float* dy, int n, int h, int w,
                          int cin, int cout, const float* in_scale, const float* in_shift, int in_relu,
-                         float* dw_oihw) {
+                         float* dw_oihw, const rfi_conv_source2* second) {
     return guarded([&] {
         ctx->activate();
         CallScope s(ctx);
         WgradArgs a;
         a.xop = View{x, cin};
+        if (second && second->x) {
+            RFI_REQUIRE(second->c > 0 && second->c < cin, "conv3x3_wgrad: the second source holds some, not all, of the cin channels");
+            a.xop = View{x, cin - second->c};
+            a.xop2 = View{second->x, second->c};
+            a.Cx2 = second->c;
+            a.xf_x2 = InXform{second->scale, second->shift, second->relu, second->slope};
+        }
         a.yop = View{dy, cout};
         a.xf_x = InXform{in_scale, in_shift, in_relu};
         a.N = n; a.H = h; a.W = w; a.Hx = h; a.Wx = w; a.Cx = cin; a.Cy = cout;
@@ -716,10 +730,10 @@
 }
 
 int rfi_op_bn_relu_pool(rfi_ctx* ctx, const float* y, int n, int h, int w, int c, const float* scale,
-                        const float* shift, float* skip, float* pooled) {
-    return guarded([&] {
-        ctx->activate();
-        launch_bn_relu_pool(ctx, y, n, h, w, c, scale, shift, MutView{skip, c}, pooled);
+                        const float* shift, float* skip, float* pooled, float slope) {
+    return guarded([&] {
+        ctx->activate();
+        launch_bn_relu_pool(ctx, y, n, h, w, c, scale, shift, MutView{skip, c}, pooled, slope);
     });
 }
 int rfi_op_pool_bwd_merge(rfi_ctx* ctx, const float* y, int n, int h, int w, int c, const float* scale,
diff --git a/rfi_toolbox_amd/csrc/conv_mfma.hip b/rfi_toolbox_amd/csrc/conv_mfma.hip
--- a/rfi_toolbox_amd/csrc/conv_mfma.hip
+++ b/rfi_toolbox_amd/csrc/conv_mfma.hip
@@ -648,6 +648,22 @@
 }
 
 void launch_conv(rfi_ctx* ctx, ConvArgs& a, int impl) {
+    if (a.x2.p) {
+        const bool in_place = (impl == IMPL_WS_X3 || (impl == IMPL_AUTO && a.bf16x3 && a.wB3)) && conv_ws_eligible(a);
+        if (!in_place) {
+            RFI_REQUIRE(a.R == 3 && a.S == 1 && a.zgroups == 1 && a.Cin2 > 0 && a.Cin2 < a.Cin && !a.xf.scale,
+                        "conv: a second source needs a 3x3 stride-1 conv whose first source has no transform");
+            CallScope sc(ctx);
+            float* cat = sc.temp<float>((size_t)a.N * a.Hin * a.Win * a.Cin);
+            launch_concat_sources(ctx, a.x, a.Cin - a.Cin2, a.x2, a.Cin2, a.xf2, a.N, a.Hin, a.Win, cat);
+            ConvArgs b = a;
+            b.x = View{cat, a.Cin};
+            b.x2 = View{}; b.Cin2 = 0; b.xf2 = InXform{};
+            launch_conv(ctx, b, impl);
+            a.stats = b.stats; a.stats_records = b.stats_records; a.done_used = b.done_used;
+            return;
+        }
+    }
     if (impl == IMPL_PLANES_X3 || impl == IMPL_PLANES_BF16) {
         RFI_REQUIRE(a.R == 3 && a.S == 1 && a.zgroups == 1, "conv: the plane kernels cover 3x3 stride-1 convolutions");
         a.planes = impl == IMPL_PLANES_X3 ? 3 : 1;
diff --git a/rfi_toolbox_amd/csrc/conv_ws.hip b/rfi_toolbox_amd/csrc/conv_ws.hip
--- a/rfi_toolbox_amd/csrc/conv_ws.hip
+++ b/rfi_toolbox_amd/csrc/conv_ws.hip
@@ -18,6 +18,11 @@
     const float* scale;
     const float* shift;
     float slope;
+    const float* x2;
+    const float* scale2;
+    const float* shift2;
+    float slope2;
+    int nkc_a, xf_a, xf_b;
     int N, H, W, Cin, Cout;
     const bf16_t* wB;
     int nkc, ncb;
@@ -51,7 +56,7 @@
 };
 
 
-template <int TB, int TH, int TW, int NTL, int XF, bool ADB, int P>
+template <int TB, int TH, int TW, int NTL, int XF, bool ADB, int P, bool TWO = false>
 __global__ __launch_bounds__(512) void conv_ws_kernel(WsDev d) {
     using C = WsCfg<TB, TH, TW, NTL, ADB, P>;
     constexpr int RB = ROWB<P>;
@@ -99,6 +104,9 @@
         const int ptid = tid - 256, pw = wave - 4;
         const unsigned q4b = (unsigned)(ptid & 3) * 16u;
         const __amdgpu_buffer_rsrc_t xrs = __builtin_amdgcn_make_buffer_rsrc(const_cast<float*>(d.x), 0, (int)d.x_bytes, 0x00020000);
+        const __amdgpu_buffer_rsrc_t xrs2 = __builtin_amdgcn_make_buffer_rsrc(const_cast<float*>(TWO ? d.x2 : d.x), 0, (int)d.x_bytes, 0x00020000);
+        bool ld_xf = true;
+        float ld_slope = d.slope;
         unsigned h_rc[C::HALO_ITEMS];
 #pragma unroll
         for (int it = 0; it < C::HALO_ITEMS; ++it) {
@@ -121,7 +129,27 @@
         u32x4 raw[C::HALO_ITEMS];
         f32x4 screg = {1.f, 1.f, 1.f, 1.f}, shreg = {0.f, 0.f, 0.f, 0.f};
         unsigned pl[C::HALO_ITEMS][2 * P];
-        auto issue_loads = [&](int c0) {
+        auto issue_loads = [&](int ch) {
+            if constexpr (TWO) {
+                const bool second = ch >= d.nkc_a;
+                const int c0 = (second ? ch - d.nkc_a : ch) * 16;
+                ld_xf = (second ? d.xf_b : d.xf_a) != 0;
+                ld_slope = second ? d.slope2 : d.slope;
+                if (ld_xf) {
+                    screg = *reinterpret_cast<const f32x4*>((second ? d.scale2 : d.scale) + c0 + (ptid & 3) * 4);
+                    shreg = *reinterpret_cast<const f32x4*>((second ? d.shift2 : d.shift) + c0 + (ptid & 3) * 4);
+                }
+                __builtin_amdgcn_sched_barrier(0);
+                if (second) {
+#pragma unroll
+                    for (int it = 0; it < C::HALO_ITEMS; ++it) raw[it] = __builtin_amdgcn_raw_buffer_load_b128(xrs2, voff[it], c0 * 4, 0);
+                } else {
+#pragma unroll
+                    for (int it = 0; it < C::HALO_ITEMS; ++it) raw[it] = __builtin_amdgcn_raw_buffer_load_b128(xrs, voff[it], c0 * 4, 0);
+                }
+                return;
+            }
+            const int c0 = ch * 16;
             if constexpr (XF != 0) {
                 screg = *reinterpret_cast<const f32x4*>(d.scale + c0 + (ptid & 3) * 4);
                 shreg = *reinterpret_cast<const f32x4*>(d.shift + c0 + (ptid & 3) * 4);
@@ -130,16 +158,18 @@
 #pragma unroll
             for (int it = 0; it < C::HALO_ITEMS; ++it) raw[it] = __builtin_amdgcn_raw_buffer_load_b128(xrs, voff[it], c0 * 4, 0);
         };
-        auto split_all = [&]() {
+        auto split_items = [&](auto do_xf_c) {
+            constexpr bool DO_XF = decltype(do_xf_c)::value;
+            const float slope = TWO ? ld_slope : d.slope;
 #pragma unroll
             for (int it = 0; it < C::HALO_ITEMS; ++it) {
                 f32x4 v = __builtin_bit_cast(f32x4, raw[it]);
-                if constexpr (XF != 0) {
+                if constexpr (DO_XF) {
 #pragma unroll
                     for (int e = 0; e < 4; ++e) {
                         float t = v[e] * screg[e] + shreg[e];
                         if constexpr (XF == 1) asm("v_max_f32 %0, 0, %1" : "=v"(t) : "v"(t));
-                        else t = __builtin_fmaxf(t, t * d.slope);
+                        else t = __builtin_fmaxf(t, t * slope);
                         v[e] = __builtin_bit_cast(float, __builtin_bit_cast(unsigned, t) & vmsk[it]);
                     }
                 }
@@ -150,6 +180,14 @@
                     pl[it][0] = cvt_pair(v.x, v.y);
                     pl[it][1] = cvt_pair(v.z, v.w);
                 }
+            }
+        };
+        auto split_all = [&]() {
+            if constexpr (TWO && XF != 0) {
+                if (ld_xf) split_items(std::true_type{});
+                else split_items(std::false_type{});
+            } else {
+                split_items(std::integral_constant<bool, XF != 0>{});
             }
         };
         auto write_all = [&](int buf) {
@@ -200,7 +238,7 @@
                         setup_halo(lt);
                     }
                 }
-                issue_loads(lch * 16);
+                issue_loads(lch);
                 __builtin_amdgcn_sched_barrier(0);
                 WS_T(t2);
                 wait_vmcnt<C::HALO_ITEMS>();
@@ -505,7 +543,7 @@
     }
 }
 
-template <int TB, int TH, int TW, int NTL, int XF, int P>
+template <int TB, int TH, int TW, int NTL, int XF, int P, bool TWO = false>
 void launch_ws(rfi_ctx* ctx, ConvArgs& a, WsDev& d) {
     constexpr bool ADB = NTL == 1 || P == 1;
     using C = WsCfg<TB, TH, TW, NTL, ADB, P>;
@@ -521,7 +559,7 @@
     d.stats = a.stats;
     static PerDeviceOnce attr_once;
     attr_once.run(ctx->device, [&] {
-        RFI_CHECK_HIP(hipFuncSetAttribute(reinterpret_cast<const void*>(&conv_ws_kernel<TB, TH, TW, NTL, XF, ADB, P>),
+        RFI_CHECK_HIP(hipFuncSetAttribute(reinterpret_cast<const void*>(&conv_ws_kernel<TB, TH, TW, NTL, XF, ADB, P, TWO>),
                                           hipFuncAttributeMaxDynamicSharedMemorySize, (int)C::LDS_BYTES));
     });
 #ifdef RFI_DIAG_STAMPS
@@ -529,7 +567,7 @@
         const size_t nw = (size_t)GX * ycols * 8;
         RFI_CHECK_HIP(hipMalloc(reinterpret_cast<void**>(&d.stamps), nw * 64));
         RFI_CHECK_HIP(hipMemsetAsync(d.stamps, 0, nw * 64, ctx->stream));
-        hipLaunchKernelGGL((conv_ws_kernel<TB, TH, TW, NTL, XF, ADB, P>), dim3(GX, ycols), dim3(512), C::LDS_BYTES, ctx->stream, d);
+        hipLaunchKernelGGL((conv_ws_kernel<TB, TH, TW, NTL, XF, ADB, P, TWO>), dim3(GX, ycols), dim3(512), C::LDS_BYTES, ctx->stream, d);
         std::vector<unsigned long long> hs(nw * 8);
         RFI_CHECK_HIP(hipMemcpyAsync(hs.data(), d.stamps, nw * 64, hipMemcpyDeviceToHost, ctx->stream));
         RFI_CHECK_HIP(hipStreamSynchronize(ctx->stream));
@@ -546,20 +584,25 @@
     }
 #endif
     if (a.done) {
-        hipExtLaunchKernelGGL((conv_ws_kernel<TB, TH, TW, NTL, XF, ADB, P>), dim3(GX, ycols), dim3(512), C::LDS_BYTES, ctx->stream, nullptr,
+        hipExtLaunchKernelGGL((conv_ws_kernel<TB, TH, TW, NTL, XF, ADB, P, TWO>), dim3(GX, ycols), dim3(512), C::LDS_BYTES, ctx->stream, nullptr,
                               a.done, 0, d);
         a.done_used = true;
     } else {
-        hipLaunchKernelGGL((conv_ws_kernel<TB, TH, TW, NTL, XF, ADB, P>), dim3(GX, ycols), dim3(512), C::LDS_BYTES, ctx->stream, d);
+        hipLaunchKernelGGL((conv_ws_kernel<TB, TH, TW, NTL, XF, ADB, P, TWO>), dim3(GX, ycols), dim3(512), C::LDS_BYTES, ctx->stream, d);
     }
     check_launch("conv_ws");
 }
 
-template <int NTL, int XF, int P>
+template <int NTL, int XF, int P, bool TWO = false>
 void dispatch_ws(rfi_ctx* ctx, ConvArgs& a, WsDev& d) {
-    if (a.W >= 32) launch_ws<1, 8, 32, NTL, XF, P>(ctx, a, d);
-    else if (a.W >= 16) launch_ws<1, 16, 16, NTL, XF, P>(ctx, a, d);
-    else launch_ws<4, 8, 8, NTL, XF, P>(ctx, a, d);
+    if (a.W >= 32) launch_ws<1, 8, 32, NTL, XF, P, TWO>(ctx, a, d);
+    else if (a.W >= 16) launch_ws<1, 16, 16, NTL, XF, P, TWO>(ctx, a, d);
+    else launch_ws<4, 8, 8, NTL, XF, P, TWO>(ctx, a, d);
+}
+template <int NTL>
+void dispatch_two(rfi_ctx* ctx, ConvArgs& a, WsDev& d, int xf) {
+    if (xf == 1) dispatch_ws<NTL, 1, 3, true>(ctx, a, d);
+    else dispatch_ws<NTL, 2, 3, true>(ctx, a, d);
 }
 template <int NTL, int P>
 void dispatch_xf(rfi_ctx* ctx, ConvArgs& a, WsDev& d, int xf) {
@@ -567,6 +610,8 @@
     else if (xf == 1) dispatch_ws<NTL, 1, P>(ctx, a, d);
     else dispatch_ws<NTL, 2, P>(ctx, a, d);
 }
+
+int xf_kind(const InXform& xf) { return !xf.scale ? 0 : (xf.relu == 1 || (xf.relu == 2 && xf.slope == 0.0f)) ? 1 : 2; }
 
 }
 
@@ -578,17 +623,31 @@
     if (a.Cin % 16 != 0 || a.x.pstride % 4 != 0 || (reinterpret_cast<uintptr_t>(a.x.p) & 15)) return false;
     if (a.xf.scale && ((reinterpret_cast<uintptr_t>(a.xf.scale) & 15) || (reinterpret_cast<uintptr_t>(a.xf.shift) & 15))) return false;
     if ((int64_t)a.N * a.H * a.W * a.x.pstride * 4 >= (int64_t)1 << 31 || (int64_t)a.N * a.H * a.W * a.y.pstride >= (int64_t)1 << 31) return false;
+    if (a.x2.p) {
+        if (a.Cin2 <= 0 || a.Cin2 >= a.Cin || a.Cin2 % 16 != 0 || (a.Cin - a.Cin2) % 16 != 0) return false;
+        if (a.x2.pstride != a.x.pstride || a.x.pstride < std::max(a.Cin - a.Cin2, a.Cin2) || (reinterpret_cast<uintptr_t>(a.x2.p) & 15)) return false;
+        if (a.xf2.scale && ((reinterpret_cast<uintptr_t>(a.xf2.scale) & 15) || (reinterpret_cast<uintptr_t>(a.xf2.shift) & 15))) return false;
+        const int ka = xf_kind(a.xf), kb = xf_kind(a.xf2);
+        if (ka == 0 && kb == 0) return false;
+        if (ka != 0 && kb != 0 && ka != kb) return false;
+    }
     return true;
 }
 
 void launch_conv_ws(rfi_ctx* ctx, ConvArgs& a, const bf16_t* wB, int P) {
     RFI_REQUIRE(conv_ws_eligible(a), "conv_ws: shape not eligible");
     RFI_REQUIRE(P == 1 || P == 3, "conv_ws: planes must be 1 or 3");
+    const bool two = a.x2.p != nullptr;
+    RFI_REQUIRE(!two || P == 3, "conv_ws: two sources exist in the 3 x bf16 arithmetic only");
     WsDev d;
     d.x = a.x.p; d.x_ps = a.x.pstride;
     d.x_bytes = (unsigned)((int64_t)a.N * a.H * a.W * a.x.pstride * 4);
     d.scale = a.xf.scale; d.shift = a.xf.shift;
     d.slope = a.xf.relu == 0 ? 1.0f : a.xf.slope;
+    d.x2 = a.x2.p; d.scale2 = a.xf2.scale; d.shift2 = a.xf2.shift;
+    d.slope2 = a.xf2.relu == 0 ? 1.0f : a.xf2.slope;
+    d.nkc_a = two ? (a.Cin - a.Cin2) / 16 : plane_chunks(a.Cin);
+    d.xf_a = xf_kind(a.xf); d.xf_b = xf_kind(a.xf2);
     d.N = a.N; d.H = a.H; d.W = a.W; d.Cin = a.Cin; d.Cout = a.Cout;
     d.wB = wB;
     d.nkc = plane_chunks(a.Cin); d.ncb = (a.Cout + 31) / 32;
@@ -606,12 +665,16 @@
     std::string label;
     if (ctx->profiling)
         label = "conv_ws N" + std::to_string(a.N) + " " + std::to_string(a.H) + "x" + std::to_string(a.W) + " " +
-                std::to_string(a.Cin) + "->" + std::to_string(a.Cout) + (a.xf.scale ? " xf" : "") + (P == 3 ? " 3xbf16" : " bf16") +
+                std::to_string(a.Cin) + "->" + std::to_string(a.Cout) + (a.xf.scale ? " xf" : "") + (two ? (a.xf2.scale ? " 2src xf2" : " 2src") : "") +
+                (P == 3 ? " 3xbf16" : " bf16") +
                 (a.W >= 32 ? " t8x32" : a.W >= 16 ? " t16x16" : " t4x8x8") + " ntl" + std::to_string(ntl);
     const double bytes = 4.0 * ((double)a.N * a.H * a.W * a.Cin + 9.0 * a.Cin * a.Cout) + 4.0 * a.N * a.H * a.W * a.Cout;
     ProfScope ps(ctx, FAM_CONV_MFMA, flops, bytes, label);
-    const int xf = !a.xf.scale ? 0 : (a.xf.relu == 1 || (a.xf.relu == 2 && a.xf.slope == 0.0f)) ? 1 : 2;
-    if (P == 3) {
+    const int xf = two ? std::max(d.xf_a, d.xf_b) : xf_kind(a.xf);
+    if (two) {
+        if (ntl == 2) dispatch_two<2>(ctx, a, d, xf);
+        else dispatch_two<1>(ctx, a, d, xf);
+    } else if (P == 3) {
         if (ntl == 2) dispatch_xf<2, 3>(ctx, a, d, xf);
         else dispatch_xf<1, 3>(ctx, a, d, xf);
     } else {
diff --git a/rfi_toolbox_amd/csrc/elem_kernels.hip b/rfi_toolbox_amd/csrc/elem_kernels.hip
--- a/rfi_toolbox_amd/csrc/elem_kernels.hip
+++ b/rfi_toolbox_amd/csrc/elem_kernels.hip
@@ -1518,6 +1518,18 @@
     launch_channel_sum(ctx, YRef(v.p, (int64_t)v.pstride), M, C, partial_ws, out, finish);
 }
 
+void launch_concat_sources(rfi_ctx* ctx, View a, int Ca, View b, int Cb, InXform xf_b, int N, int H, int W, float* out) {
+    const size_t M = (size_t)N * H * W, ps = (size_t)(Ca + Cb) * 4;
+    RFI_CHECK_HIP(hipMemcpy2DAsync(out, ps, a.p, (size_t)a.pstride * 4, (size_t)Ca * 4, M, hipMemcpyDeviceToDevice, ctx->stream));
+    if (xf_b.scale) {
+        RFI_REQUIRE(xf_b.relu != 0 && b.pstride == Cb, "concat_sources: the second source's transform is BatchNorm + (Leaky)ReLU of a dense tensor");
+        launch_bn_relu_pool(ctx, b.p, N, H, W, Cb, xf_b.scale, xf_b.shift, MutView{out + Ca, Ca + Cb}, nullptr,
+                            xf_b.relu == 2 ? xf_b.slope : 0.0f);
+    } else {
+        RFI_CHECK_HIP(hipMemcpy2DAsync(out + Ca, ps, b.p, (size_t)b.pstride * 4, (size_t)Cb * 4, M, hipMemcpyDeviceToDevice, ctx->stream));
+    }
+}
+
 void launch_bn_relu_pool(rfi_ctx* ctx, const float* y, int N, int H, int W, int C,
                          const float* scale, const float* shift, MutView skip, float* pooled, float slope) {
     const int64_t total = (int64_t)N * (H / 2) * (W / 2) * C;
diff --git a/rfi_toolbox_amd/csrc/kernels.hpp b/rfi_toolbox_amd/csrc/kernels.hpp
--- a/rfi_toolbox_amd/csrc/kernels.hpp
+++ b/rfi_toolbox_amd/csrc/kernels.hpp
@@ -41,6 +41,9 @@
     unsigned short* y16 = nullptr;
     int fold = 0;
     InXform xf;
+    View x2;
+    int Cin2 = 0;
+    InXform xf2;
     double algo_flops = -1;
     bool bf16 = false;
     bool bf16x3 = false;
@@ -74,6 +77,9 @@
 struct WgradArgs {
     View xop, yop;
     InXform xf_x, xf_y;
+    View xop2;
+    int Cx2 = 0;
+    InXform xf_x2;
     int N = 0, H = 0, W = 0;
     int Hx = 0, Wx = 0;
     int Cx = 0, Cy = 0;
@@ -139,6 +145,7 @@
 
 void launch_bn_relu_pool(rfi_ctx* ctx, const float* y, int N, int H, int W, int C,
                          const float* scale, const float* shift, MutView skip, float* pooled, float slope = 0.0f);
+void launch_concat_sources(rfi_ctx* ctx, View a, int Ca, View b, int Cb, InXform xf_b, int N, int H, int W, float* out);
 void launch_pool_bwd_merge(rfi_ctx* ctx, YRef y, int N, int H, int W, int C,
                            const float* scale, const float* shift, YRef dskip, YRef dpool,
                            float* da, float slope = 0.0f, unsigned short* da16 = nullptr);
diff --git a/rfi_toolbox_amd/csrc/model.cpp b/rfi_toolbox_amd/csrc/model.cpp
--- a/rfi_toolbox_amd/csrc/model.cpp
+++ b/rfi_toolbox_amd/csrc/model.cpp
@@ -146,7 +146,7 @@
         for (int i : {decY1[l], decY2[l], gA[l], gB[l]}) bufs[i].ensure(ctx, M * C);
         if (!planesP && !resnet_encoder) for (int i : {gAe[l], gBe[l]}) bufs[i].ensure(ctx, M * C);
         if (!resnet_encoder) for (int i : {encY1[l], encY2[l]}) bufs[i].ensure(ctx, M * C);
-        bufs[concat[l]].ensure(ctx, M * 2 * C);
+        bufs[concat[l]].ensure(ctx, M * ((planesP || resnet_encoder) ? 2 : 1) * C);
         bufs[dconcat[l]].ensure(ctx, M * 2 * C);
         if (!resnet_encoder || l == D) {
             bufs[pool[l]].ensure(ctx, M / 4 * C);
@@ -482,8 +482,9 @@
 }
 
 void rfi_model::conv_bn(ConvBN& c, View in, InXform xf, Shape s, const float* w, const float* w3, int R, int pad, int cin,
-                        float* Y, bool train, double flops) {
+                        float* Y, bool train, double flops, View in2, int cin2, InXform xf2) {
     ConvArgs a = conv_same(in, xf, s, R, pad, cin, c.cout, w, w3, c.has_bias ? params + c.b_off : nullptr, Y);
+    a.x2 = in2; a.Cin2 = cin2; a.xf2 = xf2;
     a.algo_flops = flops;
     float* ws = buf(ws_red);
     if (train) {
@@ -556,9 +557,27 @@
     forward_pass(x_dev, n, h, w, train_mode);
 }
 
+bool UNetModel::skip_in_place(int l) {
+    if (planesP || resnet_encoder || arith != Arith::X3) return false;
+    const int k = depth - l, C = ups[k].cout;
+    ConvBN& c1 = convs[i_bott + 2 + 2 * k];
+    const Shape s{pN, pH >> (l - 1), pW >> (l - 1)};
+    ConvArgs a = conv_same(View{buf(concat[l]), C}, InXform{}, s, 3, 1, c1.cin_p, c1.cout, params + c1.w_off, c1.w3, nullptr, buf(decY1[l]));
+    a.x2 = View{buf(encY2[l]), C}; a.Cin2 = C; a.xf2 = bn_xf(convs[2 * (l - 1) + 1]);
+    if (c1.cin_p != 2 * C || !a.bf16x3 || !a.wB3 || !conv_ws_eligible(a)) return false;
+    WgradArgs wa = wgrad_same(a.x, InXform{}, buf(gB[l]), s, 3, 1, c1.cin_p, c1.cout, grads + c1.w_off);
+    wa.xop2 = a.x2; wa.Cx2 = C; wa.xf_x2 = a.xf2;
+    return wgrad_ws_eligible(wa);
+}
+
 void UNetModel::forward_pass(const float* x_dev, int n, int h, int w, bool train_mode) {
     if (planesP) return forward_planes(x_dev, n, h, w, train_mode);
     const int D = depth, IB = i_bott;
+    skip_direct.assign(D + 1, 0);
+    if (!resnet_encoder) for (int l = 1; l <= D; ++l) {
+        skip_direct[l] = skip_in_place(l) ? 1 : 0;
+        if (!skip_direct[l]) bufs[concat[l]].ensure(ctx, (size_t)n * (h >> (l - 1)) * (w >> (l - 1)) * 2 * ((size_t)feat << (l - 1)));
+    }
     auto run_conv_bn = [&](ConvBN& c, View in, InXform xf, Shape s, float* Y) {
         conv_bn(c, in, xf, s, params + c.w_off, c.w3, 3, 1, c.cin_p, Y, train_mode, 2.0 * s.N * s.H * s.W * 9.0 * c.cin * c.cout);
     };
@@ -572,7 +591,7 @@
         if (l == 1) side_rebuild_wd();
         run_conv_bn(c2, View{buf(encY1[l]), c1.cout}, bn_xf(c1), s, buf(encY2[l]));
         launch_bn_relu_pool(ctx, buf(encY2[l]), s.N, s.H, s.W, c2.cout, c2.scale(), c2.shift(),
-                            MutView{buf(concat[l]) + c2.cout, 2 * c2.cout}, buf(pool[l]), act_slope);
+                            skip_direct[l] ? MutView{} : MutView{buf(concat[l]) + c2.cout, 2 * c2.cout}, buf(pool[l]), act_slope);
         cur = View{buf(pool[l]), c2.cout};
     }
     {
@@ -590,11 +609,15 @@
         Shape sin{n, h >> l, w >> l};
         Shape s{n, h >> (l - 1), w >> (l - 1)};
         ConvArgs a = convt_args(u, View{prevY, u.cin}, bn_xf(*prevBN), sin);
-        a.y = MutView{buf(concat[l]), 2 * u.cout};
+        const bool direct = !resnet_encoder && skip_direct[l];
+        a.y = MutView{buf(concat[l]), direct ? u.cout : 2 * u.cout};
         launch_conv(ctx, a);
         ConvBN& c1 = convs[IB + 2 + 2 * k];
         ConvBN& c2 = convs[IB + 2 + 2 * k + 1];
-        run_conv_bn(c1, View{buf(concat[l]), 2 * u.cout}, InXform{}, s, buf(decY1[l]));
+        if (direct)
+            conv_bn(c1, View{buf(concat[l]), u.cout}, InXform{}, s, params + c1.w_off, c1.w3, 3, 1, c1.cin_p, buf(decY1[l]), train_mode,
+                    2.0 * s.N * s.H * s.W * 9.0 * c1.cin * c1.cout, View{buf(encY2[l]), u.cout}, u.cout, bn_xf(convs[2 * (l - 1) + 1]));
+        else run_conv_bn(c1, View{buf(concat[l]), 2 * u.cout}, InXform{}, s, buf(decY1[l]));
         run_conv_bn(c2, View{buf(decY1[l]), c1.cout}, bn_xf(c1), s, buf(decY2[l]));
         prevY = buf(decY2[l]);
         prevBN = &c2;
@@ -723,7 +746,8 @@
 
 void backward_conv_bn(UNetModel* m, ConvBN& c, float* dA, const float* Y, View in, InXform in_xf,
                       Shape s, float* dx, int have_records,
-                      const float* head_dl = nullptr, const float* head_w = nullptr) {
+                      const float* head_dl = nullptr, const float* head_w = nullptr,
+                      View in2 = View{}, int cin2 = 0, InXform in2_xf = InXform{}) {
     rfi_ctx* ctx = m->ctx;
     const int64_t M = (int64_t)s.N * s.H * s.W;
     float* ws = m->buf(m->ws_red);
@@ -739,6 +763,7 @@
                         m->grads + c.b_off, m->act_slope, nullptr, 0, 0, dy_done, !m->dbias_deferred, head_dl, head_w);
     WgradArgs wa = m->wgrad_same(in, in_xf, dA, s, 3, 1, c.cin_p, c.cout, m->grads + c.w_off);
     wa.algo_flops = 2.0 * s.N * s.H * s.W * 9.0 * c.cin * c.cout;
+    wa.xop2 = in2; wa.Cx2 = cin2; wa.xf_x2 = in2_xf;
     if (!dx) {
         m->wgrad_on_side(wa, dy_done);
         return;
@@ -797,8 +822,12 @@
         backward_conv_bn(this, c2, buf(gA[l]), buf(decY2[l]), View{buf(decY1[l]), c1.cout}, bn_xf(c1), s,
                          buf(gB[l]), l == 1 ? head_records : 0, from_head ? buf(dlogits) : nullptr,
                          from_head ? params + head_w_off : nullptr);
-        backward_conv_bn(this, c1, buf(gB[l]), buf(decY1[l]), View{buf(concat[l]), 2 * u.cout}, InXform{}, s,
-                         buf(dconcat[l]), 0);
+        if (skip_direct[l])
+            backward_conv_bn(this, c1, buf(gB[l]), buf(decY1[l]), View{buf(concat[l]), u.cout}, InXform{}, s, buf(dconcat[l]), 0,
+                             nullptr, nullptr, View{buf(encY2[l]), u.cout}, u.cout, bn_xf(convs[2 * (l - 1) + 1]));
+        else
+            backward_conv_bn(this, c1, buf(gB[l]), buf(decY1[l]), View{buf(concat[l]), 2 * u.cout}, InXform{}, s,
+                             buf(dconcat[l]), 0);
         const float* prevY = (l == D) ? buf(bottY2) : buf(decY2[l + 1]);
         ConvBN& prevBN = (l == D) ? convs[IB + 1] : convs[IB + 2 + 2 * (k - 1) + 1];
         View dUp{buf(dconcat[l]), 2 * u.cout};
@@ -903,7 +932,17 @@
     else if (base == "decY2") level(decY2, 1);
     else if (base == "gA") level(!planesP && !resnet_encoder ? gAe : gA, 1);
     else if (base == "gB") level(!planesP && !resnet_encoder ? gBe : gB, 1);
-    else if (base == "concat") level(concat, 2);
+    else if (base == "concat") {
+        level(concat, 2);
+        if (to_host && (size_t)idx < skip_direct.size() && skip_direct[idx]) {
+            const int C = feat << (idx - 1);
+            if (concat_dbg < 0) concat_dbg = new_buf();
+            bufs[concat_dbg].ensure(ctx, n);
+            launch_concat_sources(ctx, View{buf(concat[idx]), C}, C, View{buf(encY2[idx]), C}, C, bn_xf(convs[2 * (idx - 1) + 1]),
+                                  pN, pH >> (idx - 1), pW >> (idx - 1), buf(concat_dbg));
+            src = buf(concat_dbg);
+        }
+    }
     else if (base == "dconcat") {
         level(dconcat, 2);
         if (convt_planes && planesP == 1 && to_host) {
diff --git a/rfi_toolbox_amd/csrc/model.hpp b/rfi_toolbox_amd/csrc/model.hpp
--- a/rfi_toolbox_amd/csrc/model.hpp
+++ b/rfi_toolbox_amd/csrc/model.hpp
@@ -236,7 +236,8 @@
     rfi::WgradArgs wgrad_same(rfi::View x, rfi::InXform xf_x, const float* dy, rfi::Shape s, int R, int pad, int cin, int cout,
                               float* dw) const;
     void conv_bn(rfi::ConvBN& c, rfi::View in, rfi::InXform xf, rfi::Shape s, const float* w, const float* w3, int R, int pad,
-                 int cin, float* Y, bool train, double flops);
+                 int cin, float* Y, bool train, double flops, rfi::View in2 = rfi::View{}, int cin2 = 0,
+                 rfi::InXform xf2 = rfi::InXform{});
     rfi::ConvArgs convt_args(const rfi::UpConv& u, rfi::View x, rfi::InXform xf, rfi::Shape s) const;
     void convt_backward(const rfi::UpConv& u, rfi::View dup, rfi::View x, rfi::InXform xf, rfi::Shape s, float* dx);
 
@@ -290,6 +291,9 @@
     rfi::InXform bn_xf(const rfi::ConvBN& c) const { return rfi::act_of(c, act_slope); }
     std::vector<int> encY1, encY2, concat, pool, decY1, decY2, gA, gB, dconcat, dpool;
     std::vector<int> gAe, gBe;
+    std::vector<char> skip_direct;
+    int concat_dbg = -1;
+    bool skip_in_place(int l);
     int bottY1 = -1, bottY2 = -1, gBottA = -1, gBottB = -1;
     float* dbias_pool = nullptr;
     void* dbias_descs = nullptr;
diff --git a/rfi_toolbox_amd/csrc/wgrad_mfma.hip b/rfi_toolbox_amd/csrc/wgrad_mfma.hip
--- a/rfi_toolbox_amd/csrc/wgrad_mfma.hip
+++ b/rfi_toolbox_amd/csrc/wgrad_mfma.hip
@@ -411,6 +411,24 @@
 
 void launch_wgrad(rfi_ctx* ctx, const WgradArgs& a_in, int impl) {
     WgradArgs a = a_in;
+    if (a.xop2.p) {
+        WgradArgs t = a;
+        if (impl == IMPL_MFMA_BF16) t.bf16 = true;
+        if (impl == IMPL_MFMA_BF16X3) t.bf16x3 = true;
+        const bool in_place = impl != IMPL_DIRECT && impl != IMPL_PLANES_X3 && impl != IMPL_PLANES_BF16 && (t.bf16x3 || t.bf16) &&
+                              !wgrad_stem_eligible(t) && wgrad_ws_eligible(t) && wgrad_split_eligible(t);
+        if (!in_place) {
+            RFI_REQUIRE(a.R == 3 && a.S == 1 && a.Cx2 > 0 && a.Cx2 < a.Cx && !a.xf_x.scale,
+                        "wgrad: a second source needs a 3x3 stride-1 conv whose first source has no transform");
+            CallScope sc(ctx);
+            float* cat = sc.temp<float>((size_t)a.N * a.Hx * a.Wx * a.Cx);
+            launch_concat_sources(ctx, a.xop, a.Cx - a.Cx2, a.xop2, a.Cx2, a.xf_x2, a.N, a.Hx, a.Wx, cat);
+            a.xop = View{cat, a.Cx};
+            a.xop2 = View{}; a.Cx2 = 0; a.xf_x2 = InXform{};
+            launch_wgrad(ctx, a, impl);
+            return;
+        }
+    }
     if (impl == IMPL_PLANES_X3 || impl == IMPL_PLANES_BF16) {
         RFI_REQUIRE(a.R == 3 && a.S == 1, "wgrad: the plane kernel covers 3x3 stride-1 convolutions");
         launch_pwgrad_from_f32(ctx, a, impl == IMPL_PLANES_X3 ? 3 : 1);
diff --git a/rfi_toolbox_amd/csrc/wgrad_ws.hip b/rfi_toolbox_amd/csrc/wgrad_ws.hip
--- a/rfi_toolbox_amd/csrc/wgrad_ws.hip
+++ b/rfi_toolbox_amd/csrc/wgrad_ws.hip
@@ -87,12 +87,19 @@
             ysc = *reinterpret_cast<const f32x4*>(a.xf_y.scale + cyq);
             ysh = *reinterpret_cast<const f32x4*>(a.xf_y.shift + cyq);
         }
-        if (a.xf_x.scale && x_cok) {
-            xsc = *reinterpret_cast<const f32x4*>(a.xf_x.scale + cxq);
-            xsh = *reinterpret_cast<const f32x4*>(a.xf_x.shift + cxq);
+        const bool two = XM == 2 && R == 3 && ST == 1 && a.xop2.p != nullptr;
+        const bool x_b = two && cxq >= a.Cx - a.Cx2;
+        const int cxs = x_b ? cxq - (a.Cx - a.Cx2) : cxq;
+        const InXform& xfs = x_b ? a.xf_x2 : a.xf_x;
+        const bool x_has = xfs.scale != nullptr;
+        const float x_slope = xfs.relu ? xfs.slope : 1.0f;
+        if (xfs.scale && x_cok) {
+            xsc = *reinterpret_cast<const f32x4*>(xfs.scale + cxs);
+            xsh = *reinterpret_cast<const f32x4*>(xfs.shift + cxs);
         }
         const __amdgpu_buffer_rsrc_t yrs = __builtin_amdgcn_make_buffer_rsrc(const_cast<float*>(a.yop.p), 0, (int)d.y_bytes, 0x00020000);
         const __amdgpu_buffer_rsrc_t xrs = __builtin_amdgcn_make_buffer_rsrc(const_cast<float*>(a.xop.p), 0, (int)d.x_bytes, 0x00020000);
+        const __amdgpu_buffer_rsrc_t xrs2 = __builtin_amdgcn_make_buffer_rsrc(const_cast<float*>(two ? a.xop2.p : a.xop.p), 0, (int)d.x_bytes, 0x00020000);
         constexpr unsigned NOWHERE = 0x81000000u, OUTSIDE = 0x80000000u;
         unsigned y_rel[C::Y_ITEMS], x_rel[C::X_ITEMS];
         int y_dyx[C::Y_ITEMS], x_dyx[C::X_ITEMS];
@@ -105,7 +112,7 @@
 #pragma unroll
         for (int it = 0; it < C::X_ITEMS; ++it) {
             const int pix = xpix0 + it * XSTEP, dy = pix / C::HW, dx = pix % C::HW;
-            x_rel[it] = (pix < C::HP && x_cok) ? (unsigned)((dy * a.Wx + dx) * a.xop.pstride + cxq) * 4u : NOWHERE;
+            x_rel[it] = (pix < C::HP && x_cok) ? (unsigned)((dy * a.Wx + dx) * a.xop.pstride + cxs) * 4u : NOWHERE;
             x_dyx[it] = pix < C::HP ? (dy << 16) | dx : 0x7fff7fff;
         }
         const int y_lds = (yq >> 3) * (C::BM * C::ROW) + (yq & 7) * 8 + ypix0 * C::ROW;
@@ -141,7 +148,23 @@
                     yvalid |= (ok ? 1u : 0u) << it;
                 }
             }
-            if (xin) {
+            if (two) {
+                xvalid = xin ? ~0u : 0u;
+                unsigned off[C::X_ITEMS];
+#pragma unroll
+                for (int it = 0; it < C::X_ITEMS; ++it) {
+                    const bool ok = xin || ((unsigned)(iy0 + (x_dyx[it] >> 16)) < (unsigned)a.Hx && (unsigned)(ix0 + (x_dyx[it] & 0xffff)) < (unsigned)a.Wx);
+                    off[it] = ok ? xbase + x_rel[it] : OUTSIDE;
+                    if (!xin) xvalid |= (ok ? 1u : 0u) << it;
+                }
+                if (!x_b) {
+#pragma unroll
+                    for (int it = 0; it < C::X_ITEMS; ++it) xreg[it] = __builtin_amdgcn_raw_buffer_load_b128(xrs, off[it], 0, 0);
+                } else {
+#pragma unroll
+                    for (int it = 0; it < C::X_ITEMS; ++it) xreg[it] = __builtin_amdgcn_raw_buffer_load_b128(xrs2, off[it], 0, 0);
+                }
+            } else if (xin) {
                 xvalid = ~0u;
 #pragma unroll
                 for (int it = 0; it < C::X_ITEMS; ++it) xreg[it] = __builtin_amdgcn_raw_buffer_load_b128(xrs, xbase + x_rel[it], 0, 0);
@@ -185,6 +208,19 @@
             }
             return v;
         };
+        auto xform_two = [&](f32x4 v, auto mask_c, unsigned valid) {
+            const unsigned m = (unsigned)__builtin_amdgcn_sbfe((int)valid, 0, 1);
+#pragma unroll
+            for (int e = 0; e < 4; ++e) {
+                float t = v[e] * xsc[e] + xsh[e];
+                const float u = t * x_slope;
+                asm("v_max_f32 %0, %1, %2" : "=v"(t) : "v"(t), "v"(u));
+                t = x_has ? t : v[e];
+                if constexpr (decltype(mask_c)::value) t = __builtin_bit_cast(float, __builtin_bit_cast(unsigned, t) & m);
+                v[e] = t;
+            }
+            return v;
+        };
         auto store_tile = [&](int buf, const TileRegs& tr) {
             const u32x4 (&yreg)[C::Y_ITEMS] = tr.yreg;
             const u32x4 (&xreg)[C::X_ITEMS] = tr.xreg;
@@ -199,7 +235,21 @@
                 if (do_y) v = xform(v, ysc, ysh, a.xf_y, std::true_type{}, yvalid >> it);
                 if (it * YSTEP + YSTEP <= C::BM || ypix0 + it * YSTEP < C::BM) put(v, sY + it * YSTEP * C::ROW);
             }
-            if (do_x && !xin) {
+            if (two) {
+                if (!xin) {
+#pragma unroll
+                    for (int it = 0; it < C::X_ITEMS; ++it) {
+                        const f32x4 v = xform_two(__builtin_bit_cast(f32x4, xreg[it]), std::true_type{}, xvalid >> it);
+                        if (it * XSTEP + XSTEP <= C::HP || xpix0 + it * XSTEP < C::HP) put(v, sX + it * XSTEP * C::ROW);
+                    }
+                } else {
+#pragma unroll
+                    for (int it = 0; it < C::X_ITEMS; ++it) {
+                        const f32x4 v = xform_two(__builtin_bit_cast(f32x4, xreg[it]), std::false_type{}, 0u);
+                        if (it * XSTEP + XSTEP <= C::HP || xpix0 + it * XSTEP < C::HP) put(v, sX + it * XSTEP * C::ROW);
+                    }
+                }
+            } else if (do_x && !xin) {
 #pragma unroll
                 for (int it = 0; it < C::X_ITEMS; ++it) {
                     const f32x4 v = xform(__builtin_bit_cast(f32x4, xreg[it]), xsc, xsh, a.xf_x, std::true_type{}, xvalid >> it);
@@ -404,7 +454,7 @@
             label = "wgrad_ws R" + std::to_string(R) + (ST == 2 ? "s2" : "") + " N" + std::to_string(a.N) + " " + std::to_string(a.H) + "x" +
                     std::to_string(a.W) + " cx" + std::to_string(a.Cx) + " cy" + std::to_string(a.Cy) + " split" +
                     std::to_string(p.nsplit) + (P == 3 ? " 3xbf16" : " bf16") + " b" + std::to_string(BYB) + "x" + std::to_string(BXB) +
-                    " t" + std::to_string(TH) + "x" + std::to_string(TW) + " xm" + std::to_string(XM) + (PWV == 8 ? " pw8" : "");
+                    " t" + std::to_string(TH) + "x" + std::to_string(TW) + " xm" + std::to_string(XM) + (PWV == 8 ? " pw8" : "") + (a.xop2.p ? " 2src" : "");
         const double bytes = 4.0 * ((double)a.N * a.Hx * a.Wx * a.Cx + (double)a.N * a.H * a.W * a.Cy + (double)R * R * a.Cx * a.Cy);
         ProfScope ps(ctx, FAM_WGRAD_MFMA, flops, bytes, label);
 #ifdef RFI_DIAG_STAMPS
@@ -434,7 +484,7 @@
 void select(rfi_ctx* ctx, const WgradArgs& a) {
     const bool y2 = a.Cy > 32, x2 = a.Cx > 32;
     const bool p1 = a.bf16 && !a.bf16x3;
-    const bool xm1 = R == 3 && a.xf_x.scale && a.xf_x.relu == 1 && a.xf_x.slope == 0.0f && !a.xf_y.scale;
+    const bool xm1 = R == 3 && a.xf_x.scale && a.xf_x.relu == 1 && a.xf_x.slope == 0.0f && !a.xf_y.scale && !a.xop2.p;
 #define RFI_WW(BYB_, BXB_, TH_, TW_)                                                \
     do {                                                                            \
         if constexpr (R == 3) {                                                     \
@@ -488,6 +538,12 @@
     if ((reinterpret_cast<uintptr_t>(a.xop.p) & 15) || (reinterpret_cast<uintptr_t>(a.yop.p) & 15)) return false;
     if ((int64_t)a.N * a.Hx * a.Wx * a.xop.pstride * 4 >= 0x7f000000ll || (int64_t)a.N * a.H * a.W * a.yop.pstride * 4 >= 0x7f000000ll) return false;
     if (((int64_t)a.Wx + 1) * a.xop.pstride * 4 >= (1 << 24)) return false;
+    if (a.xop2.p) {
+        if (!(a.R == 3 && a.S == 1 && a.pad == 1) || a.Cx2 <= 0 || a.Cx2 >= a.Cx || a.Cx2 % 16 || (a.Cx - a.Cx2) % 16) return false;
+        if (a.xop2.pstride != a.xop.pstride || a.xop.pstride < std::max(a.Cx - a.Cx2, a.Cx2) || (reinterpret_cast<uintptr_t>(a.xop2.p) & 15)) return false;
+        for (const InXform* xf : {&a.xf_x, &a.xf_x2})
+            if (xf->scale && ((reinterpret_cast<uintptr_t>(xf->scale) & 15) || (reinterpret_cast<uintptr_t>(xf->shift) & 15))) return false;
+    }
     if (a.R == 2 && a.S == 2 && a.pad == 0) {
         return a.Hx == 2 * a.H && a.Wx == 2 * a.W;
     }
```

After: 8953 patches/s. 0.979x the previous value.
